# medivhna/TF_Face_Toolbox

Hardware: AMD Instinct MI355X
Metric: images/sec (whole node), SphereFaceNet-20 112x112 bs512 (higher is better)
Workload: dtype f32; 1 GPU; SphereFaceNet-20 + A-softmax training step, 112x112x3, global batch 512, 10575 classes, Momentum, fp32; global_batch=512, per_gpu_batch=512, parallelism=dp1

## Files before the change

include/fte.h:

```cpp
#ifndef FTE_H_
#define FTE_H_

#include <stddef.h>
#include <stdint.h>

#ifdef __cplusplus
extern "C" {
#endif

#define FTE_OK 0
#define FTE_EINVAL (-1)
#define FTE_EWORKSPACE (-2)

const char* fte_version(void);

#define FTE_MFMA_F32 0
#define FTE_MFMA_BF16 1
int fte_set_mfma_dtype(int dtype);
int fte_get_mfma_dtype(void);

#define FTE_CONV_DIRECT 0
#define FTE_CONV_WINOGRAD 1
#define FTE_CONV_AUTO 2
int fte_set_conv_algo(int algo);
int fte_get_conv_algo(void);
int fte_conv3x3_algo(int n, int h, int wd, int cin, int cout, int stride, int op);
size_t fte_wino_pack_bytes(int n, int h, int wd, int c);

int fte_prof_enable(int on);
int fte_prof_count(void);
int fte_prof_get(int i, int* sig, double* flops, float* ms);
int fte_prof_get_shape(int i, int* mnk, double* bytes);
int fte_prof_get_name(int i, char* buf, int buflen);


int fte_conv3x3_fwd(const float* x, const float* w, const float* bias, const float* alpha,
                    const float* res, float* z, float* y,
                    int n, int h, int wd, int cin, int cout, int stride,
                    void* ws, size_t ws_bytes, void* stream);
size_t fte_conv3x3_fwd_ws_bytes(int n, int h, int wd, int cin, int cout, int stride);
int fte_conv3x3_fwd_keep(const float* x, const float* w, const float* bias, const float* alpha,
                         const float* res, float* z, float* y,
                         int n, int h, int wd, int cin, int cout, int stride, float* vpack,
                         void* ws, size_t ws_bytes, void* stream);
int fte_conv3x3_fwd_keep_act(const float* x, const float* xalpha, const float* w, const float* bias, const float* alpha,
                             const float* res, float* z, float* y,
                             int n, int h, int wd, int cin, int cout, int stride, float* vpack,
                             void* ws, size_t ws_bytes, void* stream);

int fte_conv3x3_dgrad(const float* dz, const float* w, const float* addin,
                      const float* zprev, const float* alpha_prev,
                      float* raw, float* dzprev, float* dalpha_prev, float* dbias_prev,
                      int n, int h, int wd, int cin, int cout, int stride,
                      void* ws, size_t ws_bytes, void* stream);
size_t fte_conv3x3_dgrad_ws_bytes(int n, int h, int wd, int cin, int cout, int stride);

int fte_conv3x3_wgrad(const float* x, const float* dz, float* dw,
                      int n, int h, int wd, int cin, int cout, int stride,
                      void* ws, size_t ws_bytes, void* stream);
size_t fte_conv3x3_wgrad_ws_bytes(int n, int h, int wd, int cin, int cout, int stride);
int fte_conv3x3_wgrad_kept(const float* x, const float* dz, float* dw,
                           int n, int h, int wd, int cin, int cout, int stride, const float* vpack,
                           void* ws, size_t ws_bytes, void* stream);


int fte_conv2d_fwd(const float* x, const float* w, const float* bias, const float* alpha, const float* res,
                   float* z, float* y, int n, int h, int wd, int cin, int cout, int ksize, int stride,
                   void* ws, size_t ws_bytes, void* stream);
size_t fte_conv2d_fwd_ws_bytes(int n, int h, int wd, int cin, int cout, int ksize, int stride);
int fte_conv2d_dgrad(const float* dz, const float* w, const float* addin, const float* zprev,
                     const float* alpha_prev, float* raw, float* dzprev, float* dalpha_prev, float* dbias_prev,
                     int n, int h, int wd, int cin, int cout, int ksize, int stride,
                     void* ws, size_t ws_bytes, void* stream);
size_t fte_conv2d_dgrad_ws_bytes(int n, int h, int wd, int cin, int cout, int ksize, int stride);
int fte_conv2d_wgrad(const float* x, const float* dz, float* dw, int n, int h, int wd, int cin, int cout,
                     int ksize, int stride, void* ws, size_t ws_bytes, void* stream);
size_t fte_conv2d_wgrad_ws_bytes(int n, int h, int wd, int cin, int cout, int ksize, int stride);

int fte_im2col_first(const float* x, float* cols, int n, int h, int wd, int cin, int ksize, int stride,
                     int kpad, void* stream);
int fte_im2col_first_s16(const float* x, uint16_t* cols16, int n, int h, int wd, int cin, int ksize, int stride, int kpad, void* stream);

int fte_preprocess_u8(const uint8_t* slots, float* out, int n, long slot_stride, int channels, int in_h, int in_w, int crop_h, int crop_w,
                      void* stream);
int fte_preprocess_u8_aug(const uint8_t* slots, float* out, int n, long slot_stride, int channels, int in_h, int in_w, int crop_h,
                          int crop_w, void* stream);
size_t fte_preprocess_u8_geo_ws_bytes(int n, int channels, int crop_h, int crop_w);
int fte_preprocess_u8_geo(const uint8_t* slots, float* out, int n, long slot_stride, int channels, int in_h, int in_w, int crop_h,
                          int crop_w, const float* affine_table, void* ws, size_t ws_bytes, void* stream);

size_t fte_bn_ws_bytes(int c);
int fte_bn_train_fwd(const float* z, const float* gamma, const float* beta, const float* res, float* y,
                     float* mean, float* rstd, float* scale, float* shift, float* moving_mean, float* moving_var,
                     long rows, int c, float eps, float decay, int relu, void* ws, size_t ws_bytes, void* stream);
int fte_bn_infer_fwd(const float* z, const float* gamma, const float* beta, const float* moving_mean,
                     const float* moving_var, const float* res, float* y, float* scale, float* shift,
                     long rows, int c, float eps, int relu, void* stream);
int fte_bn_train_bwd(const float* dy, const float* ymask, const float* z, const float* gamma, const float* mean,
                     const float* rstd, float* dz, float* dgamma, float* dbeta, long rows, int c,
                     void* ws, size_t ws_bytes, void* stream);
int fte_bn_train_bwd_zmask(const float* dy, const float* z, const float* gamma, const float* mean, const float* rstd,
                           const float* scale, const float* shift, float* dz, float* dgamma, float* dbeta, long rows, int c,
                           void* ws, size_t ws_bytes, void* stream);
int fte_bn_train_bwd_res(const float* dy, const float* y, const float* z, const float* gamma, const float* mean, const float* rstd,
                         float* g_out, float* dz, float* dgamma, float* dbeta, long rows, int c,
                         void* ws, size_t ws_bytes, void* stream);
int fte_bn_train_stats(const float* z, const float* gamma, const float* beta, float* mean, float* rstd, float* scale, float* shift,
                       float* moving_mean, float* moving_var, long rows, int c, float eps, float decay,
                       void* ws, size_t ws_bytes, void* stream);
int fte_bn_infer_coef(const float* gamma, const float* beta, const float* moving_mean, const float* moving_var,
                      float* scale, float* shift, int c, float eps, void* stream);
size_t fte_bn_prelu_ws_bytes(int c);
int fte_bn_prelu_apply(const float* z, const float* scale, const float* shift, const float* alpha, float* y, long rows, int c,
                       void* stream);
int fte_bn_prelu_infer_fwd(const float* z, const float* gamma, const float* beta, const float* moving_mean, const float* moving_var,
                           const float* alpha, float* y, float* scale, float* shift, long rows, int c, float eps, void* stream);
int fte_bn_prelu_train_bwd(const float* dy, const float* z, const float* gamma, const float* mean, const float* rstd,
                           const float* scale, const float* shift, const float* alpha, float* dz, float* dgamma, float* dbeta,
                           float* dalpha, long rows, int c, void* ws, size_t ws_bytes, void* stream);
size_t fte_se_lin_ws_bytes(int n, int hw, int c);
int fte_se_lin_squeeze(const float* z, const float* scale, const float* shift, const float* mean, const float* rstd, float* sq, float* xm,
                       int n, int hw, int c, void* ws, size_t ws_bytes, void* stream);
int fte_se_lin_apply_fwd(const float* z, const float* scale, const float* shift, const float* gate, const float* shortcut, float* out,
                         int n, int hw, int c, void* stream);
int fte_se_lin_bwd_sums(const float* dy, const float* z, const float* gamma, const float* beta, const float* mean, const float* rstd,
                        const float* gate, float* s1, float* s2, float* dgate, int n, int hw, int c, void* ws, size_t ws_bytes, void* stream);
int fte_relu_bwd(const float* dy, const float* y, float* g, long n, void* stream);

int fte_maxpool3x3s2_fwd(const float* x, float* y, uint8_t* idx, int n, int h, int wd, int c, void* stream);
int fte_maxpool3x3s2_bwd(const float* dy, const uint8_t* idx, float* dx, int n, int h, int wd, int c, void* stream);
int fte_gap_fwd(const float* x, float* y, int n, int hw, int c, void* stream);
int fte_gap_bwd(const float* dy, float* dx, int n, int hw, int c, void* stream);
int fte_dropout_fwd(const float* x, float* mask, float* y, long n, float keep_prob, uint64_t seed, void* stream);
int fte_dropout_bwd(const float* dy, const float* mask, float* dx, long n, float keep_prob, void* stream);

int fte_gconv3x3_fwd(const float* x, const float* w, float* y, int n, int h, int wd, int c, int groups,
                     int stride, void* stream);
int fte_gconv3x3_pack_bf16(const float* w, uint16_t* wpk_fwd, uint16_t* wpk_dgrad, int c, int groups, void* stream);
// ... 245 lines not shown
```

tf_face_toolbox_amd/_lib.py:

```python
import ctypes
import os
from ctypes import c_char_p, c_float, c_int, c_long, c_size_t, c_uint64, c_void_p

_HERE = os.path.dirname(os.path.abspath(__file__))
LIB_PATH = os.environ.get('FTE_LIB') or os.path.join(_HERE, 'libfte.so')


class FteError(RuntimeError):
    pass


_P = c_void_p
_SIGS = {
    'fte_version': (c_char_p, []),
    'fte_prof_enable': (c_int, [c_int]),
    'fte_prof_count': (c_int, []),
    'fte_prof_get': (c_int, [c_int, _P, _P, _P]),
    'fte_prof_get_shape': (c_int, [c_int, _P, _P]),
    'fte_prof_get_name': (c_int, [c_int, _P, c_int]),
    'fte_conv3x3_fwd': (c_int, [_P] * 7 + [c_int] * 6 + [_P, c_size_t, _P]),
    'fte_conv3x3_fwd_ws_bytes': (c_size_t, [c_int] * 6),
    'fte_conv3x3_dgrad': (c_int, [_P] * 9 + [c_int] * 6 + [_P, c_size_t, _P]),
    'fte_conv3x3_dgrad_ws_bytes': (c_size_t, [c_int] * 6),
    'fte_conv3x3_wgrad': (c_int, [_P] * 3 + [c_int] * 6 + [_P, c_size_t, _P]),
# ... 19 lines not shown
    'fte_bn_train_stats': (c_int, [_P] * 9 + [c_long, c_int, c_float, c_float, _P, c_size_t, _P]),
    'fte_bn_infer_coef': (c_int, [_P] * 6 + [c_int, c_float, _P]),
    'fte_bn_prelu_ws_bytes': (c_size_t, [c_int]),
    'fte_bn_prelu_apply': (c_int, [_P] * 5 + [c_long, c_int, _P]),
    'fte_bn_prelu_infer_fwd': (c_int, [_P] * 9 + [c_long, c_int, c_float, _P]),
    'fte_bn_prelu_train_bwd': (c_int, [_P] * 12 + [c_long, c_int, _P, c_size_t, _P]),
    'fte_se_lin_ws_bytes': (c_size_t, [c_int] * 3),
    'fte_se_lin_squeeze': (c_int, [_P] * 7 + [c_int] * 3 + [_P, c_size_t, _P]),
    'fte_se_lin_apply_fwd': (c_int, [_P] * 6 + [c_int] * 3 + [_P]),
    'fte_se_lin_bwd_sums': (c_int, [_P] * 10 + [c_int] * 3 + [_P, c_size_t, _P]),
    'fte_relu_bwd': (c_int, [_P] * 3 + [c_long, _P]),
    'fte_maxpool3x3s2_fwd': (c_int, [_P] * 3 + [c_int] * 4 + [_P]),
    'fte_maxpool3x3s2_bwd': (c_int, [_P] * 3 + [c_int] * 4 + [_P]),
    'fte_gap_fwd': (c_int, [_P] * 2 + [c_int] * 3 + [_P]),
    'fte_gap_bwd': (c_int, [_P] * 2 + [c_int] * 3 + [_P]),
    'fte_dropout_fwd': (c_int, [_P] * 3 + [c_long, c_float, c_uint64, _P]),
    'fte_dropout_bwd': (c_int, [_P] * 3 + [c_long, c_float, _P]),
    'fte_gconv3x3_fwd': (c_int, [_P] * 3 + [c_int] * 6 + [_P]),
    'fte_gconv3x3_pack_bf16': (c_int, [_P] * 3 + [c_int, c_int, _P]),
    'fte_gconv3x3_bf16': (c_int, [_P] * 3 + [c_int] * 6 + [_P]),
    'fte_gconv3x3_wgrad_bf16_ws_bytes': (c_size_t, [c_int] * 6),
    'fte_gconv3x3_wgrad_bf16': (c_int, [_P] * 3 + [c_int] * 6 + [_P, c_size_t, _P]),
    'fte_gconv3x3_dgrad': (c_int, [_P] * 3 + [c_int] * 6 + [_P]),
    'fte_gconv3x3_wgrad': (c_int, [_P] * 3 + [c_int] * 6 + [_P, c_size_t, _P]),
    'fte_gconv3x3_wgrad_ws_bytes': (c_size_t, [c_int] * 6),
    'fte_bcast_add': (c_int, [_P] * 2 + [c_int] * 3 + [c_float, _P]),
    'fte_act_fwd': (c_int, [_P] * 2 + [c_long, c_int, _P]),
    'fte_act_bwd': (c_int, [_P] * 3 + [c_long, c_int, _P]),
    'fte_channel_scale_fwd': (c_int, [_P] * 3 + [c_int] * 3 + [_P]),
    'fte_channel_scale_bwd': (c_int, [_P] * 5 + [c_int] * 4 + [_P]),
    'fte_to_bf16': (c_int, [_P, _P, c_long, _P]),
    'fte_pack_weights_bf16': (c_int, [_P, _P, _P, c_int, c_int, c_int, _P]),
    'fte_pack_weights_bf16_table': (c_int, [_P, _P, _P, c_int, c_long, c_int, _P]),
    'fte_conv2d_fwd16': (c_int, [_P] * 8 + [c_int] * 7 + [_P, c_size_t, _P]),
    'fte_conv2d_dgrad16': (c_int, [_P] * 10 + [c_int] * 7 + [_P, c_size_t, _P]),
    'fte_conv2d_wgrad16': (c_int, [_P] * 3 + [c_int] * 7 + [_P, c_size_t, _P]),
    'fte_conv2d_fwd_s16': (c_int, [_P] * 9 + [c_int] * 7 + [_P, c_size_t, _P]),
    'fte_conv2d_dgrad_s16': (c_int, [_P] * 9 + [c_int] * 7 + [_P, c_size_t, _P]),
    'fte_conv3x3_first_fwd_s16': (c_int, [_P] * 6 + [c_int] * 6 + [_P]),
    'fte_conv3x3_first_wgrad_s16': (c_int, [_P] * 3 + [c_int] * 6 + [_P, c_size_t, _P]),
    'fte_bn_train_fwd_s16': (c_int, [_P] * 11 + [c_long, c_int, c_float, c_float, c_int, c_int, _P, c_size_t, _P]),
    'fte_bn_infer_fwd_s16': (c_int, [_P] * 9 + [c_long, c_int, c_float, c_int, c_int, _P]),
    'fte_bn_train_bwd_s16': (c_int, [_P] * 12 + [c_long, c_int, c_int, _P, c_size_t, _P]),
    'fte_relu_bwd_s16': (c_int, [_P] * 3 + [c_long, _P]),
    'fte_maxpool3x3s2_fwd_s16': (c_int, [_P] * 3 + [c_int] * 4 + [_P]),
    'fte_maxpool3x3s2_bwd_s16': (c_int, [_P] * 3 + [c_int] * 4 + [_P]),
    'fte_gap_fwd_s16': (c_int, [_P] * 2 + [c_int] * 3 + [_P]),
    'fte_gap_bwd_s16': (c_int, [_P] * 2 + [c_int] * 3 + [_P]),
    'fte_gconv3x3_bf16_s16': (c_int, [_P] * 3 + [c_int] * 6 + [_P]),
    'fte_gconv3x3_wgrad_bf16_s16': (c_int, [_P] * 3 + [c_int] * 6 + [_P, c_size_t, _P]),
    'fte_channel_scale_fwd_s16': (c_int, [_P] * 3 + [c_int] * 3 + [_P]),
    'fte_channel_scale_bwd_s16': (c_int, [_P] * 4 + [c_int] * 4 + [_P]),
    'fte_channel_scale_bwd_apply_s16': (c_int, [_P] * 4 + [c_int] * 3 + [c_float, _P]),
    'fte_dense_small': (c_int, [_P] * 5 + [c_int] * 5 + [_P]),
    'fte_se_squeeze': (c_int, [_P] * 7 + [c_int] * 4 + [_P]),
    'fte_se_apply_fwd': (c_int, [_P] * 6 + [c_int] * 4 + [_P]),
    'fte_se_bwd_gate': (c_int, [_P] * 12 + [c_int] * 4 + [_P]),
    'fte_se_bn_bwd_coef': (c_int, [_P] * 11 + [c_int] * 3 + [_P]),
    'fte_se_bn_bwd_apply': (c_int, [_P] * 6 + [c_int] * 4 + [_P]),
    'fte_dwconv3x3_fwd_s16': (c_int, [_P] * 3 + [c_int] * 5 + [_P]),
    'fte_dwconv3x3_dgrad_s16': (c_int, [_P] * 3 + [c_int] * 5 + [_P]),
    'fte_dwconv3x3_wgrad_s16': (c_int, [_P] * 3 + [c_int] * 5 + [_P, c_size_t, _P]),
    'fte_channel_gather_s16': (c_int, [_P] * 4 + [c_long] + [c_int] * 3 + [_P]),
    'fte_channel_gather_affine_s16': (c_int, [_P] * 4 + [c_int, _P, _P, c_int, c_long, c_int, c_int, _P, _P, c_int, _P, _P, c_int, _P]),
    'fte_bn_train_stats_s16': (c_int, [_P] * 9 + [c_long, c_int, c_float, c_float, c_int, _P, c_size_t, _P]),
    'fte_conv2d_bn_fwd_ws_bytes': (c_size_t, [c_int] * 7),
    'fte_conv2d_bn_fwd': (c_int, [_P] * 11 + [c_float, c_float] + [_P] * 3 + [c_int] * 8 + [_P, c_size_t, _P]),
    'fte_conv2d_bn_fwd_folds': (c_int, [c_int] * 8),
    'fte_conv2d_dgrad_bn_ws_bytes': (c_size_t, [c_int] * 7),
    'fte_conv2d_dgrad_bn': (c_int, [_P] * 14 + [c_int] * 8 + [_P, c_size_t, _P]),
    'fte_bn_apply': (c_int, [_P] * 5 + [c_long, c_int, c_int, c_int, _P]),
    'fte_bn_bwd_apply': (c_int, [_P] * 4 + [c_long, c_int, c_int, _P]),
    'fte_gconv3x3_bn_ws_bytes': (c_size_t, [c_int] * 5),
    'fte_gconv3x3_bn_fwd_bf16_s16': (c_int, [_P] * 11 + [c_float, c_float] + [_P] * 3 + [c_int] * 5 + [_P, c_size_t, _P]),
    'fte_gconv3x3_dgrad_bn_bf16_s16': (c_int, [_P] * 12 + [c_int] * 5 + [_P, c_size_t, _P]),
    'fte_set_mfma_dtype': (c_int, [c_int]),
    'fte_get_mfma_dtype': (c_int, []),
    'fte_set_conv_algo': (c_int, [c_int]),
    'fte_conv3x3_algo': (c_int, [c_int] * 7),
    'fte_wino_pack_bytes': (c_size_t, [c_int] * 4),
    'fte_conv3x3_fwd_keep': (c_int, [_P] * 7 + [c_int] * 6 + [_P, _P, c_size_t, _P]),
    'fte_conv3x3_fwd_keep_act': (c_int, [_P] * 8 + [c_int] * 6 + [_P, _P, c_size_t, _P]),
    'fte_conv3x3_wgrad_kept': (c_int, [_P] * 3 + [c_int] * 6 + [_P, _P, c_size_t, _P]),
    'fte_get_conv_algo': (c_int, []),
    'fte_l2_normalize_rows': (c_int, [_P] * 3 + [c_int] * 2 + [_P]),
    'fte_pair_scores': (c_int, [_P] * 4 + [c_int] * 3 + [_P]),
    'fte_topk_search_ws_bytes': (c_size_t, [c_int] * 4),
    'fte_topk_search': (c_int, [_P] * 2 + [c_int] * 7 + [_P] * 3 + [c_size_t, _P]),
    'fte_topk_merge': (c_int, [_P] * 2 + [c_int] * 3 + [_P] * 3),
    'fte_score_histograms': (c_int, [_P, _P, c_int, _P, _P] + [c_int] * 4 + [_P] * 3),
    'fte_template_pool': (c_int, [_P, _P, c_int, c_int, _P, c_int, _P, c_int, _P, c_int, _P, _P]),
    'fte_set_pair_scores': (c_int, [_P, c_int, c_int, _P, c_int, _P, c_int, _P, c_int, _P, _P, c_int, _P, c_int, _P, _P]),
    'fte_megaface_pair_scores': (c_int, [_P, c_int, _P, c_int, c_int, _P, _P, c_int, _P, _P]),
    'fte_megaface_scan_ws_bytes': (c_size_t, [c_int] * 2),
    'fte_megaface_scan': (c_int, [_P, c_int, _P, c_int, c_int, _P, _P, c_int, c_int, _P, _P, _P, c_size_t, _P]),
    'fte_pfc_sample_ws_bytes': (c_size_t, [c_int]),
    'fte_pfc_sample': (c_int, [_P] + [c_int] * 5 + [_P] * 4 + [c_size_t, _P]),
    'fte_pfc_gather_cols': (c_int, [_P] * 3 + [c_int] * 5 + [_P]),
    'fte_pfc_scatter_cols': (c_int, [_P] * 3 + [c_int] * 5 + [_P]),
    'fte_pfc_momentum_update_cols': (c_int, [_P] * 4 + [c_int] * 5 + [c_float] * 4 + [_P]),
    'fte_pfc_adam_update_cols': (c_int, [_P] * 5 + [c_int] * 5 + [c_float] * 6 + [c_int, _P]),
    'fte_knn_links_threshold': (c_int, [_P] * 2 + [c_int] * 2 + [c_float, c_int, _P, _P]),
    'fte_knn_links_rank_order': (c_int, [_P] * 2 + [c_int] * 2 + [c_float] * 2 + [_P, _P]),
    'fte_components': (c_int, [_P] * 2 + [c_int] * 2 + [_P] * 3),
    'fte_dwconv3x3_fwd': (c_int, [_P] * 3 + [c_int] * 5 + [_P]),
    'fte_dwconv3x3_dgrad': (c_int, [_P] * 3 + [c_int] * 5 + [_P]),
    'fte_dwconv3x3_wgrad': (c_int, [_P] * 3 + [c_int] * 5 + [_P, c_size_t, _P]),
    'fte_dwconv3x3_wgrad_ws_bytes': (c_size_t, [c_int] * 5),
    'fte_channel_gather': (c_int, [_P] * 4 + [c_long] + [c_int] * 3 + [_P]),
    'fte_channel_gather_affine': (c_int, [_P] * 4 + [c_int, _P, _P, c_int, c_long, c_int, c_int, _P, _P, c_int, _P, _P, c_int, _P]),
    'fte_conv3x3_first_fwd': (c_int, [_P] * 6 + [c_int] * 6 + [_P]),
    'fte_conv3x3_first_wgrad': (c_int, [_P] * 3 + [c_int] * 6 + [_P, c_size_t, _P]),
    'fte_conv3x3_first_wgrad_ws_bytes': (c_size_t, [c_int] * 6),
    'fte_gemm_nn': (c_int, [_P] * 4 + [c_int] * 3 + [_P, c_size_t, _P]),
    'fte_gemm_nn_act': (c_int, [_P] * 4 + [c_int] * 4 + [_P, c_size_t, _P]),
    'fte_gemm_nt': (c_int, [_P] * 4 + [c_int] + [_P] * 3 + [c_int] * 3 + [_P, c_size_t, _P]),
    'fte_gemm_tn': (c_int, [_P] * 3 + [c_int] * 3 + [_P, c_size_t, _P]),
    'fte_gemm_ws_bytes': (c_size_t, [c_int] * 3),
    'fte_softmax_ce_fwd_bwd': (c_int, [_P] * 4 + [c_int] * 3 + [c_float, _P]),
    'fte_focal_loss_fwd_bwd': (c_int, [_P] * 4 + [c_int] * 3 + [c_float] * 3 + [_P]),
    'fte_asoftmax_fwd_bwd': (c_int, [_P] * 4 + [c_float] + [_P] * 4 + [c_int] * 3 + [c_float, _P]),
    'fte_asoftmax_colcoef': (c_int, [_P] * 4 + [c_int] * 3 + [_P]),
    'fte_margin_softmax_fwd_bwd': (c_int, [_P] * 4 + [c_float] * 3 + [_P] * 4 + [c_int] * 3 + [c_float, _P]),
    'fte_margin_softmax_rows_fwd_bwd': (c_int, [_P] * 4 + [c_float] + [_P] * 6 + [c_int] * 3 + [c_float, _P]),
    'fte_subcenter_margin_softmax_fwd_bwd': (c_int, [_P] * 4 + [c_int] + [c_float] * 3 + [_P] * 4 + [c_int] * 3 + [c_float, _P]),
    'fte_subcenter_colcoef': (c_int, [_P] * 4 + [c_int] * 4 + [_P]),
    'fte_subcenter_assign': (c_int, [_P] * 3 + [c_int] + [_P] * 2 + [c_int] * 3 + [_P]),
    'fte_adaface_margins': (c_int, [_P, c_int] + [c_float] * 3 + [c_int] + [_P] * 4),
    'fte_row_norms': (c_int, [_P] * 2 + [c_int] * 3 + [_P]),
    'fte_col_norms': (c_int, [_P] * 2 + [c_int] * 3 + [_P]),
    'fte_add_scaled_rows_cols': (c_int, [_P] * 4 + [c_int] * 3 + [_P]),
    'fte_flip_width': (c_int, [_P] * 2 + [c_int] * 4 + [_P]),
    'fte_axpby': (c_int, [c_float, _P, c_float, _P, _P, c_long, _P]),
    'fte_center_loss_fwd_bwd_update': (c_int, [_P] * 5 + [c_int] * 3 + [c_float] * 2 + [_P, c_size_t, _P]),
    'fte_center_scatter_update': (c_int, [_P] * 3 + [c_int] * 3 + [c_float, _P]),
    'fte_batch_hard_triplet_fwd_bwd': (c_int, [_P] * 2 + [c_float, c_int, c_float] + [_P] * 2 + [c_int] * 2 + [_P, c_size_t, _P]),
    'fte_reduce_rows': (c_int, [_P] * 3 + [c_int, c_long, c_long, c_int, c_float, _P]),
    'fte_sumsq': (c_int, [_P, c_long, c_float, _P, _P, c_size_t, _P]),
    'fte_sum': (c_int, [_P, c_long, c_float, _P, _P, c_size_t, _P]),
    'fte_momentum_update': (c_int, [_P] * 3 + [c_long] + [c_float] * 4 + [_P]),
    'fte_adam_update': (c_int, [_P] * 4 + [c_long] + [c_float] * 6 + [c_int, _P]),
}

_lib = None


def exported_names():
    return sorted(_SIGS)


_CODES = {-1: 'FTE_EINVAL -- a null pointer, a shape the kernel family does not tile (channel multiples, stride, '
              'ksize) or a tensor of 2 GiB or more (buffer-load range)',
          -2: 'FTE_EWORKSPACE -- workspace missing or smaller than the matching *_ws_bytes() query'}

MFMA_DTYPES = {'f32': 0, 'fp32': 0, 'float32': 0, 'bf16': 1, 'bfloat16': 1, 'bf16s': 1}
_storage16 = False


def load():
    global _lib
    if _lib is not None:
        return _lib
    if not os.path.exists(LIB_PATH):
        raise FteError('libfte.so not found at %s -- build it with `python -c "import __graft_entry__ as g; g.build()"` '
                       '(or tf_face_toolbox_amd/csrc/build.sh). There is no CPU fallback.' % LIB_PATH)
    lib = ctypes.CDLL(LIB_PATH)
# ... 101 lines not shown
```

tf_face_toolbox_amd/csrc/api.hip:

```cpp
#include <hip/hip_runtime.h>
#include <stdio.h>
#include <stdlib.h>
#include <string.h>

#include <initializer_list>

#include "../../include/fte.h"
#include "igemm.h"
#include "wgrad16.h"
#include "pw16.h"
#include "kernels.h"
#include "layers.h"
#include "wino.h"
#include "search.h"
#include "partial_fc.h"
#include "cluster.h"
#include "iresnet.h"

namespace {

struct Pads { int out, before; };
inline Pads same_pads(int in, int k, int stride) {
    const int out = (in + stride - 1) / stride;
    int total = (out - 1) * stride + k - in;
// ... 267 lines not shown
    const WinoGeom g = wino_geom(n, h, wd);
    WinoWs w;
    w.v_off = align_up(head);
    if (op == 0) {
        w.u_off = w.v_off + align_up(wino_pack_floats(g.M, cin) * 4);
        w.slab_off = w.total = w.u_off + align_up((size_t)16 * cin * cout * 4);
    } else if (op == 1) {
        w.u_off = w.v_off + align_up(wino_pack_floats(g.M, cout) * 4);
        w.slab_off = w.total = w.u_off + align_up((size_t)16 * cin * cout * 4);
    } else {
        w.u_off = w.v_off + align_up(wino_pack_floats(g.M, cin) * 4);
        w.slab_off = w.u_off;
        w.total = w.slab_off + align_up((size_t)wino_wgrad_splits(cin, cout) * 16 * cin * cout * 4);
    }
    return w;
}
}

extern "C" {

#ifndef FTE_SRC_SHA
#define FTE_SRC_SHA "unstamped"
#endif
const char* fte_version(void) { return "fte 0.2 gfx950 fp32-mfma src:" FTE_SRC_SHA; }

int fte_to_bf16(const float* x, uint16_t* y, long n, void* stream) {
    if (!x || !y || n <= 0 || n % 4) return FTE_EINVAL;
    return rc(k_to_bf16(x, y, n, (hipStream_t)stream));
}
int fte_pack_weights_bf16(const float* w, uint16_t* w16, uint16_t* w16t, int ksize, int cin, int cout, void* stream) {
    if (!w || (!w16 && !w16t) || ksize <= 0 || cin <= 0 || cout <= 0) return FTE_EINVAL;
    return rc(k_pack_weights_bf16(w, w16, w16t, ksize * ksize, cin, cout, (hipStream_t)stream));
}

int fte_pack_weights_bf16_table(const float* params, uint16_t* dst, const int32_t* table, int nconv, long total, int transposed, void* stream) {
    if (!params || !dst || !table || nconv <= 0 || nconv > 64 || total <= 0 || total % 4) return FTE_EINVAL;
    return rc(k_pack_weights_table(params, dst, table, nconv, total, transposed, (hipStream_t)stream));
}

int fte_set_mfma_dtype(int dtype) {
    if (dtype != FTE_MFMA_F32 && dtype != FTE_MFMA_BF16) return FTE_EINVAL;
    igemm_set_bf16(dtype == FTE_MFMA_BF16);
    return FTE_OK;
}
int fte_get_mfma_dtype(void) { return igemm_get_bf16() ? FTE_MFMA_BF16 : FTE_MFMA_F32; }

int fte_set_conv_algo(int algo) {
    if (algo < FTE_CONV_DIRECT || algo > FTE_CONV_AUTO) return FTE_EINVAL;
    wino_set_algo(algo);
    return FTE_OK;
}
int fte_get_conv_algo(void) { return wino_get_algo(); }

int fte_prof_enable(int on) { igemm_prof_enable(on != 0, on == 1); return FTE_OK; }
int fte_prof_count(void) { return igemm_prof_count(); }
int fte_prof_get_shape(int i, int* mnk, double* bytes) {
    if (!mnk || !bytes) return FTE_EINVAL;
    return rc(igemm_prof_get_shape(i, mnk, bytes));
}
int fte_prof_get_name(int i, char* buf, int buflen) {
    if (!buf || buflen <= 0) return FTE_EINVAL;
    return rc(igemm_prof_get_name(i, buf, buflen));
}
int fte_prof_get(int i, int* sig, double* flops, float* ms) {
    if (!sig || !flops || !ms) return FTE_EINVAL;
    return rc(igemm_prof_get(i, sig, flops, ms));
}

size_t fte_conv2d_fwd_ws_bytes(int n, int h, int wd, int cin, int cout, int ksize, int stride) {
    if (n <= 0 || cin <= 0 || cin % 32 || cout <= 0 || cout % 64) return 0;
    const Pads ph = same_pads(h, ksize, stride), pw = same_pads(wd, ksize, stride);
    size_t need = both_modes([&] { return plan_rows((long)n * ph.out * pw.out, cout, (long)ksize * ksize * cin, true, false, EPI_FWD).pw_bytes; });
    if (wino_sized(n, h, wd, cin, cout, ksize, stride, 0)) {
        const size_t wn = wino_ws(n, h, wd, cin, cout, 0, 0).total;
        if (wn > need) need = wn;
    }
    return need;
}

static int conv2d_fwd_impl(const void* x, const void* w, bool src16, const float* bias, const float* alpha, const float* res,
                           float* z, float* y, uint16_t* y16, int n, int h, int wd, int cin, int cout, int ksize, int stride,
                           void* ws, size_t ws_bytes, void* stream, const uint16_t* res16 = nullptr, uint16_t* z16 = nullptr,
                           float* stat_part = nullptr, int* stat_rows = nullptr, float* vpack = nullptr,
                           const float* xalpha = nullptr, bool z_only_ok = false) {
    const bool z_only = z_only_ok && !y && z && vpack;
    if ((xalpha || z_only_ok) && !vpack) return FTE_EINVAL;
    if (!x || !w || (!y && !(src16 && y16) && !z_only) || n <= 0 || cin % 32 || cout % 64 || (stride != 1 && stride != 2) || (ksize != 1 && ksize != 3))
        return FTE_EINVAL;
    const Pads ph = same_pads(h, ksize, stride), pw = same_pads(wd, ksize, stride);
    IgemmParams p;
    zero_params(&p);
    p.M = n * ph.out * pw.out; p.N = cout; p.K = ksize * ksize * cin; p.kchunk = p.K;
    p.a_OH = ph.out; p.a_OW = pw.out; p.a_IH = h; p.a_IW = wd; p.a_stride = stride;
    p.a_ld = cin; p.a_KC = cin; p.a_NT = ksize * ksize;
    for (int r = 0; r < ksize; ++r)
        for (int s = 0; s < ksize; ++s) { p.a_dh[r * ksize + s] = r - ph.before; p.a_dw[r * ksize + s] = s - pw.before; }
    p.A = (const float*)x;
    p.B = (const float*)w;
    p.c_ld = cout;
    p.Y = y; p.Z = z; p.R = res; p.bias = bias; p.alpha = alpha; p.Y16 = y16;
    p.R16 = res16; p.Z16 = z16;
    int bl = BL_KN;
    if (src16) {
        p.src16 = 1; p.b_ld = cin; bl = BL_NK;
        for (int t = 0; t < ksize * ksize; ++t) p.b_tapoff[t] = t * cout * cin;
    } else {
        p.b_ld = cout;
    }
    if (!set_bytes(&p, (size_t)n * h * wd * cin, (size_t)ksize * ksize * cin * cout, src16 ? 2 : 4)) return FTE_EINVAL;
    if (!src16 && !stat_part && (y || z_only) && wino_wanted(n, h, wd, cin, cout, ksize, stride, 0)) {
        WinoWs wl = wino_ws(n, h, wd, cin, cout, 0, 0);
        if (vpack) { wl.u_off = 0; wl.total = align_up((size_t)16 * cin * cout * 4); }
        if (ws && ws_bytes >= wl.total) {
            if (!aligned16({x, w, bias, alpha, res, z, y, ws, vpack, xalpha})) return FTE_EINVAL;
            float* V = vpack ? vpack : (float*)((char*)ws + wl.v_off);
            float* U = (float*)((char*)ws + wl.u_off);
            hipError_t e = wino_transform_filter((const float*)w, U, cin, cout, 0, (hipStream_t)stream);
            if (e != hipSuccess) return (int)e;
            e = wino_transform_tiles((const float*)x, V, n, h, wd, cin, 0, (hipStream_t)stream, wino_fwd_small_tiles(), xalpha);
            if (e != hipSuccess) return (int)e;
            WinoMMParams q;
            memset(&q, 0, sizeof(q));
            q.V = V; q.U = U; q.K = cin; q.N = cout; q.g = wino_geom(n, h, wd);
            q.Y = y; q.Z = z; q.R = res; q.bias = bias; q.alpha = alpha;
            return rc(wino_mm(q, EPI_FWD, (hipStream_t)stream));
        }
    }
    if (vpack) return FTE_EWORKSPACE;
    RowPlan rp = plan_rows(p.M, p.N, p.K, ws != nullptr, false, EPI_FWD);
    if (rp.tail_mode >= 2 && ws_bytes < rp.pw_bytes) rp = plan_rows(p.M, p.N, p.K, false);
    if (stat_part) {
        if (rp.tail_mode == 2) return FTE_EINVAL;
        p.SP = stat_part;
        *stat_rows = (int)(rp.main_mtiles + rp.tail_mtiles);
    }
    return rc(launch_rows(p, rp, AL_MK, bl, EPI_FWD, 0, (float*)ws, (hipStream_t)stream));
}
int fte_conv2d_fwd(const float* x, const float* w, const float* bias, const float* alpha, const float* res,
                   float* z, float* y, int n, int h, int wd, int cin, int cout, int ksize, int stride,
                   void* ws, size_t ws_bytes, void* stream) {
    return conv2d_fwd_impl(x, w, false, bias, alpha, res, z, y, nullptr, n, h, wd, cin, cout, ksize, stride, ws, ws_bytes, stream);
}
int fte_conv2d_fwd16(const uint16_t* x16, const uint16_t* w16t, const float* bias, const float* alpha, const float* res,
                     float* z, float* y, uint16_t* y16, int n, int h, int wd, int cin, int cout, int ksize, int stride,
                     void* ws, size_t ws_bytes, void* stream) {
    Plan16 guard;
    return conv2d_fwd_impl(x16, w16t, true, bias, alpha, res, z, y, y16, n, h, wd, cin, cout, ksize, stride, ws, ws_bytes, stream);
}

int fte_conv2d_fwd_s16(const uint16_t* x16, const uint16_t* w16t, const float* bias, const float* alpha, const uint16_t* res16,
                       uint16_t* z16, uint16_t* y16, float* z32, float* y32, int n, int h, int wd, int cin, int cout, int ksize, int stride,
                       void* ws, size_t ws_bytes, void* stream) {
    if (!y16 || (res16 && ((uintptr_t)res16 & 15))) return FTE_EINVAL;
    Plan16 guard;
    PlanS16 storage(!z32 && !y32);
    return conv2d_fwd_impl(x16, w16t, true, bias, alpha, nullptr, z32, y32, y16, n, h, wd, cin, cout, ksize, stride, ws, ws_bytes, stream, res16, z16);
}

size_t fte_conv3x3_fwd_ws_bytes(int n, int h, int wd, int cin, int cout, int stride) {
    return fte_conv2d_fwd_ws_bytes(n, h, wd, cin, cout, 3, stride);
}
int fte_conv3x3_fwd(const float* x, const float* w, const float* bias, const float* alpha, const float* res,
                    float* z, float* y, int n, int h, int wd, int cin, int cout, int stride,
                    void* ws, size_t ws_bytes, void* stream) {
    return fte_conv2d_fwd(x, w, bias, alpha, res, z, y, n, h, wd, cin, cout, 3, stride, ws, ws_bytes, stream);
}
int fte_conv3x3_fwd_keep(const float* x, const float* w, const float* bias, const float* alpha, const float* res,
                         float* z, float* y, int n, int h, int wd, int cin, int cout, int stride, float* vpack,
                         void* ws, size_t ws_bytes, void* stream) {
    if (vpack && ((uintptr_t)vpack & 15)) return FTE_EINVAL;
    return conv2d_fwd_impl(x, w, false, bias, alpha, res, z, y, nullptr, n, h, wd, cin, cout, 3, stride, ws, ws_bytes, stream,
                           nullptr, nullptr, nullptr, nullptr, vpack);
}
int fte_conv3x3_fwd_keep_act(const float* x, const float* xalpha, const float* w, const float* bias, const float* alpha, const float* res,
                             float* z, float* y, int n, int h, int wd, int cin, int cout, int stride, float* vpack,
                             void* ws, size_t ws_bytes, void* stream) {
    if (!vpack || ((uintptr_t)vpack & 15) || (!y && !z)) return FTE_EINVAL;
    return conv2d_fwd_impl(x, w, false, bias, alpha, res, z, y, nullptr, n, h, wd, cin, cout, 3, stride, ws, ws_bytes, stream,
                           nullptr, nullptr, nullptr, nullptr, vpack, xalpha, true);
}
int fte_conv3x3_algo(int n, int h, int wd, int cin, int cout, int stride, int op) {
    if (op < 0 || op > 2) return FTE_EINVAL;
    return (!igemm_get_bf16() && wino_sized(n, h, wd, cin, cout, 3, stride, op)) ? FTE_CONV_WINOGRAD : FTE_CONV_DIRECT;
}
size_t fte_wino_pack_bytes(int n, int h, int wd, int c) {
    if (n <= 0 || h < 2 || wd < 2 || c <= 0 || c % 64) return 0;
    return wino_pack_floats(wino_geom(n, h, wd).M, c) * sizeof(float);
}

namespace {
struct DgradClass { int ph, pw, hq, wq, ntap, dh[9], dw[9], wt[9]; RowPlan rp; long mtiles; };
int dgrad_classes(int n, int h, int wd, int cin, int cout, int ksize, int stride, DgradClass* cls) {
    const Pads ph = same_pads(h, ksize, stride), pw = same_pads(wd, ksize, stride);
    int nc = 0;
    for (int a = 0; a < stride; ++a)
        for (int b = 0; b < stride; ++b) {
            DgradClass& c = cls[nc];
            c.ph = a; c.pw = b;
            c.hq = (h - a + stride - 1) / stride;
            c.wq = (wd - b + stride - 1) / stride;
            c.ntap = 0;
            if (c.hq <= 0 || c.wq <= 0) continue;
            for (int r = 0; r < ksize; ++r) {
                if ((a + ph.before - r) % stride) continue;
                for (int s = 0; s < ksize; ++s) {
                    if ((b + pw.before - s) % stride) continue;
                    c.dh[c.ntap] = (a + ph.before - r) / stride;
                    c.dw[c.ntap] = (b + pw.before - s) / stride;
                    c.wt[c.ntap] = r * ksize + s;
                    ++c.ntap;
                }
            }
            const long M = (long)n * c.hq * c.wq;
            static const bool cls_big = getenv("FTE_DGRAD_CLS_BIG") && atoi(getenv("FTE_DGRAD_CLS_BIG")) == 1;
            c.rp = plan_rows(M, cin, (long)c.ntap * cout, true, stride != 1 && !cls_big, EPI_DGRAD);
            c.mtiles = c.rp.main_mtiles + c.rp.tail_mtiles;
            ++nc;
        }
    return nc;
}
static bool dgrad_merged16() {
    static const bool on = getenv("FTE_DGRAD_MERGED16") && atoi(getenv("FTE_DGRAD_MERGED16")) == 1;
    return on && plan_bf16();
}
bool dgrad_mergeable(const DgradClass* cls, int nc, int n, int cin) {
    static const char* mode = getenv("FTE_DGRAD_CLASSES");
    if (nc != 4 || (mode && mode[0] == 's')) return false;
    for (int i = 0; i < nc; ++i)
        if (cls[i].hq != cls[0].hq || cls[i].wq != cls[0].wq || cls[i].ntap < 1) return false;
    if ((mode && mode[0] == 'm') || dgrad_merged16()) return true;
    const long tiles = (((long)n * cls[0].hq * cls[0].wq + 63) / 64) * (cin / 64);
    return tiles < SLOTS;
}
static int dgrad_merged_tile(int cin) {
    if (!dgrad_merged16()) return TILE_64x64;
    return cin % 128 == 0 ? TILE_128x128 : TILE_128x64;
}
long dgrad_merged_rows(const DgradClass* cls, int nc, int n, int cin) {
    if (!dgrad_mergeable(cls, nc, n, cin)) return 0;
    int bm, bn;
    igemm_tile_dims(dgrad_merged_tile(cin), &bm, &bn);
    return (long)nc * (((long)n * cls[0].hq * cls[0].wq + bm - 1) / bm);
}
int dgrad_merged_plan(const DgradClass* cls, int nc, int n, int cin, int* order) {
    for (int i = 0; i < nc; ++i) order[i] = i;
    for (int i = 0; i < nc; ++i)
        for (int j = i + 1; j < nc; ++j)
            if (cls[order[j]].ntap > cls[order[i]].ntap) { const int t = order[i]; order[i] = order[j]; order[j] = t; }
    (void)n;
    return dgrad_merged_tile(cin);
}
}

size_t fte_conv2d_dgrad_ws_bytes(int n, int h, int wd, int cin, int cout, int ksize, int stride) {
    if (n <= 0 || cin <= 0 || cin % 64 || cout % 32) return 0;
    size_t need = both_modes([&] {
        DgradClass cls[4];
        const int nc = dgrad_classes(n, h, wd, cin, cout, ksize, stride, cls);
        long rows = 0;
        size_t pw = 0;
        for (int i = 0; i < nc; ++i) { rows += cls[i].mtiles; if (cls[i].rp.pw_bytes > pw) pw = cls[i].rp.pw_bytes; }
        const long merged_rows = dgrad_merged_rows(cls, nc, n, cin);
        if (merged_rows > rows) rows = merged_rows;
        return 2 * align_up((size_t)rows * cin * sizeof(float)) + SCRATCH_BYTES + pw;
    });
    if (wino_sized(n, h, wd, cin, cout, ksize, stride, 1)) {
        const WinoGeom g = wino_geom(n, h, wd);
        const size_t wn = wino_ws(n, h, wd, cin, cout, 1, 2 * align_up((size_t)g.MB * cin * sizeof(float)) + SCRATCH_BYTES).total;
        if (wn > need) need = wn;
    }
    return need;
}

struct DgradBn {
    const void* zbn; const void* ybn;
    const float* gamma; const float* mean; const float* rstd; const float* scale; const float* shift;
    float* dgamma; float* dbeta; float* coef;
};
static int conv2d_dgrad_impl(const void* dz, const void* w, bool src16, const float* addin, const float* zprev,
                             const float* alpha_prev, float* raw, float* dzprev, uint16_t* dzprev16, float* dalpha_prev, float* dbias_prev,
                             int n, int h, int wd, int cin, int cout, int ksize, int stride, void* ws, size_t ws_bytes, void* stream,
                             const uint16_t* addin16 = nullptr, const uint16_t* zprev16 = nullptr, uint16_t* raw16 = nullptr,
                             const DgradBn* bn = nullptr) {
    const float* zx = nullptr;
    const uint16_t* zx16 = nullptr;
    if (bn) {
        const void* msk = (!bn->scale && bn->ybn) ? bn->ybn : bn->zbn;
        const void* zb = (!bn->scale && bn->ybn) ? bn->zbn : nullptr;
        if (src16) { zprev16 = (const uint16_t*)msk; zx16 = (const uint16_t*)zb; }
        else { zprev = (const float*)msk; zx = (const float*)zb; }
        alpha_prev = bn->gamma;
        dalpha_prev = bn->dgamma; dbias_prev = bn->dbeta;
    }
    if (zprev16 && !zprev) zprev = reinterpret_cast<const float*>(zprev16);
    const bool z16only = zprev16 != nullptr;
    if (!dz || !w || (!dzprev && !(src16 && dzprev16)) || n <= 0 || cout % 32 || cin % 64 || (stride != 1 && stride != 2) || (ksize != 1 && ksize != 3)) return FTE_EINVAL;
    if (zprev && !alpha_prev) return FTE_EINVAL;
    const Pads pho = same_pads(h, ksize, stride), pwo = same_pads(wd, ksize, stride);
    if (!src16 && !bn && dzprev && !dzprev16 && !addin16 && !zprev16 && !raw16 && wino_wanted(n, h, wd, cin, cout, ksize, stride, 1)) {
        const WinoGeom g = wino_geom(n, h, wd);
        const size_t half_w = align_up((size_t)g.MB * cin * sizeof(float));
        const WinoWs wl = wino_ws(n, h, wd, cin, cout, 1, 2 * half_w + SCRATCH_BYTES);
        if (ws && ws_bytes >= wl.total) {
            if (!aligned16({dz, w, addin, zprev, alpha_prev, raw, dzprev, ws})) return FTE_EINVAL;
            const bool part = zprev && (dalpha_prev || dbias_prev);
            float* V = (float*)((char*)ws + wl.v_off);
            float* U = (float*)((char*)ws + wl.u_off);
            hipError_t e = wino_transform_filter((const float*)w, U, cin, cout, 1, (hipStream_t)stream);
            if (e != hipSuccess) return (int)e;
            e = wino_transform_tiles((const float*)dz, V, n, h, wd, cout, 0, (hipStream_t)stream);
            if (e != hipSuccess) return (int)e;
            WinoMMParams q;
            memset(&q, 0, sizeof(q));
            q.V = V; q.U = U; q.K = cout; q.N = cin; q.g = g;
            q.ADD = addin; q.RAW = raw; q.Zin = zprev; q.alpha = alpha_prev; q.amod = cin; q.DZ = dzprev;
            q.PA = part ? (float*)ws : nullptr; q.PB = part ? (float*)((char*)ws + half_w) : nullptr;
            e = wino_mm(q, EPI_DGRAD, (hipStream_t)stream);
            if (e != hipSuccess) return (int)e;
            if (part) {
                float* scratch = (float*)((char*)ws + 2 * half_w);
                if (dalpha_prev && dbias_prev) return rc(k_reduce_rows2(q.PA, dalpha_prev, q.PB, dbias_prev, nullptr, 1, g.MB, cin, 1, 1.f, scratch, (hipStream_t)stream));
                if (dalpha_prev) return rc(k_reduce_rows(q.PA, dalpha_prev, nullptr, 1, g.MB, cin, 1, 1.f, scratch, (hipStream_t)stream));
                return rc(k_reduce_rows(q.PB, dbias_prev, nullptr, 1, g.MB, cin, 1, 1.f, scratch, (hipStream_t)stream));
            }
            return FTE_OK;
        }
    }
    DgradClass cls[4];
    const int nc = dgrad_classes(n, h, wd, cin, cout, ksize, stride, cls);
    const bool merged = dgrad_mergeable(cls, nc, n, cin);
    long rows = 0;
    for (int i = 0; i < nc; ++i) rows += cls[i].mtiles;
    if (merged) rows = dgrad_merged_rows(cls, nc, n, cin);
    const bool want_part = zprev && (dalpha_prev || dbias_prev);
    const size_t half = align_up((size_t)rows * cin * sizeof(float));
    size_t pw_need = 0;
    for (int i = 0; i < nc && !merged; ++i) if (cls[i].rp.pw_bytes > pw_need) pw_need = cls[i].rp.pw_bytes;
    const size_t fixed = 2 * half + SCRATCH_BYTES;
    if ((want_part || pw_need) && (!ws || ws_bytes < fixed + pw_need)) return FTE_EWORKSPACE;
    float* scratch = want_part ? (float*)((char*)ws + 2 * half) : nullptr;
    float* pwbuf = pw_need ? (float*)((char*)ws + fixed) : nullptr;
    float* PA = want_part ? (float*)ws : nullptr;
    float* PB = want_part ? (float*)((char*)ws + half) : nullptr;
    if (merged) {
        int order[4];
        const int tile = dgrad_merged_plan(cls, nc, n, cin, order);
        IgemmParams p;
        zero_params(&p);
        const DgradClass& c0 = cls[0];
        p.M = n * c0.hq * c0.wq; p.N = cin; p.a_KC = cout;
        p.A = (const float*)dz; p.a_OH = c0.hq; p.a_OW = c0.wq; p.a_IH = pho.out; p.a_IW = pwo.out; p.a_stride = 1; p.a_ld = cout;
        p.ncls = nc;
        int t = 0;
        for (int k = 0; k < nc; ++k) {
            const DgradClass& c = cls[order[k]];
            p.cls_tap0[k] = t; p.cls_ph[k] = c.ph; p.cls_pw[k] = c.pw;
            for (int j = 0; j < c.ntap; ++j, ++t) { p.a_dh[t] = c.dh[j]; p.a_dw[t] = c.dw[j]; p.b_tapoff[t] = c.wt[j] * cin * cout; }
        }
        p.cls_tap0[nc] = t;
        p.a_NT = t; p.K = t * cout; p.kchunk = p.K;
        p.B = (const float*)w; p.b_ld = cout;
        p.c_OH = c0.hq; p.c_OW = c0.wq; p.c_FH = h; p.c_FW = wd; p.c_step = stride; p.c_ld = cin;
        p.ADD = addin; p.RAW = raw; p.Zin = z16only ? nullptr : zprev; p.alpha = alpha_prev; p.amod = cin; p.DZ = dzprev;
        p.ADD16 = addin16; p.Zin16 = zprev16; p.RAW16 = raw16;
        p.PA = PA; p.PB = PB; p.prow0 = 0;
        if (bn) { p.bn_mu = bn->mean; p.bn_rs = bn->rstd; p.bn_sc = bn->scale; p.bn_sh = bn->shift; p.Zx = zx; p.Zx16 = zx16; }
        p.src16 = src16 ? 1 : 0; p.DZ16 = dzprev16;
        if (!set_bytes(&p, (size_t)n * pho.out * pwo.out * cout, (size_t)ksize * ksize * cin * cout, src16 ? 2 : 4)) return FTE_EINVAL;
        hipError_t e = igemm_launch(p, AL_MK, BL_NK, EPI_DGRAD, tile, 1, (hipStream_t)stream);
        if (e != hipSuccess) return (int)e;
    } else {
    long prow = 0;
    for (int i = 0; i < nc; ++i) {
        const DgradClass& c = cls[i];
        IgemmParams p;
        zero_params(&p);
        p.M = n * c.hq * c.wq; p.N = cin; p.K = c.ntap * cout; p.kchunk = p.K;
        p.A = (const float*)dz; p.a_OH = c.hq; p.a_OW = c.wq; p.a_IH = pho.out; p.a_IW = pwo.out; p.a_stride = 1;
        p.a_ld = cout; p.a_KC = cout; p.a_NT = c.ntap;
        for (int t = 0; t < c.ntap; ++t) {
            p.a_dh[t] = c.dh[t]; p.a_dw[t] = c.dw[t];
            p.b_tapoff[t] = c.wt[t] * cin * cout;
        }
        p.B = (const float*)w; p.b_ld = cout;
        p.src16 = src16 ? 1 : 0; p.DZ16 = dzprev16;
        if (stride == 1) { p.c_OH = 0; }
        else { p.c_OH = c.hq; p.c_OW = c.wq; p.c_FH = h; p.c_FW = wd; p.c_step = stride; p.c_ph = c.ph; p.c_pw = c.pw; }
        p.c_ld = cin;
        p.ADD = addin; p.RAW = raw; p.Zin = z16only ? nullptr : zprev; p.alpha = alpha_prev; p.amod = cin; p.DZ = dzprev;
        p.ADD16 = addin16; p.Zin16 = zprev16; p.RAW16 = raw16;
        p.PA = PA; p.PB = PB;
        if (bn) { p.bn_mu = bn->mean; p.bn_rs = bn->rstd; p.bn_sc = bn->scale; p.bn_sh = bn->shift; p.Zx = zx; p.Zx16 = zx16; }
        if (!set_bytes(&p, (size_t)n * pho.out * pwo.out * cout, (size_t)ksize * ksize * cin * cout, src16 ? 2 : 4)) return FTE_EINVAL;
        hipError_t e = launch_rows(p, c.rp, AL_MK, BL_NK, EPI_DGRAD, prow, pwbuf, (hipStream_t)stream);
        if (e != hipSuccess) return (int)e;
        prow += c.mtiles;
    }
    }
    if (bn)
        return rc(l_bn_bwd_finalize(PB, PA, cin, (int)rows, (long)n * h * wd, cin, bn->gamma, bn->mean, bn->rstd, bn->dgamma, bn->dbeta,
                                    bn->coef, (hipStream_t)stream));
    if (want_part) {
        if (dalpha_prev && dbias_prev) {
            hipError_t e = k_reduce_rows2(PA, dalpha_prev, PB, dbias_prev, nullptr, 1, rows, cin, 1, 1.f, scratch, (hipStream_t)stream);
            if (e != hipSuccess) return (int)e;
        } else {
            if (dalpha_prev) { hipError_t e = k_reduce_rows(PA, dalpha_prev, nullptr, 1, rows, cin, 1, 1.f, scratch, (hipStream_t)stream); if (e != hipSuccess) return (int)e; }
            if (dbias_prev) { hipError_t e = k_reduce_rows(PB, dbias_prev, nullptr, 1, rows, cin, 1, 1.f, scratch, (hipStream_t)stream); if (e != hipSuccess) return (int)e; }
        }
    }
    return FTE_OK;
}

int fte_conv2d_dgrad(const float* dz, const float* w, const float* addin, const float* zprev,
                     const float* alpha_prev, float* raw, float* dzprev, float* dalpha_prev, float* dbias_prev,
                     int n, int h, int wd, int cin, int cout, int ksize, int stride, void* ws, size_t ws_bytes, void* stream) {
    return conv2d_dgrad_impl(dz, w, false, addin, zprev, alpha_prev, raw, dzprev, nullptr, dalpha_prev, dbias_prev,
                             n, h, wd, cin, cout, ksize, stride, ws, ws_bytes, stream);
}
int fte_conv2d_dgrad16(const uint16_t* dz16, const uint16_t* w16, const float* addin, const float* zprev,
                       const float* alpha_prev, float* raw, float* dzprev, uint16_t* dzprev16, float* dalpha_prev, float* dbias_prev,
                       int n, int h, int wd, int cin, int cout, int ksize, int stride, void* ws, size_t ws_bytes, void* stream) {
    Plan16 guard;
    return conv2d_dgrad_impl(dz16, w16, true, addin, zprev, alpha_prev, raw, dzprev, dzprev16, dalpha_prev, dbias_prev,
                             n, h, wd, cin, cout, ksize, stride, ws, ws_bytes, stream);
}

int fte_conv2d_dgrad_s16(const uint16_t* dz16, const uint16_t* w16, const uint16_t* addin16, const uint16_t* zprev16,
                         const float* alpha_prev, uint16_t* raw16, uint16_t* dzprev16, float* dalpha_prev, float* dbias_prev,
                         int n, int h, int wd, int cin, int cout, int ksize, int stride, void* ws, size_t ws_bytes, void* stream) {
    if (!dzprev16) return FTE_EINVAL;
    Plan16 guard;
    PlanS16 storage(true);
    return conv2d_dgrad_impl(dz16, w16, true, nullptr, nullptr, alpha_prev, nullptr, nullptr, dzprev16, dalpha_prev, dbias_prev,
                             n, h, wd, cin, cout, ksize, stride, ws, ws_bytes, stream, addin16, zprev16, raw16);
}

size_t fte_conv3x3_dgrad_ws_bytes(int n, int h, int wd, int cin, int cout, int stride) {
    return fte_conv2d_dgrad_ws_bytes(n, h, wd, cin, cout, 3, stride);
}
int fte_conv3x3_dgrad(const float* dz, const float* w, const float* addin, const float* zprev,
                      const float* alpha_prev, float* raw, float* dzprev, float* dalpha_prev, float* dbias_prev,
                      int n, int h, int wd, int cin, int cout, int stride, void* ws, size_t ws_bytes, void* stream) {
    return fte_conv2d_dgrad(dz, w, addin, zprev, alpha_prev, raw, dzprev, dalpha_prev, dbias_prev,
                            n, h, wd, cin, cout, 3, stride, ws, ws_bytes, stream);
}

namespace {
inline bool wgrad_split_major() {
    static const bool on = !getenv("FTE_WGRAD_SPLIT_MAJOR") || atoi(getenv("FTE_WGRAD_SPLIT_MAJOR")) != 0;
    return on;
}
void wgrad_plan(int n, int h, int wd, int cin, int cout, int ksize, int stride, int* tile, int* splits, int* kchunk, int* K) {
    const Pads ph = same_pads(h, ksize, stride), pw = same_pads(wd, ksize, stride);
    *K = n * ph.out * pw.out;
    const long M = (long)ksize * ksize * cin;
    static const int wg_tile = getenv("FTE_WGRAD_TILE") ? atoi(getenv("FTE_WGRAD_TILE")) : -1;
    const int narrow = (M % 192 == 0 && M % 128 != 0) ? TILE_192x64 : TILE_128x64;
    const bool tiny = ksize == 1 && M * cout <= 256L * 256;
    *tile = wg_tile >= 0 ? wg_tile : (tiny ? TILE_64x64 : (cout % 128 == 0) ? TILE_128x128 : narrow);
    plan_splits(tiles_of(*tile, M, cout), *K, splits, kchunk, false);
    if (wg_tile < 0 && *tile != TILE_64x64 && *splits > 1 && *kchunk < 1024) {
        *tile = TILE_64x64;
        plan_splits(tiles_of(*tile, M, cout), *K, splits, kchunk, false);
    }
}
}

size_t fte_conv2d_wgrad_ws_bytes(int n, int h, int wd, int cin, int cout, int ksize, int stride) {
    if (n <= 0 || cin <= 0 || cin % 4 || cout <= 0 || cout % 64) return 0;
    int tile, splits, kchunk, K;
    wgrad_plan(n, h, wd, cin, cout, ksize, stride, &tile, &splits, &kchunk, &K);
    size_t need = splits > 1 ? (size_t)splits * ksize * ksize * cin * cout * sizeof(float) : 0;
    if (ksize == 3 && stride == 1) {
        Wgrad16Params g;
        int cfg = 0;
        if (wgrad16_plan(n, h, wd, cin, cout, &g, &cfg) && g.S > 1) {
            const size_t gneed = (size_t)g.S * g.slab * sizeof(float);
            if (gneed > need) need = gneed;
        }
    }
    if (ksize == 1 && stride == 1) {
        Wgrad16Params g;
        int cfg = 0;
        if (wgrad16p_plan(n, h, wd, cin, cout, &g, &cfg) && g.S > 1) {
            const size_t gneed = (size_t)g.S * g.slab * sizeof(float);
            if (gneed > need) need = gneed;
        }
    }
    if (wino_sized(n, h, wd, cin, cout, ksize, stride, 2)) {
        const size_t wn = wino_ws(n, h, wd, cin, cout, 2, 0).total;
        if (wn > need) need = wn;
    }
    return need + SCRATCH_BYTES;
}
size_t fte_conv3x3_wgrad_ws_bytes(int n, int h, int wd, int cin, int cout, int stride) {
    return fte_conv2d_wgrad_ws_bytes(n, h, wd, cin, cout, 3, stride);
}

static int conv2d_wgrad_impl(const void* x, const void* dz, bool src16, float* dw, int n, int h, int wd, int cin, int cout, int ksize, int stride,
                             void* ws, size_t ws_bytes, void* stream, const float* vpack = nullptr) {
    if (src16 && (cin % 8 || cout % 8)) return FTE_EINVAL;
    if ((!x && !vpack) || !dz || !dw || n <= 0 || cin % 4 || cout % 64 || (stride != 1 && stride != 2) || (ksize != 1 && ksize != 3)) return FTE_EINVAL;
    const Pads ph = same_pads(h, ksize, stride), pw = same_pads(wd, ksize, stride);
    {
        const size_t lim = (size_t)1 << 31, es = src16 ? 2 : 4;
        if ((size_t)n * h * wd * cin * es >= lim || (size_t)n * ph.out * pw.out * cout * es >= lim) return FTE_EINVAL;
    }
    int tile, splits, kchunk, K;
    wgrad_plan(n, h, wd, cin, cout, ksize, stride, &tile, &splits, &kchunk, &K);
    if (!src16 && wino_wanted(n, h, wd, cin, cout, ksize, stride, 2)) {
        WinoWs wl = wino_ws(n, h, wd, cin, cout, 2, 0);
        if (vpack) {
            const size_t vsz = wl.u_off - wl.v_off;
            wl.u_off -= vsz; wl.slab_off -= vsz; wl.total -= vsz;
        }
        if (ws && ws_bytes >= wl.total) {
            if (!aligned16({x, dz, dw, ws, vpack})) return FTE_EINVAL;
            const float* V = vpack ? vpack : (float*)((char*)ws + wl.v_off);
            float* slabs = (float*)((char*)ws + wl.slab_off);
            hipError_t e = hipSuccess;
            if (!vpack) e = wino_transform_tiles((const float*)x, (float*)((char*)ws + wl.v_off), n, h, wd, cin, 0, (hipStream_t)stream);
            if (e != hipSuccess) return (int)e;
            return rc(wino_wgrad(V, (const float*)dz, slabs, dw, wino_geom(n, h, wd), cin, cout, (hipStream_t)stream));
        }
    }
    if (vpack) return FTE_EWORKSPACE;
    if (src16 && ksize == 3 && stride == 1) {
// ... 1086 lines not shown
```

tf_face_toolbox_amd/csrc/kernels.h:

```cpp
#pragma once
#include <hip/hip_runtime.h>
#include <stdint.h>

hipError_t k_pack_weights_table(const float* params, unsigned short* w16t, const int* table, int nconv, long total, int transposed, hipStream_t st);
hipError_t k_conv_first_fwd(const float* x, const float* w, const float* bias, const float* alpha, float* z, float* y,
                            unsigned short* z16, unsigned short* y16, int n, int h, int wd, int cin, int cout, int ho, int wo, int stride, int pt, int pl, hipStream_t st);
int k_conv_first_wgrad_blocks(long npix);
hipError_t k_conv_first_wgrad(const float* x, const float* dz, const unsigned short* dz16, float* part, int n, int h, int wd, int cin, int cout, int ho, int wo,
                              int stride, int pt, int pl, int blocks, hipStream_t st);
constexpr long REDUCE_SCRATCH_FLOATS = 1 << 18;
hipError_t k_reduce_rows(const float* in, float* out, const float* bias, int bmod, long rows, long cols, int fold, float scale,
                         float* scratch, hipStream_t st, int act = 0);
hipError_t k_reduce_rows2(const float* in, float* out, const float* in2, float* out2, const float* bias, int bmod, long rows, long cols,
                          int fold, float scale, float* scratch, hipStream_t st, int act = 0);
hipError_t k_sum(const float* a, long n, float scale, float* out, float* ws, bool sq, hipStream_t st);
hipError_t k_softmax_ce(const float* logits, const int32_t* labels, float* loss_rows, float* dlogits, int n, int c, int ld, float gs, hipStream_t st);
hipError_t k_to_bf16(const float* x, unsigned short* y, long n, hipStream_t st);
hipError_t k_pack_weights_bf16(const float* w, unsigned short* w16, unsigned short* w16t, int taps, int cin, int cout, hipStream_t st);
hipError_t k_focal_loss(const float* logits, const int32_t* labels, float* loss_rows, float* dlogits, int n, int c, int ld,
                        float gamma, float alpha, float gs, hipStream_t st);
hipError_t k_asoftmax(const float* s, const float* xn, const float* wn, const int32_t* labels, float lam, float* f, float* loss_rows,
                      float* G, float* rowcoef, int n, int c, int ld, float gs, hipStream_t st);
hipError_t k_margin_softmax(const float* s, const float* xn, const float* wn, const int32_t* labels, float scale, float m, float m3,
                            float* f, float* loss_rows, float* G, float* rowcoef, int n, int c, int ld, float gs, hipStream_t st);
hipError_t k_margin_softmax_rows(const float* s, const float* xn, const float* wn, const int32_t* labels, float scale, const float* a_rows,
                                 const float* b_rows, float* f, float* loss_rows, float* G, float* rowcoef, int n, int c, int ld, float gs,
                                 hipStream_t st);
hipError_t k_subcenter_margin_softmax(const float* s, const float* xn, const float* wn, const int32_t* labels, int K, float scale, float m,
                                      float m3, float* f, float* loss_rows, float* G, float* rowcoef, int n, int c, int ld, float gs,
                                      hipStream_t st);
hipError_t k_subcenter_colcoef(const float* G, const float* s, const float* wn, float* cc, int K, int n, int c, int ld, hipStream_t st);
hipError_t k_subcenter_assign(const float* x, const float* wt, const int32_t* labels, int K, int32_t* sel, float* cosv, int n, int d, int c,
                              hipStream_t st);
hipError_t k_adaface_margins(const float* xn, int n, float m, float h, float t_alpha, int update, float* stats, float* a_rows, float* b_rows,
                             hipStream_t st);
hipError_t k_asoftmax_colcoef(const float* G, const float* s, const float* wn, float* cc, int n, int c, int ld, hipStream_t st);
hipError_t k_row_norms(const float* a, float* out, int rows, int cols, int ld, hipStream_t st);
hipError_t k_col_norms(const float* a, float* out, int rows, int cols, int ld, hipStream_t st);
hipError_t k_add_scaled(float* a, const float* b, const float* rc, const float* cc, int rows, int cols, int ld, hipStream_t st);
hipError_t k_flip_w(const float* x, float* y, long rows, int w, int c, hipStream_t st);
hipError_t k_axpby(float a, const float* x, float b, const float* y, float* out, long n, hipStream_t st);
hipError_t k_center_loss(const float* feat, const int32_t* labels, float* centers, float* loss_rows, float* dfeat,
                         int n, int d, int num_classes, float alpha, float gs, float* ws, hipStream_t st);
hipError_t k_center_update(const float* diff, const int32_t* labels, float* centers, int n, int d, int num_classes, float alpha, hipStream_t st);
hipError_t k_triplet(const float* feat, const int32_t* labels, float margin, bool soft, float lw, float* loss_rows, float* dfeat,
                     int n, int d, float* ws, hipStream_t st);
hipError_t k_dense_small(const float* a, const float* w, const float* bias, const float* mask, float* out, int m, int n, int k,
                         bool trans_w, int act, bool bf16, hipStream_t st);
hipError_t k_momentum(float* w, float* acc, const float* g, long n, float lr, float mom, float wd, float gs, hipStream_t st);
hipError_t k_adam(float* w, float* m, float* v, const float* g, long n, float lr_t, float b1, float b2, float eps, float wd, float gs, hipStream_t st);
hipError_t k_preprocess_u8(const unsigned char* slots, float* out, int n, long slot_stride, int channels, int in_h, int in_w,
                           int crop_h, int crop_w, hipStream_t st);
hipError_t k_preprocess_u8_aug(const unsigned char* slots, float* out, int n, long slot_stride, int channels, int in_h, int in_w,
                               int crop_h, int crop_w, hipStream_t st);
size_t k_preprocess_u8_geo_ws_bytes(int n, int channels, int crop_h, int crop_w);
hipError_t k_preprocess_u8_geo(const unsigned char* slots, float* out, int n, long slot_stride, int channels, int in_h, int in_w,
                               int crop_h, int crop_w, const float* table, void* ws, hipStream_t st);
```

tf_face_toolbox_amd/csrc/kernels.hip:

```cpp
#include <hip/hip_runtime.h>
#include <stdint.h>
#include <stdlib.h>
#include <math.h>

#include "kernels.h"

typedef float f32x4 __attribute__((ext_vector_type(4)));

namespace {

__device__ __forceinline__ float wave_sum(float v) {
#pragma unroll
    for (int o = 32; o > 0; o >>= 1) v += __shfl_xor(v, o);
    return v;
}
__device__ __forceinline__ float wave_max(float v) {
#pragma unroll
    for (int o = 32; o > 0; o >>= 1) v = fmaxf(v, __shfl_xor(v, o));
    return v;
}
__device__ __forceinline__ float block_sum(float v, float* sh) {
    v = wave_sum(v);
    __syncthreads();
    if ((threadIdx.x & 63) == 0) sh[threadIdx.x >> 6] = v;
// ... 91 lines not shown

typedef float f32x16k __attribute__((ext_vector_type(16)));
template <int CIN, int COUT>
__global__ __launch_bounds__(256) void conv_first_wgrad_kernel(
    const float* __restrict__ x, const float* __restrict__ dz, const unsigned short* __restrict__ dz16, float* __restrict__ part,
    int n, int h, int wd, int ho, int wo, int stride, int pt, int pl, long rows_per_block) {
    constexpr int NH = COUT / 32, K = 9 * CIN;
    __shared__ float red[4][32][COUT];
    const int lane = threadIdx.x & 63, wv = threadIdx.x >> 6;
    const int li = lane & 31, lh = lane >> 5;
    const bool kok = li < K;
    const int tap = kok ? li / CIN : 0, ch = kok ? li - tap * CIN : 0;
    const int r = tap / 3, sx = tap - r * 3;
    const long nrows = (long)n * ho;
    const long r0 = (long)blockIdx.x * rows_per_block, r1 = min(nrows, r0 + rows_per_block);
    f32x16k acc[NH];
#pragma unroll
    for (int e = 0; e < NH; ++e)
#pragma unroll
        for (int i = 0; i < 16; ++i) acc[e][i] = 0.f;
    constexpr int UP = 4;
    const int tpr = (wo + 2 * UP - 1) / (2 * UP);
    const long myrows = r1 > r0 + wv ? (r1 - r0 - wv + 3) / 4 : 0;
    const long ntrips = myrows * tpr;
    auto fetch = [&](long t, float (&a)[UP], float (&bv)[NH][UP]) {
        const long rk = t / tpr;
        const int ow0 = (int)(t - rk * tpr) * 2 * UP;
        const long row = r0 + wv + 4 * rk;
        const int img = (int)(row / ho), oh = (int)(row - (long)img * ho);
        const int ih = oh * stride + r - pt;
        const bool rok = kok && ih >= 0 && ih < h;
        const float* xrow = x + ((long)(img * h + (rok ? ih : 0)) * wd) * CIN + ch;
        const float* drow = dz ? dz + row * wo * COUT : nullptr;
        const unsigned short* drow16 = dz16 ? dz16 + row * wo * COUT : nullptr;
#pragma unroll
        for (int u = 0; u < UP; ++u) {
            const int ow = ow0 + 2 * u + lh;
            const bool pok = ow < wo;
            const int iw = ow * stride + sx - pl;
            const bool ok = rok && pok && iw >= 0 && iw < wd;
            const float av = xrow[(long)(ok ? iw : 0) * CIN];
            a[u] = ok ? av : 0.f;
            const long doff = (long)(pok ? ow : 0) * COUT + NH * li;
            if constexpr (NH == 2) {
                float v0, v1;
                if (drow) { const float2 tt = *reinterpret_cast<const float2*>(drow + doff); v0 = tt.x; v1 = tt.y; }
                else { const unsigned tt = *reinterpret_cast<const unsigned*>(drow16 + doff); v0 = __builtin_bit_cast(float, tt << 16); v1 = __builtin_bit_cast(float, tt & 0xffff0000u); }
                bv[0][u] = pok ? v0 : 0.f; bv[1][u] = pok ? v1 : 0.f;
            } else {
                const float v = drow ? drow[doff] : __builtin_bit_cast(float, (unsigned)drow16[doff] << 16);
                bv[0][u] = pok ? v : 0.f;
            }
        }
    };
    float a0[UP], b0[NH][UP], a1[UP], b1[NH][UP];
    if (ntrips > 0) fetch(0, a0, b0);
    for (long t = 0; t < ntrips; t += 2) {
        if (t + 1 < ntrips) fetch(t + 1, a1, b1);
#pragma unroll
        for (int u = 0; u < UP; ++u)
#pragma unroll
            for (int e = 0; e < NH; ++e) acc[e] = __builtin_amdgcn_mfma_f32_32x32x2f32(a0[u], b0[e][u], acc[e], 0, 0, 0);
        if (t + 1 < ntrips) {
            if (t + 2 < ntrips) fetch(t + 2, a0, b0);
#pragma unroll
            for (int u = 0; u < UP; ++u)
#pragma unroll
                for (int e = 0; e < NH; ++e) acc[e] = __builtin_amdgcn_mfma_f32_32x32x2f32(a1[u], b1[e][u], acc[e], 0, 0, 0);
        }
    }
#pragma unroll
    for (int i = 0; i < 16; ++i) {
        const int k = (i & 3) + 8 * (i >> 2) + 4 * lh;
#pragma unroll
        for (int e = 0; e < NH; ++e) red[wv][k][NH * li + e] = acc[e][i];
    }
    __syncthreads();
    for (int i = threadIdx.x; i < K * COUT; i += 256) {
        const int k = i / COUT, c = i % COUT;
        part[(long)blockIdx.x * K * COUT + i] = (red[0][k][c] + red[1][k][c]) + (red[2][k][c] + red[3][k][c]);
    }
}

__global__ __launch_bounds__(256) void reduce_rows_kernel(const float* __restrict__ in, float* __restrict__ out,
                                                          const float* __restrict__ bias, int bmod, long rows,
                                                          long cols, long rows_per_split, float scale,
                                                          const float* __restrict__ in2, float* __restrict__ out2, int act) {
    __shared__ float sh[4][64];
    if (blockIdx.z == 1) { in = in2; out = out2; }
    const int c = threadIdx.x & 63, rl = threadIdx.x >> 6;
    const long j = (long)blockIdx.x * 64 + c;
    const long r0 = (long)blockIdx.y * rows_per_split;
    const long r1 = min(rows, r0 + rows_per_split);
    float s0 = 0.f, s1 = 0.f;
    if (j < cols) {
        long r = r0 + rl;
        for (; r + 28 < r1; r += 32) {
            float v[8];
#pragma unroll
            for (int u = 0; u < 8; ++u) v[u] = in[(r + 4 * u) * cols + j];
            s0 += (v[0] + v[2]) + (v[4] + v[6]);
            s1 += (v[1] + v[3]) + (v[5] + v[7]);
        }
        for (; r + 4 < r1; r += 8) {
            s0 += in[r * cols + j];
            s1 += in[(r + 4) * cols + j];
        }
        if (r < r1) s0 += in[r * cols + j];
    }
    sh[rl][c] = s0 + s1;
    __syncthreads();
    if (rl == 0 && j < cols) {
        float v = ((sh[0][c] + sh[1][c]) + (sh[2][c] + sh[3][c])) * scale;
        if (bias) v += bias[j % bmod];
        if (act == 1) v = fmaxf(v, 0.f);
        else if (act == 2) v = 1.f / (1.f + expf(-v));
        out[(long)blockIdx.y * cols + j] = v;
    }
}

template <int QB>
__global__ __launch_bounds__(256) void reduce_slabs_kernel(const f32x4* __restrict__ in, f32x4* __restrict__ out, int rows, long quads) {
    constexpr int RL = 256 / QB;
    __shared__ f32x4 sh[RL][QB];
    const int cq = threadIdx.x % QB, rl = threadIdx.x / QB;
    const long q = (long)blockIdx.x * QB + cq;
    f32x4 s = {0.f, 0.f, 0.f, 0.f};
    if (q < quads) {
        const f32x4* src = in + q;
        int r = rl;
        for (; r + 7 * RL < rows; r += 8 * RL) {
            f32x4 v[8];
#pragma unroll
            for (int u = 0; u < 8; ++u) v[u] = src[(long)(r + u * RL) * quads];
            s += ((v[0] + v[1]) + (v[2] + v[3])) + ((v[4] + v[5]) + (v[6] + v[7]));
        }
        for (; r < rows; r += RL) s += src[(long)r * quads];
    }
    sh[rl][cq] = s;
    __syncthreads();
    if (rl == 0 && q < quads) {
        f32x4 t = sh[0][cq];
#pragma unroll
        for (int w = 1; w < RL; ++w) t += sh[w][cq];
        out[q] = t;
    }
}

template <int QB>
__global__ __launch_bounds__(256) void reduce_rows_q_kernel(const f32x4* __restrict__ in, f32x4* __restrict__ out, long rows, long quads,
                                                            long rows_per_split, const f32x4* __restrict__ in2, f32x4* __restrict__ out2) {
    constexpr int RL = 256 / QB;
    __shared__ f32x4 sh[RL][QB];
    if (blockIdx.z == 1) { in = in2; out = out2; }
    const int cq = threadIdx.x % QB, rl = threadIdx.x / QB;
    const long q = (long)blockIdx.x * QB + cq;
    const long r0 = (long)blockIdx.y * rows_per_split, r1 = min(rows, r0 + rows_per_split);
    f32x4 s = {0.f, 0.f, 0.f, 0.f};
    if (q < quads) {
        const f32x4* src = in + q;
        long r = r0 + rl;
        for (; r + 7 * RL < r1; r += 8 * RL) {
            f32x4 v[8];
#pragma unroll
            for (int u = 0; u < 8; ++u) v[u] = src[(r + u * RL) * quads];
            s += ((v[0] + v[1]) + (v[2] + v[3])) + ((v[4] + v[5]) + (v[6] + v[7]));
        }
        for (; r < r1; r += RL) s += src[r * quads];
    }
    sh[rl][cq] = s;
    __syncthreads();
    if (rl == 0 && q < quads) {
        f32x4 t = sh[0][cq];
#pragma unroll
        for (int w = 1; w < RL; ++w) t += sh[w][cq];
        out[(long)blockIdx.y * quads + q] = t;
    }
}

template <bool SQ>
__global__ __launch_bounds__(256) void partial_sum_kernel(const float* __restrict__ a, long n, float* __restrict__ part) {
    __shared__ float sh[4];
    float s = 0.f;
    const long n4 = n >> 2;
    const f32x4* a4 = reinterpret_cast<const f32x4*>(a);
    for (long i = (long)blockIdx.x * 256 + threadIdx.x; i < n4; i += (long)gridDim.x * 256) {
        const f32x4 v = a4[i];
        s += SQ ? (v[0] * v[0] + v[1] * v[1]) + (v[2] * v[2] + v[3] * v[3]) : (v[0] + v[1]) + (v[2] + v[3]);
    }
    if (blockIdx.x == 0 && threadIdx.x < (n & 3)) {
        const float v = a[(n4 << 2) + threadIdx.x];
        s += SQ ? v * v : v;
    }
    s = block_sum(s, sh);
    if (threadIdx.x == 0) part[blockIdx.x] = s;
}
__global__ __launch_bounds__(256) void final_sum_kernel(const float* __restrict__ part, int np, float scale, float* out) {
    __shared__ float sh[4];
    float s = 0.f;
    for (int i = threadIdx.x; i < np; i += 256) s += part[i];
    s = block_sum(s, sh);
    if (threadIdx.x == 0) out[0] = s * scale;
}

__global__ __launch_bounds__(256) void softmax_ce_kernel(const float* __restrict__ logits, const int32_t* __restrict__ labels,
                                                         float* __restrict__ loss_rows, float* __restrict__ dlogits,
                                                         int c, int ld, float gscale) {
    __shared__ float sh[4];
    const int row = blockIdx.x;
    const float* z = logits + (long)row * ld;
    float* d = dlogits + (long)row * ld;
    float mx = -INFINITY;
    for (int j = threadIdx.x; j < c; j += 256) mx = fmaxf(mx, z[j]);
    mx = block_max(mx, sh);
    float s = 0.f;
    for (int j = threadIdx.x; j < c; j += 256) s += expf(z[j] - mx);
    s = block_sum(s, sh);
    const int yl = labels[row];
    const bool bad = (unsigned)yl >= (unsigned)c;
    const int y = bad ? 0 : yl;
    const float inv = 1.f / s;
    for (int j = threadIdx.x; j < ld; j += 256) {
        float g = 0.f;
        if (j < c) g = (expf(z[j] - mx) * inv - (j == y ? 1.f : 0.f)) * gscale;
        d[j] = (bad && j < c) ? NAN : g;
    }
    if (threadIdx.x == 0) loss_rows[row] = bad ? NAN : logf(s) - (z[y] - mx);
}

template <int NPT>
__global__ __launch_bounds__(256) void softmax_ce_reg_kernel(const float* __restrict__ logits, const int32_t* __restrict__ labels,
                                                             float* __restrict__ loss_rows, float* __restrict__ dlogits,
                                                             int c, int ld, float gscale) {
    __shared__ float sh[4];
    const int row = blockIdx.x;
    const float* z = logits + (long)row * ld;
    float* d = dlogits + (long)row * ld;
    float v[NPT];
    float mx = -INFINITY;
#pragma unroll
    for (int i = 0; i < NPT; ++i) {
        const int j = threadIdx.x + 256 * i;
        v[i] = j < c ? z[j] : -INFINITY;
        mx = fmaxf(mx, v[i]);
    }
    mx = block_max(mx, sh);
    float s = 0.f;
#pragma unroll
    for (int i = 0; i < NPT; ++i) {
        const int j = threadIdx.x + 256 * i;
        v[i] = expf(v[i] - mx);
        if (j < c) s += v[i];
    }
    s = block_sum(s, sh);
    const int yl = labels[row];
    const bool bad = (unsigned)yl >= (unsigned)c;
    const int y = bad ? 0 : yl;
    const float inv = 1.f / s;
#pragma unroll
    for (int i = 0; i < NPT; ++i) {
// ... 835 lines not shown
    extern __shared__ float cfs[];
    const int a = blockIdx.x;
    for (int b = threadIdx.x; b < n; b += 256) cfs[b] = coef[(long)a * n + b] + coef[(long)b * n + a];
    __syncthreads();
    for (int k = threadIdx.x; k < d; k += 256) {
        float g = 0.f;
        const float fa = feat[(long)a * d + k];
        for (int b = 0; b < n; ++b) {
            const float cf = cfs[b];
            if (cf != 0.f) g += cf * (fa - feat[(long)b * d + k]);
        }
        dfeat[(long)a * d + k] = g;
    }
}

__global__ __launch_bounds__(256) void momentum_kernel(float* __restrict__ w, float* __restrict__ acc, const float* __restrict__ g,
                                                       long n, float lr, float mom, float wd, float gs) {
    const long n4 = n >> 2;
    f32x4* w4 = reinterpret_cast<f32x4*>(w);
    f32x4* a4 = reinterpret_cast<f32x4*>(acc);
    const f32x4* g4 = reinterpret_cast<const f32x4*>(g);
    for (long i = (long)blockIdx.x * 256 + threadIdx.x; i < n4; i += (long)gridDim.x * 256) {
        f32x4 wv = w4[i], av = a4[i];
        const f32x4 gv = g4[i];
        av = mom * av + (gs * gv + wd * wv);
        wv = wv - lr * av;
        a4[i] = av;
        w4[i] = wv;
    }
    if (blockIdx.x == 0 && threadIdx.x < (n & 3)) {
        const long i = (n4 << 2) + threadIdx.x;
        const float av = mom * acc[i] + (gs * g[i] + wd * w[i]);
        acc[i] = av;
        w[i] = w[i] - lr * av;
    }
}
__global__ __launch_bounds__(256) void adam_kernel(float* __restrict__ w, float* __restrict__ m, float* __restrict__ v,
                                                   const float* __restrict__ g, long n, float lr_t, float b1, float b2,
                                                   float eps, float wd, float gs) {
    for (long i = (long)blockIdx.x * 256 + threadIdx.x; i < n; i += (long)gridDim.x * 256) {
        const float gv = gs * g[i] + wd * w[i];
        const float mv = b1 * m[i] + (1.f - b1) * gv;
        const float vv = b2 * v[i] + (1.f - b2) * gv * gv;
        m[i] = mv;
        v[i] = vv;
        w[i] = w[i] - lr_t * mv / (sqrtf(vv) + eps);
    }
}

inline int grid_for(long n, int per) { long b = (n + per - 1) / per; return (int)(b < 1 ? 1 : (b > 4096 ? 4096 : b)); }

}

hipError_t k_conv_first_fwd(const float* x, const float* w, const float* bias, const float* alpha, float* z, float* y,
                            unsigned short* z16, unsigned short* y16,
                            int n, int h, int wd, int cin, int cout, int ho, int wo, int stride, int pt, int pl, hipStream_t st) {
    const long ngrp = (long)n * ho * ((wo + 31) / 32);
    long nb = (ngrp + 3) / 4;
    if (nb > 4096) nb = 4096;
    const int blocks = (int)nb;
#define FTE_CF(CI_, CO_) hipLaunchKernelGGL((conv_first_fwd_kernel<CI_, CO_>), dim3(blocks), dim3(256), 0, st, x, w, bias, alpha, z, y, z16, y16, n, h, wd, ho, wo, stride, pt, pl)
    if (cin == 1 && cout == 64) FTE_CF(1, 64);
    else if (cin == 3 && cout == 64) FTE_CF(3, 64);
    else if (cin == 1 && cout == 32) FTE_CF(1, 32);
    else if (cin == 3 && cout == 32) FTE_CF(3, 32);
    else return hipErrorInvalidValue;
#undef FTE_CF
    return hipGetLastError();
}
int k_conv_first_wgrad_blocks(long npix) { long b = (npix + 511) / 512; return (int)(b > 2048 ? 2048 : (b < 1 ? 1 : b)); }
hipError_t k_conv_first_wgrad(const float* x, const float* dz, const unsigned short* dz16, float* part, int n, int h, int wd, int cin, int cout, int ho, int wo,
                              int stride, int pt, int pl, int blocks, hipStream_t st) {
    const long nrows = (long)n * ho;
    const long rpb = (nrows + blocks - 1) / blocks;
#define FTE_CW(CI_, CO_) hipLaunchKernelGGL((conv_first_wgrad_kernel<CI_, CO_>), dim3(blocks), dim3(256), 0, st, x, dz, dz16, part, n, h, wd, ho, wo, stride, pt, pl, rpb)
    if (cin == 1 && cout == 64) FTE_CW(1, 64);
    else if (cin == 3 && cout == 64) FTE_CW(3, 64);
    else if (cin == 1 && cout == 32) FTE_CW(1, 32);
    else if (cin == 3 && cout == 32) FTE_CW(3, 32);
    else return hipErrorInvalidValue;
#undef FTE_CW
    return hipGetLastError();
}
hipError_t k_reduce_rows2(const float* in, float* out, const float* in2, float* out2, const float* bias, int bmod, long rows, long cols,
                          int fold, float scale, float* scratch, hipStream_t st, int act) {
    rows *= fold;
    cols /= fold;
    static const bool slabs_off = getenv("FTE_REDUCE_SLABS") && atoi(getenv("FTE_REDUCE_SLABS")) == 0;
    if (!slabs_off && !act && !in2 && !bias && scale == 1.f && rows >= 2 && rows < (1 << 20) && cols >= 4096 && cols % 4 == 0 &&
        (reinterpret_cast<uintptr_t>(in) | reinterpret_cast<uintptr_t>(out)) % 16 == 0) {
        const long quads = cols / 4;
        if (quads / 64 >= 1024 || rows < 32)
            hipLaunchKernelGGL(reduce_slabs_kernel<64>, dim3((unsigned)((quads + 63) / 64)), dim3(256), 0, st, reinterpret_cast<const f32x4*>(in),
                               reinterpret_cast<f32x4*>(out), (int)rows, quads);
        else
            hipLaunchKernelGGL(reduce_slabs_kernel<16>, dim3((unsigned)((quads + 15) / 16)), dim3(256), 0, st, reinterpret_cast<const f32x4*>(in),
                               reinterpret_cast<f32x4*>(out), (int)rows, quads);
        return hipGetLastError();
    }
    const unsigned nz = in2 ? 2 : 1;
    static const bool rq_off = getenv("FTE_REDUCE_ROWS_Q") && atoi(getenv("FTE_REDUCE_ROWS_Q")) == 0;
    if (!rq_off && !act && scratch && !bias && scale == 1.f && rows >= 32 && cols % 4 == 0 && cols <= 1024 &&
        (reinterpret_cast<uintptr_t>(in) | reinterpret_cast<uintptr_t>(out) | reinterpret_cast<uintptr_t>(in2) | reinterpret_cast<uintptr_t>(out2) |
         reinterpret_cast<uintptr_t>(scratch)) % 16 == 0) {
        const long quads = cols / 4;
        const int QB = quads >= 64 ? 64 : 16, RL = 256 / QB;
        const long qb = (quads + QB - 1) / QB;
        long rs = 1024 / (qb * nz);
        if (rs > rows / (8L * RL)) rs = rows / (8L * RL);
        if (rs * cols * nz > REDUCE_SCRATCH_FLOATS) rs = REDUCE_SCRATCH_FLOATS / (cols * nz);
        if (rs < 1 || rows < 256) rs = 1;
        const long rps = (rows + rs - 1) / rs;
        rs = (rows + rps - 1) / rps;
        f32x4* s1 = reinterpret_cast<f32x4*>(scratch);
        f32x4* s2 = s1 + rs * quads;
#define FTE_RQ(QB_, GY_, IN_, OUT_, ROWS_, RPS_, IN2_, OUT2_) hipLaunchKernelGGL((reduce_rows_q_kernel<QB_>), dim3((unsigned)qb, (unsigned)(GY_), nz), dim3(256), 0, st, \
            reinterpret_cast<const f32x4*>(IN_), reinterpret_cast<f32x4*>(OUT_), (long)(ROWS_), quads, (long)(RPS_), reinterpret_cast<const f32x4*>(IN2_), reinterpret_cast<f32x4*>(OUT2_))
        if (rs == 1) {
            if (QB == 64) FTE_RQ(64, 1, in, out, rows, rows, in2, out2); else FTE_RQ(16, 1, in, out, rows, rows, in2, out2);
            return hipGetLastError();
        }
        if (QB == 64) { FTE_RQ(64, rs, in, s1, rows, rps, in2, s2); FTE_RQ(64, 1, s1, out, rs, rs, s2, out2); }
        else { FTE_RQ(16, rs, in, s1, rows, rps, in2, s2); FTE_RQ(16, 1, s1, out, rs, rs, s2, out2); }
#undef FTE_RQ
        return hipGetLastError();
    }
    const long cb = (cols + 63) / 64;
    long rs = 1;
    if (scratch && cb < 512 && rows >= 64) {
        rs = 1;
        while (rs * rs < rows) ++rs;
        if (rs < 256 / cb) rs = 256 / cb;
        if (rs > 1024 / cb) rs = 1024 / cb;
        if (rs > rows / 16) rs = rows / 16;
        if (rs * cols * nz > REDUCE_SCRATCH_FLOATS) rs = REDUCE_SCRATCH_FLOATS / (cols * nz);
        if (rs < 1) rs = 1;
    }
    if (rs == 1) {
        hipLaunchKernelGGL(reduce_rows_kernel, dim3((unsigned)cb, 1, nz), dim3(256), 0, st, in, out, bias, bmod, rows, cols, rows, scale, in2, out2, act);
        return hipGetLastError();
    }
    const long rps = (rows + rs - 1) / rs;
    rs = (rows + rps - 1) / rps;
    float* scratch2 = scratch + rs * cols;
    hipLaunchKernelGGL(reduce_rows_kernel, dim3((unsigned)cb, (unsigned)rs, nz), dim3(256), 0, st, in, scratch, (const float*)nullptr, 1, rows, cols, rps, 1.f,
                       in2, scratch2, 0);
    hipLaunchKernelGGL(reduce_rows_kernel, dim3((unsigned)cb, 1, nz), dim3(256), 0, st, (const float*)scratch, out, bias, bmod, rs, cols, rs, scale,
                       (const float*)scratch2, out2, act);
    return hipGetLastError();
}
hipError_t k_reduce_rows(const float* in, float* out, const float* bias, int bmod, long rows, long cols, int fold, float scale,
                         float* scratch, hipStream_t st, int act) {
    return k_reduce_rows2(in, out, nullptr, nullptr, bias, bmod, rows, cols, fold, scale, scratch, st, act);
}
hipError_t k_sum(const float* a, long n, float scale, float* out, float* ws, bool sq, hipStream_t st) {
    const int nb = grid_for(n, 256 * 4 * 8) > 1024 ? 1024 : grid_for(n, 256 * 4 * 8);
    if (sq) hipLaunchKernelGGL(partial_sum_kernel<true>, dim3(nb), dim3(256), 0, st, a, n, ws);
    else hipLaunchKernelGGL(partial_sum_kernel<false>, dim3(nb), dim3(256), 0, st, a, n, ws);
    hipLaunchKernelGGL(final_sum_kernel, dim3(1), dim3(256), 0, st, ws, nb, scale, out);
    return hipGetLastError();
}
hipError_t k_softmax_ce(const float* logits, const int32_t* labels, float* loss_rows, float* dlogits, int n, int c, int ld, float gs, hipStream_t st) {
    if (ld <= 256 * 8) hipLaunchKernelGGL(softmax_ce_reg_kernel<8>, dim3(n), dim3(256), 0, st, logits, labels, loss_rows, dlogits, c, ld, gs);
    else if (ld <= 256 * 48) hipLaunchKernelGGL(softmax_ce_reg_kernel<48>, dim3(n), dim3(256), 0, st, logits, labels, loss_rows, dlogits, c, ld, gs);
    else hipLaunchKernelGGL(softmax_ce_kernel, dim3(n), dim3(256), 0, st, logits, labels, loss_rows, dlogits, c, ld, gs);
    return hipGetLastError();
}
namespace {
__global__ __launch_bounds__(256) void to_bf16_kernel(const float* __restrict__ x, unsigned short* __restrict__ y, long n4) {
    for (long i = (long)blockIdx.x * 256 + threadIdx.x; i < n4; i += (long)gridDim.x * 256) {
        const f32x4 v = *reinterpret_cast<const f32x4*>(x + i * 4);
        unsigned short o[4];
#pragma unroll
        for (int e = 0; e < 4; ++e) o[e] = __builtin_bit_cast(unsigned short, (__bf16)v[e]);
        *reinterpret_cast<uint2*>(y + i * 4) = make_uint2(o[0] | ((unsigned)o[1] << 16), o[2] | ((unsigned)o[3] << 16));
    }
}
__global__ __launch_bounds__(256) void pack_weights_kernel(const float* __restrict__ w, unsigned short* __restrict__ w16,
                                                           unsigned short* __restrict__ w16t, int taps, int cin, int cout) {
    const long total = (long)taps * cin * cout;
    for (long i = (long)blockIdx.x * 256 + threadIdx.x; i < total; i += (long)gridDim.x * 256) {
        const unsigned short v = __builtin_bit_cast(unsigned short, (__bf16)w[i]);
        if (w16) w16[i] = v;
        if (w16t) {
            const int co = (int)(i % cout);
            const long t2 = i / cout;
            const int ci = (int)(t2 % cin), tap = (int)(t2 / cin);
            w16t[((long)tap * cout + co) * cin + ci] = v;
        }
    }
}
typedef float f32x4k __attribute__((ext_vector_type(4)));
__global__ __launch_bounds__(256) void pack_weights_table_kernel(const float* __restrict__ params, unsigned short* __restrict__ w16t,
                                                                 const int* __restrict__ table, int nconv, long total4, int transposed) {
    __shared__ int tb[64 * 6];
    for (int i = threadIdx.x; i < nconv * 6; i += 256) tb[i] = table[i];
    __syncthreads();
    for (long i = (long)blockIdx.x * 256 + threadIdx.x; i < total4; i += (long)gridDim.x * 256) {
        int lo = 0, hi = nconv - 1;
        while (lo < hi) {
            const int mid = (lo + hi + 1) >> 1;
            if ((long)tb[mid * 6 + 5] <= i) lo = mid; else hi = mid - 1;
        }
        const int* d = tb + lo * 6;
        const int cin = d[3], cout = d[4];
        const long j = (i - d[5]) * 4;
        if (!transposed) {
            const f32x4k v = *reinterpret_cast<const f32x4k*>(params + d[0] + j);
            *reinterpret_cast<uint2*>(w16t + d[1] + j) = make_uint2(
                __builtin_bit_cast(unsigned short, (__bf16)v[0]) | ((unsigned)__builtin_bit_cast(unsigned short, (__bf16)v[1]) << 16),
                __builtin_bit_cast(unsigned short, (__bf16)v[2]) | ((unsigned)__builtin_bit_cast(unsigned short, (__bf16)v[3]) << 16));
            continue;
        }
        const int ci = (int)(j % cin);
        const long t2 = j / cin;
        const int co = (int)(t2 % cout), tap = (int)(t2 / cout);
        const float* src = params + d[0] + ((long)tap * cin + ci) * cout + co;
        unsigned short o[4];
#pragma unroll
        for (int e = 0; e < 4; ++e) o[e] = __builtin_bit_cast(unsigned short, (__bf16)src[(long)e * cout]);
        *reinterpret_cast<uint2*>(w16t + d[1] + j) = make_uint2(o[0] | ((unsigned)o[1] << 16), o[2] | ((unsigned)o[3] << 16));
    }
}
__global__ __launch_bounds__(256) void pack_weights_tiles_kernel(const float* __restrict__ params, unsigned short* __restrict__ w16t,
                                                                 const int* __restrict__ table, int nconv) {
    __shared__ int tb[64 * 6];
    __shared__ unsigned short tile[64][68];
    for (int i = threadIdx.x; i < nconv * 6; i += 256) tb[i] = table[i];
    __syncthreads();
    const int tid = threadIdx.x;
    for (long t = blockIdx.x;; t += gridDim.x) {
// ... 622 lines not shown
```

tf_face_toolbox_amd/csrc/wino.h:

```cpp
#pragma once
#include <hip/hip_runtime.h>
#include <stddef.h>

struct WinoGeom {
    int n, h, w, th, tw;
    long M;
    int MB;
};
WinoGeom wino_geom(int n, int h, int w);

inline size_t wino_pack_floats(long rows, int c) { return (size_t)((rows + 63) / 64) * 64 * (size_t)c * 16; }

hipError_t wino_transform_tiles(const float* x, float* pack, int n, int h, int w, int c, int mode, hipStream_t st, bool small = false,
                                const float* alpha = nullptr);
hipError_t wino_transform_filter(const float* w, float* pack, int cin, int cout, int dgrad, hipStream_t st);

struct WinoMMParams {
    const float* V;
    const float* U;
    int K, N;
    WinoGeom g;
    float* Y; float* Z; const float* R; const float* bias; const float* alpha;
    const float* ADD; float* RAW; const float* Zin; float* DZ; float* PA; float* PB;
    int amod;
};
hipError_t wino_mm(const WinoMMParams& p, int epi, hipStream_t st);
bool wino_lean_enabled();

int wino_wgrad_splits(int cin, int cout);
hipError_t wino_wgrad(const float* V, const float* dz, float* slabs, float* dw, const WinoGeom& g, int cin, int cout, hipStream_t st);

void wino_set_algo(int a);
int wino_get_algo();
```

tf_face_toolbox_amd/csrc/wino.hip:

```cpp
#include <hip/hip_runtime.h>
#include <stdint.h>
#include <stdio.h>
#include <stdlib.h>
#include <string.h>

#include <atomic>

#include "igemm.h"
#include "igemm_dev.h"
#include "wino.h"

#ifdef FTE_WINO_STAMP
__device__ unsigned long long* g_wino_stamp = nullptr;
extern "C" int fte_debug_set_wino_stamp(void* buf) {
    return (int)hipMemcpyToSymbol(HIP_SYMBOL(g_wino_stamp), &buf, sizeof(buf));
}
#endif

namespace {

using namespace igemm_dev;

typedef __attribute__((address_space(3))) void lds_void;
__device__ __forceinline__ void dma16(const __amdgpu_buffer_rsrc_t& r, char* lds, unsigned voff, unsigned soff) {
// ... 24 lines not shown
    int n = 0, ty = 0, tx = 0;
    const bool mv = m < M;
    if (mv) { n = (int)(m / tpi); const int rem = (int)(m - (long)n * tpi); ty = rem / TW; tx = rem - ty * TW; }
    const int y0 = 2 * ty - (MODE == 0 ? 1 : 0), x0 = 2 * tx - (MODE == 0 ? 1 : 0);
    const __amdgpu_buffer_rsrc_t rs = __builtin_amdgcn_make_buffer_rsrc(const_cast<float*>(x), 0, x_bytes, 0x00020000);
    const unsigned choff = (unsigned)(blockIdx.y * 32 + c4 * 4) * 4u;
    f32x4 d[P][P];
#pragma unroll
    for (int i = 0; i < P; ++i)
#pragma unroll
        for (int j = 0; j < P; ++j) {
            const int yy = y0 + i, xx = x0 + j;
            const bool ok = mv && yy >= 0 && yy < H && xx >= 0 && xx < W;
            d[i][j] = __builtin_bit_cast(f32x4, __builtin_amdgcn_raw_buffer_load_b128(rs, ok ? (unsigned)(((n * H + yy) * W + xx) * C) * 4u + choff : OOB, 0, 0));
        }
    if constexpr (ACT) {
        const f32x4 al4 = *reinterpret_cast<const f32x4*>(alpha + blockIdx.y * 32 + c4 * 4);
#pragma unroll
        for (int i = 0; i < P; ++i)
#pragma unroll
            for (int j = 0; j < P; ++j)
#pragma unroll
                for (int e = 0; e < 4; ++e) d[i][j][e] = d[i][j][e] > 0.f ? d[i][j][e] : al4[e] * d[i][j][e];
    }
    const int ks = blockIdx.y * 4 + (c4 >> 1), sw = (r >> 4) & 1;
    float* o = pack + (((size_t)mb * KS + ks) * 16 * 64 + r) * 8 + (((c4 & 1) ^ sw) << 2);
    if constexpr (MODE == 0) {
#pragma unroll
        for (int i = 0; i < 4; ++i) {
            f32x4 w[4];
#pragma unroll
            for (int j = 0; j < 4; ++j)
                w[j] = i == 0 ? d[0][j] - d[2][j] : i == 1 ? d[1][j] + d[2][j] : i == 2 ? d[2][j] - d[1][j] : d[1][j] - d[3][j];
            *reinterpret_cast<f32x4*>(o + (size_t)(4 * i + 0) * 512) = w[0] - w[2];
            *reinterpret_cast<f32x4*>(o + (size_t)(4 * i + 1) * 512) = w[1] + w[2];
            *reinterpret_cast<f32x4*>(o + (size_t)(4 * i + 2) * 512) = w[2] - w[1];
            *reinterpret_cast<f32x4*>(o + (size_t)(4 * i + 3) * 512) = w[1] - w[3];
        }
    } else {
#pragma unroll
        for (int i = 0; i < 4; ++i) {
            f32x4 u[2];
#pragma unroll
            for (int j = 0; j < 2; ++j)
                u[j] = i == 0 ? d[0][j] : i == 1 ? 0.5f * (d[0][j] + d[1][j]) : i == 2 ? 0.5f * (d[0][j] - d[1][j]) : d[1][j];
            *reinterpret_cast<f32x4*>(o + (size_t)(4 * i + 0) * 512) = u[0];
            *reinterpret_cast<f32x4*>(o + (size_t)(4 * i + 1) * 512) = 0.5f * (u[0] + u[1]);
            *reinterpret_cast<f32x4*>(o + (size_t)(4 * i + 2) * 512) = 0.5f * (u[0] - u[1]);
            *reinterpret_cast<f32x4*>(o + (size_t)(4 * i + 3) * 512) = u[1];
        }
    }
}

__global__ __launch_bounds__(256) void wino_filter_kernel(const float* __restrict__ w, float* __restrict__ pack, int cin, int cout, int dgrad) {
    const int K = dgrad ? cout : cin, NR = dgrad ? cin : cout;
    const int idx = blockIdx.x * 256 + threadIdx.x;
    if (idx >= K * NR) return;
    int k, row;
    if (dgrad) { k = idx % K; row = idx / K; }
    else { row = idx % NR; k = idx / NR; }
    float g[3][3];
#pragma unroll
    for (int a = 0; a < 3; ++a)
#pragma unroll
        for (int b = 0; b < 3; ++b)
            g[a][b] = dgrad ? w[(((2 - a) * 3 + (2 - b)) * (size_t)cin + row) * cout + k] : w[((a * 3 + b) * (size_t)cin + k) * cout + row];
    float p[4][3];
#pragma unroll
    for (int b = 0; b < 3; ++b) {
        p[0][b] = g[0][b];
        p[1][b] = 0.5f * (g[0][b] + g[1][b] + g[2][b]);
        p[2][b] = 0.5f * (g[0][b] - g[1][b] + g[2][b]);
        p[3][b] = g[2][b];
    }
    const int KS = K >> 3, rb = row >> 6, r = row & 63, c8 = k & 7;
    float* o = pack + ((((size_t)rb * KS + (k >> 3)) * 16) * 64 + r) * 8 + (((c8 >> 2) ^ ((r >> 4) & 1)) << 2) + (c8 & 3);
#pragma unroll
    for (int i = 0; i < 4; ++i) {
        o[(size_t)(4 * i + 0) * 512] = p[i][0];
        o[(size_t)(4 * i + 1) * 512] = 0.5f * (p[i][0] + p[i][1] + p[i][2]);
        o[(size_t)(4 * i + 2) * 512] = 0.5f * (p[i][0] - p[i][1] + p[i][2]);
        o[(size_t)(4 * i + 3) * 512] = p[i][2];
    }
}

template <int EPI, int NWN, bool LEAN>
__global__ __launch_bounds__(256 * NWN, 1) void wino_mm_kernel(const WinoMMParams p, int NBX, int GRP, int vid0, int nvirt) {
    constexpr int NW = 4 * NWN;
    constexpr int NST = LEAN ? 8 : 16;
    constexpr int BSTG = NWN * (SLAB_B / 2);
    constexpr int STG = SLAB_B + BSTG;
    extern __shared__ __attribute__((aligned(16))) char wsm[];
    const int tid = threadIdx.x;
    const int lane = tid & 63;
    const int wid = __builtin_amdgcn_readfirstlane(tid >> 6);
    const int q = wid & 1, mi = (wid >> 1) & 1, ni = NWN == 2 ? wid >> 2 : 0;
    const int hb = NWN == 2 ? 0 : (int)(blockIdx.x & 1);
    const int li = lane & 31, lh = lane >> 5;
    const int KS = p.K >> 3, NB = p.N >> 6;
    auto decode = [&](int vid, int& mb, int& nb) -> bool {
        if (GRP > 0) {
            const int xcd = vid & 7, slot = vid >> 3;
            const int grp = xcd % GRP, cls = xcd / GRP, C = 8 / GRP;
            mb = (slot / NBX) * C + cls;
            nb = grp * NBX + slot % NBX;
        } else {
            mb = vid / NB; nb = vid - mb * NB;
        }
        return mb < p.g.MB;
    };
    auto next_valid = [&](int vid, int& mb, int& nb) -> int {
        if constexpr (NWN == 2) {
            for (; vid < nvirt; vid += (int)gridDim.x)
                if (decode(vid, mb, nb)) return vid;
        } else if (vid == vid0) {
            int c = 0;
            for (int v = vid0; v < nvirt; ++v)
                if (decode(v, mb, nb)) {
                    if (c == (int)(blockIdx.x >> 1)) return v;
                    ++c;
                }
        }
        return nvirt;
    };
    const unsigned voff = (unsigned)lane * 16u;
    auto issue = [&](int mb, int nb, int s, int stage) {
        const __amdgpu_buffer_rsrc_t rsA = __builtin_amdgcn_make_buffer_rsrc(const_cast<float*>(p.V + (size_t)mb * KS * SLAB_F), 0, (unsigned)KS * SLAB_B, 0x00020000);
        const __amdgpu_buffer_rsrc_t rsB = __builtin_amdgcn_make_buffer_rsrc(const_cast<float*>(p.U + (size_t)nb * KS * SLAB_F), 0, (unsigned)KS * SLAB_B, 0x00020000);
        char* base = wsm + stage * STG;
#pragma unroll
        for (int i = 0; i < 32 / NW; ++i) {
            const int piece = wid + NW * i;
            dma16(rsA, base + piece * 1024, voff, (unsigned)(s * SLAB_B + piece * 1024));
        }
#pragma unroll
        for (int i = 0; i < 4; ++i) {
            const int piece = wid + NW * i;
            dma16(rsB, base + SLAB_B + piece * 1024, voff, (unsigned)(s * SLAB_B + (NWN == 2 ? piece : 2 * piece + hb) * 1024));
        }
    };
    constexpr int BPL = NWN * 1024;
    const int a_off = ((8 * q) * 64 + 32 * mi + li) * 32 + ((lh ^ ((li >> 4) & 1)) << 4);
    const int b_off = (8 * q) * BPL + (32 * ni + li) * 32 + ((lh ^ ((li >> 4) & 1)) << 4);
    float* xb = reinterpret_cast<float*>(wsm + STG);
    int* rowpix = reinterpret_cast<int*>(wsm + 2 * STG);
    int* rowflag = rowpix + 64;
    float* red = reinterpret_cast<float*>(rowflag + 64);

    int mb = 0, nb = 0;
    int vid = next_valid(NWN == 2 ? vid0 + (int)blockIdx.x : vid0, mb, nb);
    if (vid >= nvirt) return;
    f32x4 xa[4], xb4[4], ya[4], yb[4];
    auto read_frags = [&](int stage, int half, f32x4 (&fa)[4], f32x4 (&fb)[4], int t) {
        const char* As = wsm + stage * STG;
        fa[t] = *reinterpret_cast<const f32x4*>(As + a_off + (4 * half + t) * 2048);
        fb[t] = *reinterpret_cast<const f32x4*>(As + SLAB_B + b_off + (4 * half + t) * BPL);
    };
    auto dma_piece = [&](const __amdgpu_buffer_rsrc_t& rsA, const __amdgpu_buffer_rsrc_t& rsB, int s, int stage, int i) {
        char* base = wsm + stage * STG;
        if constexpr (NWN == 2) {
            const int piece = wid + 8 * (i >> 1);
            if (i & 1) dma16(rsB, base + SLAB_B + piece * 1024, voff, (unsigned)(s * SLAB_B + piece * 1024));
            else dma16(rsA, base + piece * 1024, voff, (unsigned)(s * SLAB_B + piece * 1024));
        } else {
            const int piece = wid + 4 * (i & 7);
            if (i >= 8) dma16(rsB, base + SLAB_B + piece * 1024, voff, (unsigned)(s * SLAB_B + (2 * piece + hb) * 1024));
// ... 335 lines not shown
            }
            __builtin_amdgcn_sched_barrier(0);
        });
    }
    asm volatile("s_waitcnt vmcnt(0)" ::: "memory");
    const size_t plane = (size_t)cin * cout;
#pragma unroll
    for (int t = 0; t < 2; ++t)
#pragma unroll
        for (int i = 0; i < 2; ++i)
#pragma unroll
            for (int k = 0; k < 2; ++k) {
                float* o = slabs + ((size_t)split * 16 + 2 * wid + t) * plane + (size_t)(cb * 64 + 32 * i + 4 * lh) * cout + nb * 64 + 32 * k + li;
#pragma unroll
                for (int r = 0; r < 16; ++r) o[(size_t)((r & 3) + 8 * (r >> 2)) * cout] = acc[t][i][k][r];
            }
}

constexpr int WF_E = 32;
__global__ __launch_bounds__(16 * WF_E) void wino_wgrad_finish_kernel(const float* __restrict__ slabs, float* __restrict__ dw, int S, long plane) {
    __shared__ float sums[16][WF_E + 1];
    const int t = threadIdx.x / WF_E, e = threadIdx.x % WF_E;
    const long idx = (long)blockIdx.x * WF_E + e;
    float acc = 0.f;
    if (idx < plane) {
        const float* src = slabs + (size_t)t * plane + idx;
#pragma unroll 8
        for (int s = 0; s < S; ++s) acc += src[(size_t)s * 16 * plane];
    }
    sums[t][e] = acc;
    __syncthreads();
    if (t != 0 || idx >= plane) return;
    float m[16];
#pragma unroll
    for (int k = 0; k < 16; ++k) m[k] = sums[k][e];
#pragma unroll
    for (int k = 0; k < 16; ++k) {
        const float sc = (((k >> 2) == 1 || (k >> 2) == 2) ? 0.5f : 1.f) * (((k & 3) == 1 || (k & 3) == 2) ? 0.5f : 1.f);
        m[k] *= sc;
    }
    float pr[3][4];
#pragma unroll
    for (int j = 0; j < 4; ++j) {
        pr[0][j] = m[0 + j] + m[4 + j] + m[8 + j];
        pr[1][j] = m[4 + j] - m[8 + j];
        pr[2][j] = m[4 + j] + m[8 + j] - m[12 + j];
    }
#pragma unroll
    for (int a = 0; a < 3; ++a) {
        dw[(size_t)(a * 3 + 0) * plane + idx] = pr[a][0] + pr[a][1] + pr[a][2];
        dw[(size_t)(a * 3 + 1) * plane + idx] = pr[a][1] - pr[a][2];
        dw[(size_t)(a * 3 + 2) * plane + idx] = pr[a][1] + pr[a][2] - pr[a][3];
    }
}

int g_algo = -1;

}

WinoGeom wino_geom(int n, int h, int w) {
    WinoGeom g;
    g.n = n; g.h = h; g.w = w; g.th = (h + 1) / 2; g.tw = (w + 1) / 2;
    g.M = (long)n * g.th * g.tw;
    g.MB = (int)((g.M + 63) / 64);
    return g;
}

hipError_t wino_transform_tiles(const float* x, float* pack, int n, int h, int w, int c, int mode, hipStream_t st, bool small, const float* alpha) {
    if (c % 32 || (alpha && mode != 0)) return hipErrorInvalidValue;
    const WinoGeom g = wino_geom(n, h, w);
    const size_t xb = (size_t)n * h * w * c * 4;
    if (xb >= ((size_t)1 << 31)) return hipErrorInvalidValue;
    const dim3 grid(8 * ((g.MB + 7) / 8) * (small ? 2 : 1), c / 32);
    if (mode == 0 && small && alpha) hipLaunchKernelGGL((wino_tiles_kernel<0, 256, true>), grid, dim3(256), 0, st, x, alpha, pack, h, w, c, g.th, g.tw, g.M, g.MB, (unsigned)xb);
    else if (mode == 0 && alpha) hipLaunchKernelGGL((wino_tiles_kernel<0, 512, true>), grid, dim3(512), 0, st, x, alpha, pack, h, w, c, g.th, g.tw, g.M, g.MB, (unsigned)xb);
    else if (mode == 0 && small) hipLaunchKernelGGL((wino_tiles_kernel<0, 256, false>), grid, dim3(256), 0, st, x, alpha, pack, h, w, c, g.th, g.tw, g.M, g.MB, (unsigned)xb);
    else if (mode == 0) hipLaunchKernelGGL((wino_tiles_kernel<0, 512, false>), grid, dim3(512), 0, st, x, alpha, pack, h, w, c, g.th, g.tw, g.M, g.MB, (unsigned)xb);
    else hipLaunchKernelGGL((wino_tiles_kernel<1, 512, false>), grid, dim3(512), 0, st, x, alpha, pack, h, w, c, g.th, g.tw, g.M, g.MB, (unsigned)xb);
    return hipGetLastError();
}

hipError_t wino_transform_filter(const float* w, float* pack, int cin, int cout, int dgrad, hipStream_t st) {
    if (cin % 64 || cout % 64) return hipErrorInvalidValue;
    const int total = cin * cout;
    hipLaunchKernelGGL(wino_filter_kernel, dim3((total + 255) / 256), dim3(256), 0, st, w, pack, cin, cout, dgrad);
    return hipGetLastError();
}

namespace {
template <int EPI, int NWN, bool LEAN>
hipError_t wino_mm_launch(const WinoMMParams& p, int NBX, int GRP, int vid0, int vid1, int grid, int tiles, hipStream_t st) {
    constexpr int NW = 4 * NWN;
    const size_t lds = 2 * ((size_t)SLAB_B + NWN * (SLAB_B / 2)) + 2560 + (size_t)NW * 16 * 36 * 4;
    static std::atomic<unsigned> attr{0u};
    int dev = 0;
    (void)hipGetDevice(&dev);
    const unsigned bit = 1u << (dev & 31);
    if (!(attr.load(std::memory_order_acquire) & bit)) {
        hipError_t e = hipFuncSetAttribute(reinterpret_cast<const void*>(wino_mm_kernel<EPI, NWN, LEAN>), hipFuncAttributeMaxDynamicSharedMemorySize, (int)lds);
        if (e != hipSuccess) return e;
        attr.fetch_or(bit, std::memory_order_release);
    }
    const int sig[5] = {AL_MK, BL_NK, EPI, 8, 1};
    const double frac = (double)tiles / ((double)p.g.MB * (p.N / 64));
    const double flops = 2.0 * 16.0 * (double)tiles * 64.0 * 64.0 * p.K;
    const double bytes = frac * ((double)wino_pack_floats(p.g.M, p.K) * 4.0 + 16.0 * p.N * p.K * 4.0 + (double)p.g.n * p.g.h * p.g.w * p.N * 4.0 *
                                 (EPI == EPI_FWD ? (1 + (p.Z ? 1 : 0) + (p.R ? 1 : 0)) : (1 + (p.ADD ? 1 : 0) + (p.RAW ? 1 : 0) + (p.Zin ? 1 : 0))));
    const int h = igemm_prof_begin(sig, (int)((long)tiles * 64 / (p.N / 64)), p.N, 16 * p.K, flops, bytes, st);
    hipLaunchKernelGGL((wino_mm_kernel<EPI, NWN, LEAN>), dim3(grid), dim3(256 * NWN), lds, st, p, NBX, GRP, vid0, vid1);
    static const char* const names[2][2][2] = {{{"wino_mm_kernel<0,1>", "wino_mm_kernel<0,1,1>"}, {"wino_mm_kernel<0,2>", "wino_mm_kernel<0,2,1>"}},
                                               {{"wino_mm_kernel<1,1>", "wino_mm_kernel<1,1,1>"}, {"wino_mm_kernel<1,2>", "wino_mm_kernel<1,2,1>"}}};
    igemm_prof_end(h, names[EPI == EPI_FWD ? 0 : 1][NWN - 1][LEAN ? 1 : 0], st);
    return hipGetLastError();
}
template <int NWN>
hipError_t wino_mm_pick(const WinoMMParams& p, int epi, bool lean, int NBX, int GRP, int vid0, int vid1, int grid, int tiles, hipStream_t st) {
    if (epi == EPI_FWD) return lean ? wino_mm_launch<EPI_FWD, NWN, true>(p, NBX, GRP, vid0, vid1, grid, tiles, st)
                                    : wino_mm_launch<EPI_FWD, NWN, false>(p, NBX, GRP, vid0, vid1, grid, tiles, st);
    return lean ? wino_mm_launch<EPI_DGRAD, NWN, true>(p, NBX, GRP, vid0, vid1, grid, tiles, st)
                : wino_mm_launch<EPI_DGRAD, NWN, false>(p, NBX, GRP, vid0, vid1, grid, tiles, st);
}
}

bool wino_lean_enabled() {
    const char* e = getenv("FTE_WINO_LEAN");
    return !e || strcmp(e, "0") != 0;
}

hipError_t wino_mm(const WinoMMParams& p, int epi, hipStream_t st) {
    if (p.K % 64 || p.N % 64 || p.g.MB <= 0) return hipErrorInvalidValue;
    if ((size_t)p.g.n * p.g.h * p.g.w * p.N >= ((size_t)1 << 31)) return hipErrorInvalidValue;
    if (epi == EPI_FWD ? (!p.Y && !p.Z) : !p.DZ) return hipErrorInvalidValue;
    const bool lean = wino_lean_enabled() && (epi == EPI_FWD ? (!p.R && !p.Y) : (!p.ADD && !p.RAW));
    const int NB = p.N / 64;
    int NBX = NB < 2 ? NB : 2, GRP = NB / NBX;
    static const int plain = getenv("FTE_WINO_PLAIN_ORDER") ? atoi(getenv("FTE_WINO_PLAIN_ORDER")) : 0;
    int nvirt;
    if (plain || NB % NBX || 8 % GRP) { GRP = 0; nvirt = p.g.MB * NB; }
    else { const int C = 8 / GRP; nvirt = 8 * ((p.g.MB + C - 1) / C) * NBX; }
    static int cus = 0;
    if (!cus) {
        int dev = 0;
        hipDeviceProp_t prop;
        if (hipGetDevice(&dev) != hipSuccess || hipGetDeviceProperties(&prop, dev) != hipSuccess) return hipErrorInvalidDevice;
        cus = prop.multiProcessorCount > 8 ? prop.multiProcessorCount / 8 * 8 : 8;
    }
    const int grid = nvirt < cus ? (nvirt + 7) / 8 * 8 : cus;
    static const int halves = getenv("FTE_WINO_HALF_TILES") ? atoi(getenv("FTE_WINO_HALF_TILES")) : 1;
    auto valid = [&](int vid) {
        if (GRP > 0) { const int xcd = vid & 7, slot = vid >> 3, cls = xcd / GRP, C = 8 / GRP; return (slot / NBX) * C + cls < p.g.MB; }
        return vid / NB < p.g.MB;
    };
    const int rounds = (nvirt + grid - 1) / grid, last = grid * (rounds - 1);
    int L = 0;
    for (int v = last; v < nvirt; ++v) L += valid(v) ? 1 : 0;
    const int total = p.g.MB * NB;
    int tail_base = nvirt;
    if (halves && L > 0 && 2 * L <= cus && (rounds == 1 || halves == 2)) tail_base = last;
    hipError_t e = hipSuccess;
    if (tail_base > 0) {
        e = wino_mm_pick<2>(p, epi, lean, NBX, GRP, 0, tail_base, grid, total - (tail_base < nvirt ? L : 0), st);
        if (e != hipSuccess) return e;
    }
    if (tail_base < nvirt) e = wino_mm_pick<1>(p, epi, lean, NBX, GRP, tail_base, nvirt, 2 * L, L, st);
    return e;
}

int wino_wgrad_splits(int cin, int cout) {
// ... 48 lines not shown
```

tf_face_toolbox_amd/nets/sphere.py:

```python
import math
import os
from collections import OrderedDict

import torch

from .. import _lib, heads
from ..loss import sample_size
from .net_base import NORMALISED_HEADS, Network, adaface_params, adaface_state, margin_params, side_stream

NUM_BLOCKS = (1, 2, 4, 1)
EMBED = 512


def same_pads(in_size, k, stride):
    out = -(-in_size // stride)
    total = max((out - 1) * stride + k - in_size, 0)
    return out, total // 2, total - total // 2


class _Conv(object):
    __slots__ = ('name', 'stage', 'stride', 'has_bias', 'second', 'cin', 'cout', 'hin', 'win', 'hout', 'wout')


class Variable(object):

    def __init__(self, name, kind, ref_shape, offset, size):
        self.name, self.kind, self.ref_shape, self.offset, self.size = name, kind, tuple(ref_shape), offset, size

    def __repr__(self):
        return '<Variable %s %s>' % (self.name, self.ref_shape)


def _stream():
    return torch.cuda.current_stream().cuda_stream


class SphereNet(Network):
    head = 'softmax'

    def __init__(self, weight_decay=0.0005, data_format='NCHW', name='SphereNet', seed=0):
        super(SphereNet, self).__init__(weight_decay, data_format, name)
        self.num_outputs = [64, 128, 256, 512]
        self.seed = seed
        self.built = False
        self.bf16_copies = os.environ.get('FTE_BF16_COPIES', '1') != '0'
        self.tower_scale = 1.0
        self.global_step = 0
        self.sub_centers = 1
        self._act_n = None

    def _conv_specs(self, h, w, cin):
        specs = []
        for si, nb in enumerate(NUM_BLOCKS):
            stage = '%s/conv%d' % (self.name, si + 1)
            lst = [(stage + '/Conv', 2, True, None)]
            for b in range(nb):
                blk = stage + ('/resBlock' if nb == 1 else '/Repeat/resBlock_%d' % (b + 1))
                lst += [(blk + '/Conv', 1, False, 0), (blk + '/Conv_1', 1, False, 1)]
            for nm, stride, has_bias, second in lst:
                c = _Conv()
                c.name, c.stage, c.stride, c.has_bias, c.second = nm, si, stride, has_bias, second
                c.cin, c.cout, c.hin, c.win = cin, self.num_outputs[si], h, w
                c.hout, c.wout = same_pads(h, 3, stride)[0], same_pads(w, 3, stride)[0]
                specs.append(c)
                h, w, cin = c.hout, c.wout, c.cout
        return specs

    def build(self, height, width, channels, num_classes, device='cuda'):
        _lib.load()
        self.device = torch.device(device)
        self.in_hwc = (height, width, channels)
        self.num_classes = int(num_classes)
        self.cpad = (self.num_classes + 127) // 128 * 128
        self.convs = self._conv_specs(height, width, channels)
        last = self.convs[-1]
        self.feat_hwc = (last.hout, last.wout, last.cout)
        self.fin = last.hout * last.wout * last.cout
        small, big = [], []
        for c in self.convs:
            if c.has_bias:
                small.append((c.name + '/biases', 'bias', (c.cout,), c.cout))
            small.append((c.name + '/alpha', 'alpha', (c.cout,), c.cout))
            big.append((c.name + '/weights', 'conv_w', (3, 3, c.cin, c.cout), 9 * c.cin * c.cout))
        small.append((self.name + '/fully_connected/biases', 'fc_b', (EMBED,), EMBED))
        big.append((self.name + '/fully_connected/weights', 'fc_w', (self.fin, EMBED), self.fin * EMBED))
        K = self.sub_centers
        big.append(('classifier/fc_classifier/weights', 'cls_w', (EMBED, K * self.num_classes), EMBED * K * self.cpad))
        self.variables = OrderedDict()
        off = 0
        for nm, kind, shape, size in small + big:
            self.variables[nm] = Variable(nm, kind, shape, off, size)
            off += (size + 3) // 4 * 4
        self.small_end = self.variables[big[0][0]].offset
        self.cls_start = self.variables['classifier/fc_classifier/weights'].offset
        self.fc_start = self.variables[self.name + '/fully_connected/weights'].offset
        self._stage_first = [min(self.variables[c.name + '/weights'].offset for c in self.convs if c.stage == st_)
                             for st_ in sorted(set(c.stage for c in self.convs))]
        self.arena_size = off
        dev = self.device
        self.params = torch.zeros(off, dtype=torch.float32, device=dev)
        self.grads = torch.zeros(off + 4, dtype=torch.float32, device=dev)
        self.loss_slots = self.grads[off:off + 4]
        self.state = self._make_state()
        self._init_params()
        self.built = True
        return self

    def _make_state(self):
        return OrderedDict()

    def view(self, name, arena=None):
        v = self.variables[name]
        a = self.params if arena is None else arena
        return a[v.offset:v.offset + v.size]

    def _init_params(self):
        g = torch.Generator().manual_seed(self.seed)
        for c in self.convs:
            if c.has_bias:
                lim = (6.0 / (9 * c.cin + 9 * c.cout)) ** 0.5
                w = (torch.rand(3, 3, c.cin, c.cout, generator=g) * 2 - 1) * lim
            else:
                w = torch.randn(3, 3, c.cin, c.cout, generator=g) * 0.01
            self.view(c.name + '/weights').copy_(w.reshape(-1))
            self.view(c.name + '/alpha').fill_(0.25)
        lim = (6.0 / (self.fin + EMBED)) ** 0.5
        w = (torch.rand(self.fin, EMBED, generator=g) * 2 - 1) * lim
        self.view(self.name + '/fully_connected/weights').copy_(w.reshape(-1))
        K = self.sub_centers
        wc = torch.zeros(EMBED, K, self.cpad)
        wc[:, :, :self.num_classes] = (torch.randn(EMBED, K * self.num_classes, generator=g) * 0.001).reshape(EMBED, K, self.num_classes)
        self.view('classifier/fc_classifier/weights').copy_(wc.reshape(-1))

    def _fc_perm(self, t, to_internal):
        if self.data_format == 'NHWC':
            return t
        h, w, c = self.feat_hwc
        if to_internal:
            return t.reshape(c, h, w, EMBED).permute(1, 2, 0, 3).reshape(self.fin, EMBED)
        return t.reshape(h, w, c, EMBED).permute(2, 0, 1, 3).reshape(self.fin, EMBED)

    def get_variable(self, name, arena=None):
        if name in self.state:
            return self.state[name].clone()
        v = self.variables[name]
        t = self.view(name, arena)
        if v.kind == 'cls_w':
            return t.reshape(EMBED, self.sub_centers, self.cpad)[:, :, :self.num_classes].reshape(v.ref_shape).clone()
        if v.kind == 'fc_w':
            return self._fc_perm(t.reshape(self.fin, EMBED), False).contiguous()
        return t.reshape(v.ref_shape).clone()

    def set_variable(self, name, value, arena=None):
        if name in self.state:
            self.state[name].copy_(torch.as_tensor(value, dtype=torch.float32).reshape(self.state[name].shape))
            return
        v = self.variables[name]
        t = torch.as_tensor(value, dtype=torch.float32).to(self.device)
        assert tuple(t.shape) == v.ref_shape, (name, tuple(t.shape), v.ref_shape)
        if v.kind == 'cls_w':
            buf = torch.zeros(EMBED, self.sub_centers, self.cpad, device=self.device)
            buf[:, :, :self.num_classes] = t.reshape(EMBED, self.sub_centers, self.num_classes)
            t = buf
        elif v.kind == 'fc_w':
            t = self._fc_perm(t, True)
        self.view(name, arena).copy_(t.reshape(-1))

    def load_params(self, params):
        for k, val in params.items():
            self.set_variable(k, val)

    def _storage16(self):
        return _lib.bf16_storage()

    def _alloc_acts(self, n):
        s16 = self._storage16()
        key = (s16, _lib.get_mfma_dtype(), _lib.query('fte_get_conv_algo'))
        if self._act_n == n and getattr(self, '_act_key', None) == key:
            return
        self._act_key = key
        dev = self.device
        f32 = dict(dtype=torch.float32, device=dev)
        i16 = dict(dtype=torch.int16, device=dev)
        self._act_s16 = s16
        self.y16 = None
        self.z, self.y = [], []
        last = len(self.convs) - 1
        for l, c in enumerate(self.convs):
            keep32 = not s16 or l == last
            self.z.append(torch.empty(n, c.hout, c.wout, c.cout, **f32) if keep32 else None)
            self.y.append(torch.empty(n, c.hout, c.wout, c.cout, **f32) if keep32 else None)
        self.lean = [False] * len(self.convs)
        if s16:
            self.z16 = [torch.empty(n, c.hout, c.wout, c.cout, **i16) for c in self.convs]
        self.emb = torch.empty(n, EMBED, **f32)
        hw = self._head_width()
        self.s_raw = torch.empty(n, hw, **f32)
        self.G = torch.empty(n, hw, **f32)
        self.logits_buf = torch.empty(n, hw // self.sub_centers, **f32) if self.head == 'asoftmax' or self.head in NORMALISED_HEADS else self.s_raw
        self.loss_rows = torch.empty(n, **f32)
        self.xn = torch.empty(n, **f32)
        self.wn = torch.empty(hw, **f32)
        self.rowcoef = torch.empty(n, **f32)
        self.colcoef = torch.empty(hw, **f32)
        self.demb = torch.empty(n, EMBED, **f32)
        self.bwd = {}
        for si in range(4):
            c = [q for q in self.convs if q.stage == si][0]
            shp = (n, c.hout, c.wout, c.cout)
            if s16:
                one = [torch.empty(shp, **f32)] if si == 3 else []
                self.bwd[si] = dict(dz=one, raw=list(one and [torch.empty(shp, **f32)]), dzi=0, rawi=0,
                                    dz16=[torch.empty(shp, **i16) for _ in range(self._dz_buffers())],
                                    raw16=[torch.empty(shp, **i16), torch.empty(shp, **i16)])
            else:
                self.bwd[si] = dict(dz=[torch.empty(shp, **f32) for _ in range(self._dz_buffers())],
                                    raw=[torch.empty(shp, **f32), torch.empty(shp, **f32)], dzi=0, rawi=0)
        need = 4096
        q = _lib.query
        self.vpack = [None] * len(self.convs)
        if not s16 and os.environ.get('FTE_WINO_KEEP', '1') != '0':
            for l, c in enumerate(self.convs):
                if l > 0 and c.stride == 1 and q('fte_conv3x3_algo', n, c.hin, c.win, c.cin, c.cout, 1, 0) == 1 \
                        and q('fte_conv3x3_algo', n, c.hin, c.win, c.cin, c.cout, 1, 2) == 1:
                    self.vpack[l] = torch.empty(q('fte_wino_pack_bytes', n, c.hin, c.win, c.cin) // 4, **f32)
            for l, c in enumerate(self.convs):
                if c.second == 1 and self.vpack[l] is not None and self.vpack[l - 1] is not None:
                    self.lean[l] = True
                    self.y[l - 1] = None
        for c in self.convs[1:]:
            need = max(need, q('fte_conv3x3_fwd_ws_bytes', n, c.hin, c.win, c.cin, c.cout, c.stride),
                       q('fte_conv3x3_wgrad_ws_bytes', n, c.hin, c.win, c.cin, c.cout, c.stride),
                       q('fte_conv3x3_dgrad_ws_bytes', n, c.hin, c.win, c.cin, c.cout, c.stride))
        c0 = self.convs[0]
        need = max(need, q('fte_conv3x3_first_wgrad_ws_bytes', n, c0.hin, c0.win, c0.cin, c0.cout, c0.stride),
                   q('fte_gemm_ws_bytes', n, EMBED, self.fin), q('fte_gemm_ws_bytes', n, hw, EMBED))
        self.ws = torch.empty((need + 3) // 4 + 1024, **f32)
        self.ws_bytes = self.ws.numel() * 4
        self.side = side_stream(self.device) if os.environ.get('FTE_SIDE_STREAM', '1') != '0' else None
        self.ws_side = torch.empty_like(self.ws) if self.side is not None else self.ws
        self._alloc_head(n)
        self._act_n = n
        self.y16 = None

    def _y_buf(self, l):
        if self.y[l] is None and not self._storage16():
            c = self.convs[l]
            self.y[l] = torch.empty(self._act_n, c.hout, c.wout, c.cout, dtype=torch.float32, device=self.device)
        return self.y[l]

    def _head_width(self):
        return self.sub_centers * self.cpad

    def _alloc_head(self, n):
        """further head buffers of a subclass, sized with the activations"""

    def _use_copies(self):
        return self.bf16_copies and _lib.get_mfma_dtype() == 'bf16'

    def _alloc_copies(self):
        if self.y16 is not None and self.y16[0].shape[0] == self._act_n:
            return
        i16 = dict(dtype=torch.int16, device=self.device)
        n = self._act_n
        self.y16 = [torch.empty(n, c.hout, c.wout, c.cout, **i16) for c in self.convs]
        for si in range(4):
            b = self.bwd[si]
            if 'dz16' not in b:
                b['dz16'] = [torch.empty(b['dz'][0].shape, **i16) for _ in b['dz']]
        if getattr(self, 'packs', None) is None:
            from ._packs import FilterPacks
            self.packs = FilterPacks([(c.name, self.variables[c.name + '/weights'].offset, 3, c.cin, c.cout) for c in self.convs[1:]], self.device)
            self.w16, self.w16t = self.packs.w16, self.packs.w16t

    def _pack_weights(self, st):
        self.packs.refresh(self.params, st)

    def prelu(self, x, name='prelu'):
        raise RuntimeError('PReLU is fused into the conv epilogue (fte_conv3x3_fwd); it is not a separate op here.')

    def _check_images(self, images):
        if not (isinstance(images, torch.Tensor) and images.is_cuda and images.dtype == torch.float32):
            raise TypeError('images must be a float32 CUDA tensor in NHWC (data.py:275-279 layout)')
        if not images.is_contiguous():
            images = images.contiguous()
        return images

    def _fwd_split(self, n, copies):
        env = os.environ.get('FTE_FWD_HALVES', 'auto')
        if env == '0' or copies or self.side is None or n < 2 or getattr(self, 'one_stream', False):
            return 0
        key = (n, getattr(self, '_act_key', None))
        if getattr(self, '_split_key', None) != key:
            q = _lib.query
            gran = 1
            for l, c in enumerate(self.convs):
                if self.vpack[l] is not None:
                    tpi = ((c.hin + 1) // 2) * ((c.win + 1) // 2)
                    gran = max(gran, 64 // math.gcd(64, tpi))
            a = int(os.environ.get('FTE_FWD_SPLIT', (n // 2) // gran * gran))
            ok, any_w = 0 < a < n, False
            for l, c in enumerate(self.convs):
                if l == 0 or c.stride != 1 or not ok:
                    continue
                algo = [q('fte_conv3x3_algo', m, c.hin, c.win, c.cin, c.cout, 1, 0) for m in (n, a, n - a)]
                any_w = any_w or algo[0] == 1
                if algo[1] != algo[0] or algo[2] != algo[0]:
                    ok = False
                if self.vpack[l] is not None and (a * ((c.hin + 1) // 2) * ((c.win + 1) // 2)) % 64:
                    ok = False
            self._split_key, self._split = key, (a if ok and any_w else 0)
        if not self._split:
            return 0
        return self._split if env == '1' or n >= int(os.environ.get('FTE_FWD_HALVES_MIN', '128')) else 0

    def _fwd_halves(self, n, copies):
        return self._fwd_split(n, copies) > 0

    def backbone(self, inputs, is_training=False, reuse=None):
        x = self._check_images(inputs)
        n, h, w, ch = x.shape
        if not self.built:
            raise RuntimeError('call build() or forward(..., num_classes=) with is_training=True first')
        assert (h, w, ch) == self.in_hwc, ((h, w, ch), self.in_hwc)
        self._alloc_acts(n)
        st = _stream()
        call = _lib.call
        keep = is_training
        self._images = x
        s16 = self._storage16()
        copies = self._use_copies() or s16
        self._copies_live = copies and keep
        self._s16_live = s16 and keep
        self._vpack_live = keep and not copies
        lean_live = self._vpack_live and os.environ.get('FTE_WINO_LEAN', '1') != '0'
        self._lean_live = lean_live
        nl = len(self.convs)
        if not lean_live:
            for l in range(nl):
                self._y_buf(l)
        if copies:
            self._alloc_copies()
            self._pack_weights(st)
        def part_pack(l, c, lo, hi, m):
            vp = self.vpack[l]
            if m != n:
                per = ((c.hin + 1) // 2) * ((c.win + 1) // 2) * c.cin * 16
                vp = vp[lo * per:hi * per] if hi < n else vp[lo * per:]
            return vp

        def layer(l, c, lo, hi, ws, st):
            m = hi - lo
            wv = self.view(c.name + '/weights')
            bv = self.view(c.name + '/biases') if c.has_bias else None
            av = self.view(c.name + '/alpha')
            zz = self.z[l][lo:hi] if keep and self.z[l] is not None else None
            if s16:
                z16 = self.z16[l][lo:hi] if keep else None
                if l == 0:
                    call('fte_conv3x3_first_fwd_s16', x[lo:hi], wv, bv, av, z16, self.y16[0][lo:hi], m, c.hin, c.win, c.cin, c.cout, c.stride, st)
                else:
                    call('fte_conv2d_fwd_s16', self.y16[l - 1][lo:hi], self.w16t[c.name], bv, av, self.y16[l - 2][lo:hi] if c.second == 1 else None,
                         z16, self.y16[l][lo:hi], zz, self.y[l][lo:hi] if self.y[l] is not None else None, m, c.hin, c.win, c.cin, c.cout, 3, c.stride,
                         ws, self.ws_bytes, st)
            elif lean_live and self.lean[l]:
                p = self.convs[l - 1]
                call('fte_conv3x3_fwd_keep_act', self.z[l - 1][lo:hi], self.view(p.name + '/alpha'), wv, bv, av, self.y[l - 2][lo:hi], zz,
                     self.y[l][lo:hi], m, c.hin, c.win, c.cin, c.cout, c.stride, part_pack(l, c, lo, hi, m), ws, self.ws_bytes, st)
            elif lean_live and l + 1 < nl and self.lean[l + 1]:
                call('fte_conv3x3_fwd_keep_act', self.y[l - 1][lo:hi], None, wv, bv, av, None, zz, None,
                     m, c.hin, c.win, c.cin, c.cout, c.stride, part_pack(l, c, lo, hi, m), ws, self.ws_bytes, st)
            elif l == 0:
                call('fte_conv3x3_first_fwd', x[lo:hi], wv, bv, av, zz, self.y[0][lo:hi], m, c.hin, c.win, c.cin, c.cout, c.stride, st)
                if copies:
                    call('fte_to_bf16', self.y[0][lo:hi], self.y16[0][lo:hi], self.y[0][lo:hi].numel(), st)
            else:
                res = self.y[l - 2][lo:hi] if c.second == 1 else None
                if copies:
                    call('fte_conv2d_fwd16', self.y16[l - 1][lo:hi], self.w16t[c.name], bv, av, res, zz, self._y_buf(l)[lo:hi], self.y16[l][lo:hi],
                         m, c.hin, c.win, c.cin, c.cout, 3, c.stride, ws, self.ws_bytes, st)
                elif keep and self.vpack[l] is not None:
                    call('fte_conv3x3_fwd_keep', self._y_buf(l - 1)[lo:hi], wv, bv, av, res, zz, self._y_buf(l)[lo:hi],
                         m, c.hin, c.win, c.cin, c.cout, c.stride, part_pack(l, c, lo, hi, m), ws, self.ws_bytes, st)
                else:
                    call('fte_conv3x3_fwd', self._y_buf(l - 1)[lo:hi], wv, bv, av, res, zz, self._y_buf(l)[lo:hi],
                         m, c.hin, c.win, c.cin, c.cout, c.stride, ws, self.ws_bytes, st)

        split = self._fwd_split(n, copies)
        if split:
            main, side = torch.cuda.current_stream(), self.side
            side.wait_stream(main)
            for l, c in enumerate(self.convs):
                layer(l, c, 0, split, self.ws, st)
                layer(l, c, split, n, self.ws_side, side.cuda_stream)
            main.wait_stream(side)
        else:
            for l, c in enumerate(self.convs):
                layer(l, c, 0, n, self.ws, st)
        call('fte_gemm_nn', self.y[-1], self.view(self.name + '/fully_connected/weights'),
             self.view(self.name + '/fully_connected/biases'), self.emb, n, EMBED, self.fin, self.ws, self.ws_bytes, st)
        return self.emb

    def _head_cols(self):
        cls = 'classifier/fc_classifier/weights'
        return self.view(cls), self.view(cls, self.grads), self.num_classes, self.cpad

    def _classifier_raw(self, n):
        W, _, _, ld = self._head_cols()
        _lib.call('fte_gemm_nn', self.emb, W, None, self.s_raw, n, self.sub_centers * ld, EMBED, self.ws, self.ws_bytes, _stream())

    def _ensure_built(self, images, num_classes):
        if not self.built:
            n, h, w, ch = images.shape
            self.build(h, w, ch, num_classes, images.device)
        else:
            assert num_classes == self.num_classes, 'num_classes changed after the variables were created'

    def forward(self, images, num_classes=None, is_training=True):
        if is_training:
            assert num_classes is not None, 'num_classes must be given when is_training=True'
            self._ensure_built(images, num_classes)
            self.backbone(images, is_training=True)
            self._classifier_raw(images.shape[0])
            return {'logits': self.s_raw[:, :self.num_classes]}
        return self._eval_features(images)

    def _eval_features(self, images):
        images = self._check_images(images)
        n, h, w, ch = images.shape
        st = _stream()
        out = torch.empty(n, EMBED, dtype=torch.float32, device=images.device)
        f1 = self.backbone(images, is_training=False)
        _lib.call('fte_axpby', 0.5, f1, 0.0, f1, out, n * EMBED, st)
        flipped = torch.empty_like(images)
        _lib.call('fte_flip_width', images, flipped, n, h, w, ch, st)
        f2 = self.backbone(flipped, is_training=False)
        _lib.call('fte_axpby', 1.0, out, 0.5, f2, out, n * EMBED, st)
        return out

    def _grad_scale(self, n):
        return self.tower_scale / n

    def _finish_losses(self, n):
        st = _stream()
        _lib.call('fte_sum', self.loss_rows, n, self.tower_scale / n, self.loss_slots[0:1], self.ws, self.ws_bytes, st)
        nreg = self.arena_size - self.small_end
        _lib.call('fte_sumsq', self.params[self.small_end:], nreg, 0.5 * self.weight_decay * self.tower_scale,
                  self.loss_slots[1:2], self.ws, self.ws_bytes, st)

    def loss_function(self, scope, labels, **logits):
        n = labels.shape[0]
        labels = heads.check_labels(labels)
        self._labels = labels
        _lib.call('fte_softmax_ce_fwd_bwd', self.s_raw, labels, self.loss_rows, self.G, n, self.num_classes, self.cpad,
                  self._grad_scale(n), _stream())
        self._finish_losses(n)
        return [self.loss_slots[0], self.loss_slots[1]], ['cross_entropy', 'reg_loss'], OrderedDict()

    def _head_backward(self, n, st):
        W, dW, _, ld = self._head_cols()
        ld *= self.sub_centers
        norm = self.head != 'softmax'
        heads.classifier_dw(self, self.emb, W, dW, n, EMBED, ld, self.ws, self.ws_bytes, st, norm)
        self._scatter_dw(st)
        heads.classifier_dx(self, self.emb, W, self.demb, n, EMBED, ld, self.ws, self.ws_bytes, st, norm)

    def _scatter_dw(self, st):
        """what a head on a subset of the columns does with its dW before the input side runs; nothing for all columns"""

    def backward_head(self):
        n = self._act_n
        st = _stream()
        call = _lib.call
        g = self.grads
        self._head_backward(n, st)
        fcw = self.name + '/fully_connected/weights'
        call('fte_reduce_rows', self.demb, self.view(self.name + '/fully_connected/biases', g), None, 1, n, EMBED, 1, 1.0, st)
        call('fte_gemm_tn', self.y[-1], self.demb, self.view(fcw, g), n, EMBED, self.fin, self.ws, self.ws_bytes, st)

    def backward(self):
        for stage in self.backward_stages():
            stage()

    def backward_stages(self):
        it = self._body_walk()
        return [self.backward_head] + [lambda it=it: next(it) for _ in range(len(self._stage_first))]

    @staticmethod
    def _dz_buffers():
        return max(2, int(os.environ.get('FTE_DZ_BUFFERS', '3')))

    def _side_stream(self, n):
        if self.side is None or getattr(self, 'one_stream', False):
            return None
        if os.environ.get('FTE_SIDE_STREAM') == '1':
            return self.side
        return self.side if (n <= 256 or _lib.get_mfma_dtype() == 'bf16' or _lib.query('fte_get_conv_algo') != 0) else None

    def backward_body(self):
        for _ in self._body_walk():
            pass

    def _body_walk(self):
        n = self._act_n
        st = _stream()
        call = _lib.call
        g = self.grads
        fcw = self.name + '/fully_connected/weights'
        L = self.convs
        last = len(L) - 1
        b4 = self.bwd[L[last].stage]
        d_out, dz_cur = b4['raw'][0], b4['dz'][0]
        b4['rawi'], b4['dzi'] = 0, 0
        call('fte_gemm_nt', self.demb, self.view(fcw), self.z[last], self.view(L[last].name + '/alpha'), L[last].cout,
             d_out, dz_cur, self.view(L[last].name + '/alpha', g), n, EMBED, self.fin, self.ws, self.ws_bytes, st)
        s16 = getattr(self, '_s16_live', False) and self._storage16()
        copies = s16 or (getattr(self, '_copies_live', False) and self._use_copies())
        dz16_cur = None
        d16_out = None
        if copies:
            dz16_cur = b4['dz16'][0]
            call('fte_to_bf16', dz_cur, dz16_cur, dz_cur.numel(), st)
        if s16:
            d16_out = b4['raw16'][0]
            call('fte_to_bf16', d_out, d16_out, d_out.numel(), st)
        trace = getattr(self, '_trace_dz', None)
        main, side = torch.cuda.current_stream(), self._side_stream(n)
        wst, wws = (side.cuda_stream, self.ws_side) if side is not None else (st, self.ws)
        readers = {}
        last_w = None
        for l in range(last, -1, -1):
            c = L[l]
            if trace is not None:
                trace[c.name] = (dz16_cur if s16 else dz_cur).clone()
            gw = self.view(c.name + '/weights', g)
            if l == 0:
                if last_w is not None:
                    main.wait_event(last_w)
                if s16:
                    call('fte_conv3x3_first_wgrad_s16', self._images, dz16_cur, gw, n, c.hin, c.win, c.cin, c.cout, c.stride,
                         self.ws, self.ws_bytes, st)
                else:
                    call('fte_conv3x3_first_wgrad', self._images, dz_cur, gw, n, c.hin, c.win, c.cin, c.cout, c.stride,
                         self.ws, self.ws_bytes, st)
                break
            if side is not None:
                side.wait_event(main.record_event())
            if copies:
                call('fte_conv2d_wgrad16', self.y16[l - 1], dz16_cur, gw, n, c.hin, c.win, c.cin, c.cout, 3, c.stride,
                     wws, self.ws_bytes, wst)
            elif getattr(self, '_vpack_live', False) and self.vpack[l] is not None:
                call('fte_conv3x3_wgrad_kept', None if getattr(self, '_lean_live', False) and self.lean[l] else self.y[l - 1], dz_cur, gw, n, c.hin, c.win, c.cin, c.cout, c.stride,
                     self.vpack[l], wws, self.ws_bytes, wst)
            else:
                call('fte_conv3x3_wgrad', self.y[l - 1], dz_cur, gw, n, c.hin, c.win, c.cin, c.cout, c.stride,
                     wws, self.ws_bytes, wst)
            if side is not None:
                last_w = readers[(dz16_cur if s16 else dz_cur).data_ptr()] = side.record_event()
            p = L[l - 1]
            bp = self.bwd[p.stage]
            if s16:
                if p.stage != c.stage:
                    bp['dzi'], bp['rawi'] = 0, 0
                    raw16_t = bp['raw16'][0]
                else:
                    bp['dzi'] = (bp['dzi'] + 1) % len(bp['dz16'])
                    raw16_t = bp['raw16'][bp['rawi'] ^ 1]
                dz16_prev = bp['dz16'][bp['dzi']]
                raw16 = raw16_t if p.second == 1 else None
                ev = readers.pop(dz16_prev.data_ptr(), None)
                if ev is not None:
                    main.wait_event(ev)
                call('fte_conv2d_dgrad_s16', dz16_cur, self.w16[c.name], d16_out if c.second == 0 else None, self.z16[l - 1],
                     self.view(p.name + '/alpha'), raw16, dz16_prev, self.view(p.name + '/alpha', g),
                     self.view(p.name + '/biases', g) if p.has_bias else None,
                     n, c.hin, c.win, c.cin, c.cout, 3, c.stride, self.ws, self.ws_bytes, st)
                if raw16 is not None:
                    d16_out = raw16
                    if p.stage == c.stage:
                        bp['rawi'] ^= 1
                dz16_cur = dz16_prev
                if p.stage != c.stage:
                    if last_w is not None:
                        main.wait_event(last_w)
                        last_w = None
                        readers.clear()
                    yield
                continue
            addin = d_out if c.second == 0 else None
            if p.stage != c.stage:
                bp['dzi'], bp['rawi'] = 0, 0
                dz_prev, raw_t = bp['dz'][0], bp['raw'][0]
            else:
                bp['dzi'] = (bp['dzi'] + 1) % len(bp['dz'])
                dz_prev = bp['dz'][bp['dzi']]
                raw_t = bp['raw'][bp['rawi'] ^ 1]
            raw = raw_t if p.second == 1 else None
            ev = readers.pop(dz_prev.data_ptr(), None)
            if ev is not None:
                main.wait_event(ev)
            if copies:
                dz16_prev = bp['dz16'][bp['dzi']]
                call('fte_conv2d_dgrad16', dz16_cur, self.w16[c.name], addin, self.z[l - 1],
                     self.view(p.name + '/alpha'), raw, dz_prev, dz16_prev, self.view(p.name + '/alpha', g),
                     self.view(p.name + '/biases', g) if p.has_bias else None,
                     n, c.hin, c.win, c.cin, c.cout, 3, c.stride, self.ws, self.ws_bytes, st)
                dz16_cur = dz16_prev
            else:
                call('fte_conv3x3_dgrad', dz_cur, self.view(c.name + '/weights'), addin, self.z[l - 1],
                     self.view(p.name + '/alpha'), raw, dz_prev, self.view(p.name + '/alpha', g),
                     self.view(p.name + '/biases', g) if p.has_bias else None,
                     n, c.hin, c.win, c.cin, c.cout, c.stride, self.ws, self.ws_bytes, st)
            if raw is not None:
                d_out = raw
                if p.stage == c.stage:
                    bp['rawi'] ^= 1
            dz_cur = dz_prev
            if p.stage != c.stage:
                if last_w is not None:
                    main.wait_event(last_w)
                    last_w = None
                    readers.clear()
                yield
        yield

    def param_list(self, is_training, trainable, scope=None):
        bb = [v for k, v in self.variables.items() if k.startswith(self.name + '/')]
        if is_training:
            return [bb, [self.variables['classifier/fc_classifier/weights']]]
        return [bb]

    def pretrained_param(self, scope=None):
        return [v for grp in self.param_list(is_training=False, trainable=False, scope=scope) for v in grp
                if self.name in v.name]

    def arena_groups(self):
        return [(0, self.small_end, False, 0), (self.small_end, self.cls_start, True, 0),
                (self.cls_start, self.arena_size, True, 1)]

    def grad_buckets(self):
        firsts = self._stage_first
        ends = firsts[1:] + [self.fc_start]
        buckets = [(self.fc_start, self.arena_size + 4)]
        for i in range(len(firsts) - 1, 0, -1):
            buckets.append((firsts[i], ends[i]))
        buckets.append((0, ends[0]))
        return buckets


class SphereNetMargin(SphereNet):
    head = 'asoftmax'
    needs_labels = True

    def __init__(self, weight_decay=0.0005, data_format='NCHW', name='SphereNet', seed=0,
                 lambda_base=1000.0, gamma=0.12, power=1.0, lambda_min=5.0):
        super(SphereNetMargin, self).__init__(weight_decay, data_format, name, seed)
        self.lambda_base, self.gamma, self.power, self.lambda_min = lambda_base, gamma, power, lambda_min

    def current_lambda(self):
        return max(self.lambda_min, self.lambda_base * (1.0 + self.gamma * self.global_step) ** (-self.power))

    def forward(self, images, labels=None, num_classes=None, is_training=True):
        if not is_training:
            return self._eval_features(images)
        assert num_classes is not None, 'num_classes must be given when is_training=True'
        assert labels is not None, 'margin nets take labels in forward (data_parallel.py:220)'
        self._ensure_built(images, num_classes)
        n = images.shape[0]
        self._check_sample(n)
        labels = heads.check_labels(labels)
        self._labels = labels
        st = _stream()
        self.backbone(images, is_training=True)
        labels, extra = self._sample_classes(labels, n, st)
        self._classifier_raw(n)
        W, _, c, ld = self._head_cols()
        heads.margin_forward(self, self.emb, W, self.s_raw, labels, self.logits_buf, self._head_spec(), n, EMBED, c, ld,
                             self._grad_scale(n), st)
        return dict({'logits': self.logits_buf[:, :c]}, **extra)

    def _check_sample(self, n):
        """a sampled-class head refuses a batch its sample cannot hold"""

    def _sample_classes(self, labels, n, st):
        return labels, {}

    def _head_spec(self):
        self.lam = self.current_lambda()
        return ('asoftmax', self.lam)

# ... 141 lines not shown
```

Before: 15360 images/sec.

## Batch Winograd filter transforms and defer dgrad bias/alpha reductions into table launches

Adds precomputed Winograd filter packs, transformed once per step in a single table-driven launch, for forward and dgrad of stride-1 3x3 convs. Dgrad partial sums for PReLU alpha and bias now go into a persistent arena. They are reduced in a few batched table launches at the end of backward instead of one reduce per layer. The aim is fewer small kernel launches and less redundant filter-transform work. In exchange it adds extra memory for the packs and parts and a more complex schedule. Filter packs are enabled only for small batches by default.

```diff
diff --git a/include/fte.h b/include/fte.h
--- a/include/fte.h
+++ b/include/fte.h
@@ -48,12 +48,31 @@
                              int n, int h, int wd, int cin, int cout, int stride, float* vpack,
                              void* ws, size_t ws_bytes, void* stream);
 
+size_t fte_wino_filter_pack_bytes(int cin, int cout);
+int fte_wino_filter_pack_blocks(int cin, int cout);
+int fte_wino_pack_filters_table(const float* params, float* packs, const int32_t* table, int nrows, int nblocks, long pack_floats, void* stream);
+int fte_conv3x3_fwd_pack(const float* x, const float* xalpha, const float* w, const float* bias, const float* alpha,
+                         const float* res, float* z, float* y,
+                         int n, int h, int wd, int cin, int cout, int stride, float* vpack, const float* upack,
+                         void* ws, size_t ws_bytes, void* stream);
+
 int fte_conv3x3_dgrad(const float* dz, const float* w, const float* addin,
                       const float* zprev, const float* alpha_prev,
                       float* raw, float* dzprev, float* dalpha_prev, float* dbias_prev,
                       int n, int h, int wd, int cin, int cout, int stride,
                       void* ws, size_t ws_bytes, void* stream);
 size_t fte_conv3x3_dgrad_ws_bytes(int n, int h, int wd, int cin, int cout, int stride);
+int fte_conv3x3_dgrad_pack(const float* dz, const float* w, const float* addin,
+                           const float* zprev, const float* alpha_prev,
+                           float* raw, float* dzprev, float* dalpha_prev, float* dbias_prev,
+                           int n, int h, int wd, int cin, int cout, int stride,
+                           const float* upack, float* parts, size_t parts_bytes,
+                           void* ws, size_t ws_bytes, void* stream);
+int fte_conv3x3_dgrad_parts_rows(int n, int h, int wd, int cin, int cout, int stride);
+size_t fte_conv3x3_dgrad_parts_bytes(int n, int h, int wd, int cin, int cout, int stride);
+int fte_reduce_rows_plan(long rows, long cols, int nmat, int* plan);
+int fte_reduce_rows_table(const float* in, float* out, float* scratch, const int32_t* table, int nrows, int blocks1, int blocks2,
+                          long out_floats, long scratch_floats, void* stream);
 
 int fte_conv3x3_wgrad(const float* x, const float* dz, float* dw,
                       int n, int h, int wd, int cin, int cout, int stride,
diff --git a/tf_face_toolbox_amd/_lib.py b/tf_face_toolbox_amd/_lib.py
--- a/tf_face_toolbox_amd/_lib.py
+++ b/tf_face_toolbox_amd/_lib.py
@@ -125,6 +125,15 @@
     'fte_conv3x3_fwd_keep': (c_int, [_P] * 7 + [c_int] * 6 + [_P, _P, c_size_t, _P]),
     'fte_conv3x3_fwd_keep_act': (c_int, [_P] * 8 + [c_int] * 6 + [_P, _P, c_size_t, _P]),
     'fte_conv3x3_wgrad_kept': (c_int, [_P] * 3 + [c_int] * 6 + [_P, _P, c_size_t, _P]),
+    'fte_wino_filter_pack_bytes': (c_size_t, [c_int] * 2),
+    'fte_wino_filter_pack_blocks': (c_int, [c_int] * 2),
+    'fte_wino_pack_filters_table': (c_int, [_P, _P, _P, c_int, c_int, c_long, _P]),
+    'fte_conv3x3_fwd_pack': (c_int, [_P] * 8 + [c_int] * 6 + [_P, _P, _P, c_size_t, _P]),
+    'fte_conv3x3_dgrad_pack': (c_int, [_P] * 9 + [c_int] * 6 + [_P, _P, c_size_t, _P, c_size_t, _P]),
+    'fte_conv3x3_dgrad_parts_rows': (c_int, [c_int] * 6),
+    'fte_conv3x3_dgrad_parts_bytes': (c_size_t, [c_int] * 6),
+    'fte_reduce_rows_plan': (c_int, [c_long, c_long, c_int, _P]),
+    'fte_reduce_rows_table': (c_int, [_P, _P, _P, _P, c_int, c_int, c_int, c_long, c_long, _P]),
     'fte_get_conv_algo': (c_int, []),
     'fte_l2_normalize_rows': (c_int, [_P] * 3 + [c_int] * 2 + [_P]),
     'fte_pair_scores': (c_int, [_P] * 4 + [c_int] * 3 + [_P]),
diff --git a/tf_face_toolbox_amd/csrc/api.hip b/tf_face_toolbox_amd/csrc/api.hip
--- a/tf_face_toolbox_amd/csrc/api.hip
+++ b/tf_face_toolbox_amd/csrc/api.hip
@@ -373,7 +373,7 @@
                            float* z, float* y, uint16_t* y16, int n, int h, int wd, int cin, int cout, int ksize, int stride,
                            void* ws, size_t ws_bytes, void* stream, const uint16_t* res16 = nullptr, uint16_t* z16 = nullptr,
                            float* stat_part = nullptr, int* stat_rows = nullptr, float* vpack = nullptr,
-                           const float* xalpha = nullptr, bool z_only_ok = false) {
+                           const float* xalpha = nullptr, bool z_only_ok = false, const float* upack = nullptr) {
     const bool z_only = z_only_ok && !y && z && vpack;
     if ((xalpha || z_only_ok) && !vpack) return FTE_EINVAL;
     if (!x || !w || (!y && !(src16 && y16) && !z_only) || n <= 0 || cin % 32 || cout % 64 || (stride != 1 && stride != 2) || (ksize != 1 && ksize != 3))
@@ -402,11 +402,12 @@
     if (!src16 && !stat_part && (y || z_only) && wino_wanted(n, h, wd, cin, cout, ksize, stride, 0)) {
         WinoWs wl = wino_ws(n, h, wd, cin, cout, 0, 0);
         if (vpack) { wl.u_off = 0; wl.total = align_up((size_t)16 * cin * cout * 4); }
-        if (ws && ws_bytes >= wl.total) {
-            if (!aligned16({x, w, bias, alpha, res, z, y, ws, vpack, xalpha})) return FTE_EINVAL;
+        if (upack) wl.total = wl.u_off;
+        if (wl.total == 0 || (ws && ws_bytes >= wl.total)) {
+            if (!aligned16({x, w, bias, alpha, res, z, y, wl.total ? ws : nullptr, vpack, xalpha, upack})) return FTE_EINVAL;
             float* V = vpack ? vpack : (float*)((char*)ws + wl.v_off);
-            float* U = (float*)((char*)ws + wl.u_off);
-            hipError_t e = wino_transform_filter((const float*)w, U, cin, cout, 0, (hipStream_t)stream);
+            const float* U = upack ? upack : (const float*)((char*)ws + wl.u_off);
+            hipError_t e = upack ? hipSuccess : wino_transform_filter((const float*)w, (float*)((char*)ws + wl.u_off), cin, cout, 0, (hipStream_t)stream);
             if (e != hipSuccess) return (int)e;
             e = wino_transform_tiles((const float*)x, V, n, h, wd, cin, 0, (hipStream_t)stream, wino_fwd_small_tiles(), xalpha);
             if (e != hipSuccess) return (int)e;
@@ -417,7 +418,7 @@
             return rc(wino_mm(q, EPI_FWD, (hipStream_t)stream));
         }
     }
-    if (vpack) return FTE_EWORKSPACE;
+    if (vpack || upack) return FTE_EWORKSPACE;
     RowPlan rp = plan_rows(p.M, p.N, p.K, ws != nullptr, false, EPI_FWD);
     if (rp.tail_mode >= 2 && ws_bytes < rp.pw_bytes) rp = plan_rows(p.M, p.N, p.K, false);
     if (stat_part) {
@@ -469,6 +470,27 @@
     if (!vpack || ((uintptr_t)vpack & 15) || (!y && !z)) return FTE_EINVAL;
     return conv2d_fwd_impl(x, w, false, bias, alpha, res, z, y, nullptr, n, h, wd, cin, cout, 3, stride, ws, ws_bytes, stream,
                            nullptr, nullptr, nullptr, nullptr, vpack, xalpha, true);
+}
+int fte_conv3x3_fwd_pack(const float* x, const float* xalpha, const float* w, const float* bias, const float* alpha, const float* res,
+                         float* z, float* y, int n, int h, int wd, int cin, int cout, int stride, float* vpack, const float* upack,
+                         void* ws, size_t ws_bytes, void* stream) {
+    if (((uintptr_t)vpack | (uintptr_t)upack) & 15) return FTE_EINVAL;
+    if (!vpack && (xalpha || !y)) return FTE_EINVAL;
+    return conv2d_fwd_impl(x, w, false, bias, alpha, res, z, y, nullptr, n, h, wd, cin, cout, 3, stride, ws, ws_bytes, stream,
+                           nullptr, nullptr, nullptr, nullptr, vpack, xalpha, vpack != nullptr, upack);
+}
+size_t fte_wino_filter_pack_bytes(int cin, int cout) {
+    if (cin <= 0 || cout <= 0 || cin % 64 || cout % 64) return 0;
+    return (size_t)16 * cin * cout * sizeof(float);
+}
+int fte_wino_filter_pack_blocks(int cin, int cout) {
+    if (cin <= 0 || cout <= 0 || cin % 64 || cout % 64) return 0;
+    return wino_filter_blocks(cin, cout);
+}
+int fte_wino_pack_filters_table(const float* params, float* packs, const int32_t* table, int nrows, int nblocks, long pack_floats, void* stream) {
+    if (!params || !packs || !table || nrows <= 0 || nrows > 64 || nblocks <= 0 || pack_floats <= 0 || (((uintptr_t)params | (uintptr_t)packs) & 15))
+        return FTE_EINVAL;
+    return rc(wino_transform_filter_table(params, packs, table, nrows, nblocks, pack_floats, (hipStream_t)stream));
 }
 int fte_conv3x3_algo(int n, int h, int wd, int cin, int cout, int stride, int op) {
     if (op < 0 || op > 2) return FTE_EINVAL;
@@ -572,7 +594,7 @@
                              const float* alpha_prev, float* raw, float* dzprev, uint16_t* dzprev16, float* dalpha_prev, float* dbias_prev,
                              int n, int h, int wd, int cin, int cout, int ksize, int stride, void* ws, size_t ws_bytes, void* stream,
                              const uint16_t* addin16 = nullptr, const uint16_t* zprev16 = nullptr, uint16_t* raw16 = nullptr,
-                             const DgradBn* bn = nullptr) {
+                             const DgradBn* bn = nullptr, const float* upack = nullptr, float* parts = nullptr, size_t parts_bytes = 0) {
     const float* zx = nullptr;
     const uint16_t* zx16 = nullptr;
     if (bn) {
@@ -591,13 +613,15 @@
     if (!src16 && !bn && dzprev && !dzprev16 && !addin16 && !zprev16 && !raw16 && wino_wanted(n, h, wd, cin, cout, ksize, stride, 1)) {
         const WinoGeom g = wino_geom(n, h, wd);
         const size_t half_w = align_up((size_t)g.MB * cin * sizeof(float));
-        const WinoWs wl = wino_ws(n, h, wd, cin, cout, 1, 2 * half_w + SCRATCH_BYTES);
+        WinoWs wl = wino_ws(n, h, wd, cin, cout, 1, parts ? 0 : 2 * half_w + SCRATCH_BYTES);
+        if (upack) wl.total = wl.u_off;
+        const bool part = zprev && (dalpha_prev || dbias_prev);
+        if (parts && part && parts_bytes < 2 * half_w) return FTE_EWORKSPACE;
         if (ws && ws_bytes >= wl.total) {
-            if (!aligned16({dz, w, addin, zprev, alpha_prev, raw, dzprev, ws})) return FTE_EINVAL;
-            const bool part = zprev && (dalpha_prev || dbias_prev);
+            if (!aligned16({dz, w, addin, zprev, alpha_prev, raw, dzprev, ws, upack, parts})) return FTE_EINVAL;
             float* V = (float*)((char*)ws + wl.v_off);
-            float* U = (float*)((char*)ws + wl.u_off);
-            hipError_t e = wino_transform_filter((const float*)w, U, cin, cout, 1, (hipStream_t)stream);
+            const float* U = upack ? upack : (const float*)((char*)ws + wl.u_off);
+            hipError_t e = upack ? hipSuccess : wino_transform_filter((const float*)w, (float*)((char*)ws + wl.u_off), cin, cout, 1, (hipStream_t)stream);
             if (e != hipSuccess) return (int)e;
             e = wino_transform_tiles((const float*)dz, V, n, h, wd, cout, 0, (hipStream_t)stream);
             if (e != hipSuccess) return (int)e;
@@ -605,10 +629,11 @@
             memset(&q, 0, sizeof(q));
             q.V = V; q.U = U; q.K = cout; q.N = cin; q.g = g;
             q.ADD = addin; q.RAW = raw; q.Zin = zprev; q.alpha = alpha_prev; q.amod = cin; q.DZ = dzprev;
-            q.PA = part ? (float*)ws : nullptr; q.PB = part ? (float*)((char*)ws + half_w) : nullptr;
+            char* pbase = parts ? (char*)parts : (char*)ws;
+            q.PA = part ? (float*)pbase : nullptr; q.PB = part ? (float*)(pbase + half_w) : nullptr;
             e = wino_mm(q, EPI_DGRAD, (hipStream_t)stream);
             if (e != hipSuccess) return (int)e;
-            if (part) {
+            if (part && !parts) {
                 float* scratch = (float*)((char*)ws + 2 * half_w);
                 if (dalpha_prev && dbias_prev) return rc(k_reduce_rows2(q.PA, dalpha_prev, q.PB, dbias_prev, nullptr, 1, g.MB, cin, 1, 1.f, scratch, (hipStream_t)stream));
                 if (dalpha_prev) return rc(k_reduce_rows(q.PA, dalpha_prev, nullptr, 1, g.MB, cin, 1, 1.f, scratch, (hipStream_t)stream));
@@ -616,7 +641,9 @@
             }
             return FTE_OK;
         }
-    }
+        if (parts) return FTE_EWORKSPACE;
+    }
+    if (upack) return FTE_EWORKSPACE;
     DgradClass cls[4];
     const int nc = dgrad_classes(n, h, wd, cin, cout, ksize, stride, cls);
     const bool merged = dgrad_mergeable(cls, nc, n, cin);
@@ -627,12 +654,14 @@
     const size_t half = align_up((size_t)rows * cin * sizeof(float));
     size_t pw_need = 0;
     for (int i = 0; i < nc && !merged; ++i) if (cls[i].rp.pw_bytes > pw_need) pw_need = cls[i].rp.pw_bytes;
-    const size_t fixed = 2 * half + SCRATCH_BYTES;
-    if ((want_part || pw_need) && (!ws || ws_bytes < fixed + pw_need)) return FTE_EWORKSPACE;
-    float* scratch = want_part ? (float*)((char*)ws + 2 * half) : nullptr;
+    const size_t fixed = parts ? 0 : 2 * half + SCRATCH_BYTES;
+    if (parts && want_part && (parts_bytes < 2 * half || ((uintptr_t)parts & 15))) return FTE_EWORKSPACE;
+    if (((want_part && !parts) || pw_need) && (!ws || ws_bytes < fixed + pw_need)) return FTE_EWORKSPACE;
+    float* scratch = want_part && !parts ? (float*)((char*)ws + 2 * half) : nullptr;
     float* pwbuf = pw_need ? (float*)((char*)ws + fixed) : nullptr;
-    float* PA = want_part ? (float*)ws : nullptr;
-    float* PB = want_part ? (float*)((char*)ws + half) : nullptr;
+    char* pbase = parts ? (char*)parts : (char*)ws;
+    float* PA = want_part ? (float*)pbase : nullptr;
+    float* PB = want_part ? (float*)(pbase + half) : nullptr;
     if (merged) {
         int order[4];
         const int tile = dgrad_merged_plan(cls, nc, n, cin, order);
@@ -691,7 +720,7 @@
     if (bn)
         return rc(l_bn_bwd_finalize(PB, PA, cin, (int)rows, (long)n * h * wd, cin, bn->gamma, bn->mean, bn->rstd, bn->dgamma, bn->dbeta,
                                     bn->coef, (hipStream_t)stream));
-    if (want_part) {
+    if (want_part && !parts) {
         if (dalpha_prev && dbias_prev) {
             hipError_t e = k_reduce_rows2(PA, dalpha_prev, PB, dbias_prev, nullptr, 1, rows, cin, 1, 1.f, scratch, (hipStream_t)stream);
             if (e != hipSuccess) return (int)e;
@@ -735,6 +764,46 @@
                       int n, int h, int wd, int cin, int cout, int stride, void* ws, size_t ws_bytes, void* stream) {
     return fte_conv2d_dgrad(dz, w, addin, zprev, alpha_prev, raw, dzprev, dalpha_prev, dbias_prev,
                             n, h, wd, cin, cout, 3, stride, ws, ws_bytes, stream);
+}
+
+int fte_conv3x3_dgrad_parts_rows(int n, int h, int wd, int cin, int cout, int stride) {
+    if (n <= 0 || cin <= 0 || cin % 64 || cout <= 0 || cout % 32 || (stride != 1 && stride != 2)) return 0;
+    if (wino_wanted(n, h, wd, cin, cout, 3, stride, 1)) return wino_geom(n, h, wd).MB;
+    DgradClass cls[4];
+    const int nc = dgrad_classes(n, h, wd, cin, cout, 3, stride, cls);
+    if (dgrad_mergeable(cls, nc, n, cin)) return (int)dgrad_merged_rows(cls, nc, n, cin);
+    long rows = 0;
+    for (int i = 0; i < nc; ++i) rows += cls[i].mtiles;
+    return (int)rows;
+}
+size_t fte_conv3x3_dgrad_parts_bytes(int n, int h, int wd, int cin, int cout, int stride) {
+    return 2 * align_up((size_t)fte_conv3x3_dgrad_parts_rows(n, h, wd, cin, cout, stride) * cin * sizeof(float));
+}
+int fte_conv3x3_dgrad_pack(const float* dz, const float* w, const float* addin, const float* zprev,
+                           const float* alpha_prev, float* raw, float* dzprev, float* dalpha_prev, float* dbias_prev,
+                           int n, int h, int wd, int cin, int cout, int stride, const float* upack, float* parts, size_t parts_bytes,
+                           void* ws, size_t ws_bytes, void* stream) {
+    if (((uintptr_t)upack | (uintptr_t)parts) & 15) return FTE_EINVAL;
+    return conv2d_dgrad_impl(dz, w, false, addin, zprev, alpha_prev, raw, dzprev, nullptr, dalpha_prev, dbias_prev,
+                             n, h, wd, cin, cout, 3, stride, ws, ws_bytes, stream, nullptr, nullptr, nullptr, nullptr, upack, parts, parts_bytes);
+}
+int fte_reduce_rows_plan(long rows, long cols, int nmat, int* plan) {
+    if (!plan || rows <= 0 || cols <= 0 || cols % 4 || (nmat != 1 && nmat != 2)) return FTE_EINVAL;
+    const ReducePlan pl = k_reduce_rows_plan(rows, cols, nmat, true, true, true, true);
+    if (pl.kind != REDUCE_SCALAR && pl.kind != REDUCE_Q16 && pl.kind != REDUCE_Q64) return FTE_EINVAL;
+    const int QB = pl.kind == REDUCE_Q64 ? 64 : 16;
+    const long cb = pl.kind == REDUCE_SCALAR ? (cols + 63) / 64 : (cols / 4 + QB - 1) / QB;
+    plan[0] = pl.kind; plan[1] = (int)pl.rs; plan[2] = (int)pl.rps;
+    plan[3] = (int)(cb * pl.rs * nmat); plan[4] = pl.rs > 1 ? (int)(cb * nmat) : 0;
+    plan[5] = pl.rs > 1 ? (int)(pl.rs * cols * nmat) : 0;
+    return FTE_OK;
+}
+int fte_reduce_rows_table(const float* in, float* out, float* scratch, const int32_t* table, int nrows, int blocks1, int blocks2,
+                          long out_floats, long scratch_floats, void* stream) {
+    if (!in || !out || !table || nrows <= 0 || nrows > 64 || blocks1 <= 0 || blocks2 < 0 || out_floats <= 0 || (blocks2 > 0 && (!scratch || scratch_floats <= 0)) ||
+        (((uintptr_t)in | (uintptr_t)out | (uintptr_t)scratch) & 15))
+        return FTE_EINVAL;
+    return rc(k_reduce_rows_table(in, out, scratch, table, nrows, blocks1, blocks2, out_floats, scratch_floats, (hipStream_t)stream));
 }
 
 namespace {
diff --git a/tf_face_toolbox_amd/csrc/kernels.h b/tf_face_toolbox_amd/csrc/kernels.h
--- a/tf_face_toolbox_amd/csrc/kernels.h
+++ b/tf_face_toolbox_amd/csrc/kernels.h
@@ -13,6 +13,11 @@
                          float* scratch, hipStream_t st, int act = 0);
 hipError_t k_reduce_rows2(const float* in, float* out, const float* in2, float* out2, const float* bias, int bmod, long rows, long cols,
                           int fold, float scale, float* scratch, hipStream_t st, int act = 0);
+enum { REDUCE_SCALAR = 0, REDUCE_Q16 = 1, REDUCE_Q64 = 2, REDUCE_SLABS16 = 3, REDUCE_SLABS64 = 4 };
+struct ReducePlan { int kind; long rs, rps; };
+ReducePlan k_reduce_rows_plan(long rows, long cols, int nmat, bool plain, bool has_scratch, bool al_io, bool al_all);
+hipError_t k_reduce_rows_table(const float* in, float* out, float* scratch, const int* table, int nrows, int blocks1, int blocks2,
+                               long out_floats, long scratch_floats, hipStream_t st);
 hipError_t k_sum(const float* a, long n, float scale, float* out, float* ws, bool sq, hipStream_t st);
 hipError_t k_softmax_ce(const float* logits, const int32_t* labels, float* loss_rows, float* dlogits, int n, int c, int ld, float gs, hipStream_t st);
 hipError_t k_to_bf16(const float* x, unsigned short* y, long n, hipStream_t st);
diff --git a/tf_face_toolbox_amd/csrc/kernels.hip b/tf_face_toolbox_amd/csrc/kernels.hip
--- a/tf_face_toolbox_amd/csrc/kernels.hip
+++ b/tf_face_toolbox_amd/csrc/kernels.hip
@@ -197,15 +197,12 @@
     }
 }
 
-__global__ __launch_bounds__(256) void reduce_rows_kernel(const float* __restrict__ in, float* __restrict__ out,
-                                                          const float* __restrict__ bias, int bmod, long rows,
-                                                          long cols, long rows_per_split, float scale,
-                                                          const float* __restrict__ in2, float* __restrict__ out2, int act) {
-    __shared__ float sh[4][64];
-    if (blockIdx.z == 1) { in = in2; out = out2; }
+__device__ __forceinline__ void reduce_rows_body(const float* __restrict__ in, float* __restrict__ out, const float* __restrict__ bias, int bmod,
+                                                 long rows, long cols, long rows_per_split, float scale, int act, unsigned bx, unsigned by,
+                                                 float (*sh)[64]) {
     const int c = threadIdx.x & 63, rl = threadIdx.x >> 6;
-    const long j = (long)blockIdx.x * 64 + c;
-    const long r0 = (long)blockIdx.y * rows_per_split;
+    const long j = (long)bx * 64 + c;
+    const long r0 = (long)by * rows_per_split;
     const long r1 = min(rows, r0 + rows_per_split);
     float s0 = 0.f, s1 = 0.f;
     if (j < cols) {
@@ -230,8 +227,16 @@
         if (bias) v += bias[j % bmod];
         if (act == 1) v = fmaxf(v, 0.f);
         else if (act == 2) v = 1.f / (1.f + expf(-v));
-        out[(long)blockIdx.y * cols + j] = v;
-    }
+        out[(long)by * cols + j] = v;
+    }
+}
+__global__ __launch_bounds__(256) void reduce_rows_kernel(const float* __restrict__ in, float* __restrict__ out,
+                                                          const float* __restrict__ bias, int bmod, long rows,
+                                                          long cols, long rows_per_split, float scale,
+                                                          const float* __restrict__ in2, float* __restrict__ out2, int act) {
+    __shared__ float sh[4][64];
+    if (blockIdx.z == 1) { in = in2; out = out2; }
+    reduce_rows_body(in, out, bias, bmod, rows, cols, rows_per_split, scale, act, blockIdx.x, blockIdx.y, sh);
 }
 
 template <int QB>
@@ -263,14 +268,12 @@
 }
 
 template <int QB>
-__global__ __launch_bounds__(256) void reduce_rows_q_kernel(const f32x4* __restrict__ in, f32x4* __restrict__ out, long rows, long quads,
-                                                            long rows_per_split, const f32x4* __restrict__ in2, f32x4* __restrict__ out2) {
+__device__ __forceinline__ void reduce_rows_q_body(const f32x4* __restrict__ in, f32x4* __restrict__ out, long rows, long quads, long rows_per_split,
+                                                   unsigned bx, unsigned by, f32x4 (*sh)[QB]) {
     constexpr int RL = 256 / QB;
-    __shared__ f32x4 sh[RL][QB];
-    if (blockIdx.z == 1) { in = in2; out = out2; }
     const int cq = threadIdx.x % QB, rl = threadIdx.x / QB;
-    const long q = (long)blockIdx.x * QB + cq;
-    const long r0 = (long)blockIdx.y * rows_per_split, r1 = min(rows, r0 + rows_per_split);
+    const long q = (long)bx * QB + cq;
+    const long r0 = (long)by * rows_per_split, r1 = min(rows, r0 + rows_per_split);
     f32x4 s = {0.f, 0.f, 0.f, 0.f};
     if (q < quads) {
         const f32x4* src = in + q;
@@ -289,8 +292,54 @@
         f32x4 t = sh[0][cq];
 #pragma unroll
         for (int w = 1; w < RL; ++w) t += sh[w][cq];
-        out[(long)blockIdx.y * quads + q] = t;
-    }
+        out[(long)by * quads + q] = t;
+    }
+}
+template <int QB>
+__global__ __launch_bounds__(256) void reduce_rows_q_kernel(const f32x4* __restrict__ in, f32x4* __restrict__ out, long rows, long quads,
+                                                            long rows_per_split, const f32x4* __restrict__ in2, f32x4* __restrict__ out2) {
+    __shared__ f32x4 sh[256 / QB][QB];
+    if (blockIdx.z == 1) { in = in2; out = out2; }
+    reduce_rows_q_body<QB>(in, out, rows, quads, rows_per_split, blockIdx.x, blockIdx.y, sh);
+}
+
+template <int PASS>
+__global__ __launch_bounds__(256) void reduce_rows_table_kernel(const float* __restrict__ in, float* __restrict__ out, float* __restrict__ scratch,
+                                                                const int* __restrict__ table, int nrows, long out_floats, long scratch_floats) {
+    __shared__ int tb[64 * 12];
+    __shared__ f32x4 sh[256];
+    for (int i = threadIdx.x; i < nrows * 12; i += 256) tb[i] = table[i];
+    __syncthreads();
+    int q = -1;
+    for (int i = 0; i < nrows; ++i) {
+        const int f = tb[i * 12 + (PASS == 1 ? 10 : 11)];
+        if (f >= 0 && (int)blockIdx.x >= f) q = i;
+    }
+    if (q < 0) return;
+    const int* d = tb + q * 12;
+    const long rows = d[4], cols = d[5], rs = d[7], rps = d[8];
+    const int kind = d[6], nz = d[1] >= 0 ? 2 : 1;
+    const int QB = kind == 2 ? 64 : 16;
+    const long cb = kind == 0 ? (cols + 63) / 64 : (cols / 4 + QB - 1) / QB;
+    const long gy = PASS == 1 ? rs : 1;
+    const long local = (long)blockIdx.x - d[PASS == 1 ? 10 : 11];
+    const unsigned bx = (unsigned)(local % cb), by = (unsigned)((local / cb) % gy);
+    const long bz = local / (cb * gy);
+    if (bz >= nz) return;
+    const long o_off = bz ? d[3] : d[2], s_off = (long)d[9] + bz * rs * cols;
+    if (o_off < 0 || o_off + cols > out_floats || (rs > 1 && (d[9] < 0 || (long)d[9] + nz * rs * cols > scratch_floats))) return;
+    const float* src;
+    float* dst;
+    long nr, per;
+    if (PASS == 1) {
+        src = in + (bz ? d[1] : d[0]); nr = rows;
+        if (rs == 1) { dst = out + o_off; per = rows; } else { dst = scratch + s_off; per = rps; }
+    } else {
+        src = scratch + s_off; dst = out + o_off; nr = rs; per = rs;
+    }
+    if (kind == 2) reduce_rows_q_body<64>(reinterpret_cast<const f32x4*>(src), reinterpret_cast<f32x4*>(dst), nr, cols / 4, per, bx, by, reinterpret_cast<f32x4(*)[64]>(sh));
+    else if (kind == 1) reduce_rows_q_body<16>(reinterpret_cast<const f32x4*>(src), reinterpret_cast<f32x4*>(dst), nr, cols / 4, per, bx, by, reinterpret_cast<f32x4(*)[16]>(sh));
+    else reduce_rows_body(src, dst, nullptr, 1, nr, cols, per, 1.f, 0, bx, by, reinterpret_cast<float(*)[64]>(sh));
 }
 
 template <bool SQ>
@@ -1292,27 +1341,18 @@
 #undef FTE_CW
     return hipGetLastError();
 }
-hipError_t k_reduce_rows2(const float* in, float* out, const float* in2, float* out2, const float* bias, int bmod, long rows, long cols,
-                          int fold, float scale, float* scratch, hipStream_t st, int act) {
-    rows *= fold;
-    cols /= fold;
+ReducePlan k_reduce_rows_plan(long rows, long cols, int nmat, bool plain, bool has_scratch, bool al_io, bool al_all) {
+    ReducePlan pl;
+    pl.rs = 1; pl.rps = rows;
     static const bool slabs_off = getenv("FTE_REDUCE_SLABS") && atoi(getenv("FTE_REDUCE_SLABS")) == 0;
-    if (!slabs_off && !act && !in2 && !bias && scale == 1.f && rows >= 2 && rows < (1 << 20) && cols >= 4096 && cols % 4 == 0 &&
-        (reinterpret_cast<uintptr_t>(in) | reinterpret_cast<uintptr_t>(out)) % 16 == 0) {
+    if (!slabs_off && plain && nmat == 1 && rows >= 2 && rows < (1 << 20) && cols >= 4096 && cols % 4 == 0 && al_io) {
         const long quads = cols / 4;
-        if (quads / 64 >= 1024 || rows < 32)
-            hipLaunchKernelGGL(reduce_slabs_kernel<64>, dim3((unsigned)((quads + 63) / 64)), dim3(256), 0, st, reinterpret_cast<const f32x4*>(in),
-                               reinterpret_cast<f32x4*>(out), (int)rows, quads);
-        else
-            hipLaunchKernelGGL(reduce_slabs_kernel<16>, dim3((unsigned)((quads + 15) / 16)), dim3(256), 0, st, reinterpret_cast<const f32x4*>(in),
-                               reinterpret_cast<f32x4*>(out), (int)rows, quads);
-        return hipGetLastError();
-    }
-    const unsigned nz = in2 ? 2 : 1;
+        pl.kind = (quads / 64 >= 1024 || rows < 32) ? REDUCE_SLABS64 : REDUCE_SLABS16;
+        return pl;
+    }
+    const long nz = nmat;
     static const bool rq_off = getenv("FTE_REDUCE_ROWS_Q") && atoi(getenv("FTE_REDUCE_ROWS_Q")) == 0;
-    if (!rq_off && !act && scratch && !bias && scale == 1.f && rows >= 32 && cols % 4 == 0 && cols <= 1024 &&
-        (reinterpret_cast<uintptr_t>(in) | reinterpret_cast<uintptr_t>(out) | reinterpret_cast<uintptr_t>(in2) | reinterpret_cast<uintptr_t>(out2) |
-         reinterpret_cast<uintptr_t>(scratch)) % 16 == 0) {
+    if (!rq_off && plain && has_scratch && rows >= 32 && cols % 4 == 0 && cols <= 1024 && al_all) {
         const long quads = cols / 4;
         const int QB = quads >= 64 ? 64 : 16, RL = 256 / QB;
         const long qb = (quads + QB - 1) / QB;
@@ -1322,6 +1362,51 @@
         if (rs < 1 || rows < 256) rs = 1;
         const long rps = (rows + rs - 1) / rs;
         rs = (rows + rps - 1) / rps;
+        pl.kind = QB == 64 ? REDUCE_Q64 : REDUCE_Q16; pl.rs = rs; pl.rps = rs == 1 ? rows : rps;
+        return pl;
+    }
+    const long cb = (cols + 63) / 64;
+    long rs = 1;
+    if (has_scratch && cb < 512 && rows >= 64) {
+        rs = 1;
+        while (rs * rs < rows) ++rs;
+        if (rs < 256 / cb) rs = 256 / cb;
+        if (rs > 1024 / cb) rs = 1024 / cb;
+        if (rs > rows / 16) rs = rows / 16;
+        if (rs * cols * nz > REDUCE_SCRATCH_FLOATS) rs = REDUCE_SCRATCH_FLOATS / (cols * nz);
+        if (rs < 1) rs = 1;
+    }
+    pl.kind = REDUCE_SCALAR;
+    if (rs > 1) {
+        const long rps = (rows + rs - 1) / rs;
+        pl.rs = (rows + rps - 1) / rps; pl.rps = rps;
+    }
+    return pl;
+}
+hipError_t k_reduce_rows2(const float* in, float* out, const float* in2, float* out2, const float* bias, int bmod, long rows, long cols,
+                          int fold, float scale, float* scratch, hipStream_t st, int act) {
+    rows *= fold;
+    cols /= fold;
+    const bool al_io = (reinterpret_cast<uintptr_t>(in) | reinterpret_cast<uintptr_t>(out)) % 16 == 0;
+    const bool al_all = (reinterpret_cast<uintptr_t>(in) | reinterpret_cast<uintptr_t>(out) | reinterpret_cast<uintptr_t>(in2) | reinterpret_cast<uintptr_t>(out2) |
+                         reinterpret_cast<uintptr_t>(scratch)) % 16 == 0;
+    const ReducePlan pl = k_reduce_rows_plan(rows, cols, in2 ? 2 : 1, !act && !bias && scale == 1.f, scratch != nullptr, al_io, al_all);
+    const long rs = pl.rs, rps = pl.rps;
+    if (pl.kind == REDUCE_SLABS64 || pl.kind == REDUCE_SLABS16) {
+        const long quads = cols / 4;
+        if (pl.kind == REDUCE_SLABS64)
+            hipLaunchKernelGGL(reduce_slabs_kernel<64>, dim3((unsigned)((quads + 63) / 64)), dim3(256), 0, st, reinterpret_cast<const f32x4*>(in),
+                               reinterpret_cast<f32x4*>(out), (int)rows, quads);
+        else
+            hipLaunchKernelGGL(reduce_slabs_kernel<16>, dim3((unsigned)((quads + 15) / 16)), dim3(256), 0, st, reinterpret_cast<const f32x4*>(in),
+                               reinterpret_cast<f32x4*>(out), (int)rows, quads);
+        return hipGetLastError();
+    }
+    const unsigned nz = in2 ? 2 : 1;
+    if (pl.kind == REDUCE_Q64 || pl.kind == REDUCE_Q16) {
+        const long quads = cols / 4;
+        const int QB = pl.kind == REDUCE_Q64 ? 64 : 16;
+        const long qb = (quads + QB - 1) / QB;
         f32x4* s1 = reinterpret_cast<f32x4*>(scratch);
         f32x4* s2 = s1 + rs * quads;
 #define FTE_RQ(QB_, GY_, IN_, OUT_, ROWS_, RPS_, IN2_, OUT2_) hipLaunchKernelGGL((reduce_rows_q_kernel<QB_>), dim3((unsigned)qb, (unsigned)(GY_), nz), dim3(256), 0, st, \
@@ -1336,27 +1421,23 @@
         return hipGetLastError();
     }
     const long cb = (cols + 63) / 64;
-    long rs = 1;
-    if (scratch && cb < 512 && rows >= 64) {
-        rs = 1;
-        while (rs * rs < rows) ++rs;
-        if (rs < 256 / cb) rs = 256 / cb;
-        if (rs > 1024 / cb) rs = 1024 / cb;
-        if (rs > rows / 16) rs = rows / 16;
-        if (rs * cols * nz > REDUCE_SCRATCH_FLOATS) rs = REDUCE_SCRATCH_FLOATS / (cols * nz);
-        if (rs < 1) rs = 1;
-    }
     if (rs == 1) {
         hipLaunchKernelGGL(reduce_rows_kernel, dim3((unsigned)cb, 1, nz), dim3(256), 0, st, in, out, bias, bmod, rows, cols, rows, scale, in2, out2, act);
         return hipGetLastError();
     }
-    const long rps = (rows + rs - 1) / rs;
-    rs = (rows + rps - 1) / rps;
     float* scratch2 = scratch + rs * cols;
     hipLaunchKernelGGL(reduce_rows_kernel, dim3((unsigned)cb, (unsigned)rs, nz), dim3(256), 0, st, in, scratch, (const float*)nullptr, 1, rows, cols, rps, 1.f,
                        in2, scratch2, 0);
     hipLaunchKernelGGL(reduce_rows_kernel, dim3((unsigned)cb, 1, nz), dim3(256), 0, st, (const float*)scratch, out, bias, bmod, rs, cols, rs, scale,
                        (const float*)scratch2, out2, act);
+    return hipGetLastError();
+}
+hipError_t k_reduce_rows_table(const float* in, float* out, float* scratch, const int* table, int nrows, int blocks1, int blocks2,
+                               long out_floats, long scratch_floats, hipStream_t st) {
+    if (nrows <= 0 || nrows > 64 || blocks1 <= 0 || blocks2 < 0) return hipErrorInvalidValue;
+    hipLaunchKernelGGL(reduce_rows_table_kernel<1>, dim3((unsigned)blocks1), dim3(256), 0, st, in, out, scratch, table, nrows, out_floats, scratch_floats);
+    if (blocks2 > 0)
+        hipLaunchKernelGGL(reduce_rows_table_kernel<2>, dim3((unsigned)blocks2), dim3(256), 0, st, in, out, scratch, table, nrows, out_floats, scratch_floats);
     return hipGetLastError();
 }
 hipError_t k_reduce_rows(const float* in, float* out, const float* bias, int bmod, long rows, long cols, int fold, float scale,
diff --git a/tf_face_toolbox_amd/csrc/wino.h b/tf_face_toolbox_amd/csrc/wino.h
--- a/tf_face_toolbox_amd/csrc/wino.h
+++ b/tf_face_toolbox_amd/csrc/wino.h
@@ -14,6 +14,8 @@
 hipError_t wino_transform_tiles(const float* x, float* pack, int n, int h, int w, int c, int mode, hipStream_t st, bool small = false,
                                 const float* alpha = nullptr);
 hipError_t wino_transform_filter(const float* w, float* pack, int cin, int cout, int dgrad, hipStream_t st);
+hipError_t wino_transform_filter_table(const float* params, float* packs, const int* table, int nrows, int nblocks, long pack_floats, hipStream_t st);
+inline int wino_filter_blocks(int cin, int cout) { return (cin >> 6) * (cout >> 4); }
 
 struct WinoMMParams {
     const float* V;
diff --git a/tf_face_toolbox_amd/csrc/wino.hip b/tf_face_toolbox_amd/csrc/wino.hip
--- a/tf_face_toolbox_amd/csrc/wino.hip
+++ b/tf_face_toolbox_amd/csrc/wino.hip
@@ -130,6 +130,62 @@
         o[(size_t)(4 * i + 2) * 512] = 0.5f * (p[i][0] - p[i][1] + p[i][2]);
         o[(size_t)(4 * i + 3) * 512] = p[i][2];
     }
+}
+
+__device__ __forceinline__ void wino_filter_quad(const float* __restrict__ w, float* __restrict__ pack, int cin, int cout, int dgrad, int rb, int ko, int t) {
+    const int K = dgrad ? cout : cin, KS = K >> 3;
+    const int half = t & 1, r = (t >> 1) & 63;
+    const int row = rb * 64 + r, k0 = ko * 8 + half * 4;
+    f32x4 g[3][3];
+#pragma unroll
+    for (int a = 0; a < 3; ++a)
+#pragma unroll
+        for (int b = 0; b < 3; ++b) {
+            if (dgrad) {
+                g[a][b] = *reinterpret_cast<const f32x4*>(w + (((2 - a) * 3 + (2 - b)) * (size_t)cin + row) * cout + k0);
+            } else {
+#pragma unroll
+                for (int e = 0; e < 4; ++e) g[a][b][e] = w[((a * 3 + b) * (size_t)cin + k0 + e) * cout + row];
+            }
+        }
+    f32x4 p[4][3];
+#pragma unroll
+    for (int b = 0; b < 3; ++b) {
+        p[0][b] = g[0][b];
+        p[1][b] = 0.5f * (g[0][b] + g[1][b] + g[2][b]);
+        p[2][b] = 0.5f * (g[0][b] - g[1][b] + g[2][b]);
+        p[3][b] = g[2][b];
+    }
+    float* o = pack + ((((size_t)rb * KS + ko) * 16) * 64 + r) * 8 + ((half ^ ((r >> 4) & 1)) << 2);
+#pragma unroll
+    for (int i = 0; i < 4; ++i) {
+        *reinterpret_cast<f32x4*>(o + (size_t)(4 * i + 0) * 512) = p[i][0];
+        *reinterpret_cast<f32x4*>(o + (size_t)(4 * i + 1) * 512) = 0.5f * (p[i][0] + p[i][1] + p[i][2]);
+        *reinterpret_cast<f32x4*>(o + (size_t)(4 * i + 2) * 512) = 0.5f * (p[i][0] - p[i][1] + p[i][2]);
+        *reinterpret_cast<f32x4*>(o + (size_t)(4 * i + 3) * 512) = p[i][2];
+    }
+}
+__global__ __launch_bounds__(256) void wino_filter_quads_kernel(const float* __restrict__ w, float* __restrict__ pack, int cin, int cout, int dgrad) {
+    const int KP = (dgrad ? cout : cin) >> 4;
+    const int rb = (int)blockIdx.x / KP, ko = ((int)blockIdx.x - rb * KP) * 2 + (threadIdx.x >> 7);
+    wino_filter_quad(w, pack, cin, cout, dgrad, rb, ko, threadIdx.x & 127);
+}
+__global__ __launch_bounds__(256) void wino_filter_table_kernel(const float* __restrict__ params, float* __restrict__ packs,
+                                                                const int* __restrict__ table, int nrows, long pack_floats) {
+    __shared__ int tb[64 * 6];
+    for (int i = threadIdx.x; i < nrows * 6; i += 256) tb[i] = table[i];
+    __syncthreads();
+    int q = -1;
+    for (int i = 0; i < nrows; ++i)
+        if ((int)blockIdx.x >= tb[i * 6 + 5]) q = i;
+    if (q < 0) return;
+    const int* d = tb + q * 6;
+    const int cin = d[1], cout = d[2], dgrad = d[3];
+    const int K = dgrad ? cout : cin, NR = dgrad ? cin : cout;
+    const int local = (int)blockIdx.x - d[5], KP = K >> 4;
+    const int rb = local / KP, ko = (local - rb * KP) * 2 + (threadIdx.x >> 7);
+    if (rb >= (NR >> 6) || (long)d[4] + 16L * cin * cout > pack_floats) return;
+    wino_filter_quad(params + d[0], packs + d[4], cin, cout, dgrad, rb, ko, threadIdx.x & 127);
 }
 
 template <int EPI, int NWN, bool LEAN>
@@ -631,8 +687,19 @@
 
 hipError_t wino_transform_filter(const float* w, float* pack, int cin, int cout, int dgrad, hipStream_t st) {
     if (cin % 64 || cout % 64) return hipErrorInvalidValue;
-    const int total = cin * cout;
-    hipLaunchKernelGGL(wino_filter_kernel, dim3((total + 255) / 256), dim3(256), 0, st, w, pack, cin, cout, dgrad);
+    const char* e = getenv("FTE_WINO_FILTER_QUADS");
+    if ((e && atoi(e) == 0) || ((uintptr_t)w | (uintptr_t)pack) % 16) {
+        const int total = cin * cout;
+        hipLaunchKernelGGL(wino_filter_kernel, dim3((total + 255) / 256), dim3(256), 0, st, w, pack, cin, cout, dgrad);
+    } else {
+        hipLaunchKernelGGL(wino_filter_quads_kernel, dim3((unsigned)wino_filter_blocks(cin, cout)), dim3(256), 0, st, w, pack, cin, cout, dgrad);
+    }
+    return hipGetLastError();
+}
+
+hipError_t wino_transform_filter_table(const float* params, float* packs, const int* table, int nrows, int nblocks, long pack_floats, hipStream_t st) {
+    if (nrows <= 0 || nrows > 64 || nblocks <= 0) return hipErrorInvalidValue;
+    hipLaunchKernelGGL(wino_filter_table_kernel, dim3((unsigned)nblocks), dim3(256), 0, st, params, packs, table, nrows, pack_floats);
     return hipGetLastError();
 }
 
diff --git a/tf_face_toolbox_amd/nets/_wino_packs.py b/tf_face_toolbox_amd/nets/_wino_packs.py
--- /dev/null
+++ b/tf_face_toolbox_amd/nets/_wino_packs.py
@@ -0,0 +1,88 @@
+import ctypes
+
+import torch
+
+from .. import _lib
+
+CHUNK = 64
+
+
+class WinoFilterPacks(object):
+
+    def __init__(self, entries, device):
+        q = _lib.query
+        rows = {0: [], 1: []}
+        off = 0
+        self.fwd, self.dgrad = {}, {}
+        spans = []
+        for name, src, cin, cout, want_f, want_d in entries:
+            size = q('fte_wino_filter_pack_bytes', cin, cout) // 4
+            if not size:
+                continue
+            for dg, want in ((0, want_f), (1, want_d)):
+                if want:
+                    rows[dg].append([int(src), cin, cout, dg, off, q('fte_wino_filter_pack_blocks', cin, cout)])
+                    spans.append((name, dg, off, size))
+                    off += size
+        self.total = off
+        self.arena = torch.empty(max(off, 4), dtype=torch.float32, device=device)
+        for name, dg, o, size in spans:
+            (self.dgrad if dg else self.fwd)[name] = self.arena[o:o + size]
+        self.launches = {0: [], 1: []}
+        for dg in (0, 1):
+            for c0 in range(0, len(rows[dg]), CHUNK):
+                tab, first = [], 0
+                for src, cin, cout, d, dst, blocks in rows[dg][c0:c0 + CHUNK]:
+                    tab.append([src, cin, cout, d, dst, first])
+                    first += blocks
+                self.launches[dg].append((torch.tensor(tab, dtype=torch.int32, device=device).contiguous(), len(tab), first))
+
+    def _refresh(self, dg, params, st):
+        for tab, n, blocks in self.launches[dg]:
+            _lib.call('fte_wino_pack_filters_table', params, self.arena, tab, n, blocks, self.arena.numel(), st)
+
+    def refresh_fwd(self, params, st):
+        self._refresh(0, params, st)
+
+    def refresh_dgrad(self, params, st):
+        self._refresh(1, params, st)
+
+
+def reduce_plan(rows, cols, nmat):
+    plan = (ctypes.c_int * 6)()
+    r = _lib.query('fte_reduce_rows_plan', rows, cols, nmat, ctypes.cast(plan, ctypes.c_void_p))
+    if r != 0:
+        raise _lib.FteError('fte_reduce_rows_plan(%d, %d, %d) failed with code %d' % (rows, cols, nmat, r))
+    return tuple(plan)
+
+
+class PartsReducer(object):
+
+    def __init__(self, layers, device):
+        self.parts, self.launches = {}, []
+        off = soff = 0
+        rows_all = []
+        for key, rows, cols, nbytes, o1, o2 in layers:
+            assert nbytes % 32 == 0 and o1 % 4 == 0 and (o2 is None or o2 % 4 == 0), (key, nbytes, o1, o2)
+            nmat = 1 if o2 is None else 2
+            kind, rs, rps, b1, b2, sfl = reduce_plan(rows, cols, nmat)
+            half = nbytes // 8
+            rows_all.append((key, off, nbytes // 4, [off, off + half if nmat == 2 else -1, o1, -1 if o2 is None else o2, rows, cols, kind, rs, rps,
+                                                     soff if b2 else 0], b1, b2))
+            off += nbytes // 4
+            soff += (sfl + 3) // 4 * 4
+        self.arena = torch.empty(max(off, 4), dtype=torch.float32, device=device)
+        self.scratch = torch.empty(max(soff, 4), dtype=torch.float32, device=device)
+        for key, o, size, _, _, _ in rows_all:
+            self.parts[key] = self.arena[o:o + size]
+        for c0 in range(0, len(rows_all), CHUNK):
+            tab, f1, f2 = [], 0, 0
+            for _, _, _, row, b1, b2 in rows_all[c0:c0 + CHUNK]:
+                tab.append(row + [f1, f2 if b2 else -1])
+                f1 += b1
+                f2 += b2
+            self.launches.append((torch.tensor(tab, dtype=torch.int32, device=device).contiguous(), len(tab), f1, f2))
+
+    def run(self, out, out_floats, st):
+        for tab, n, b1, b2 in self.launches:
+            _lib.call('fte_reduce_rows_table', self.arena, out, self.scratch, tab, n, b1, b2, out_floats, self.scratch.numel(), st)
diff --git a/tf_face_toolbox_amd/nets/sphere.py b/tf_face_toolbox_amd/nets/sphere.py
--- a/tf_face_toolbox_amd/nets/sphere.py
+++ b/tf_face_toolbox_amd/nets/sphere.py
@@ -103,8 +103,21 @@
         self.loss_slots = self.grads[off:off + 4]
         self.state = self._make_state()
         self._init_params()
+        self._build_wino_packs()
         self.built = True
         return self
+
+    def _build_wino_packs(self):
+        from ._wino_packs import WinoFilterPacks
+        q = _lib.query
+        self._wpack_key = q('fte_get_conv_algo')
+        ent = []
+        for c in self.convs[1:]:
+            if c.stride == 1:
+                ent.append((c.name, self.variables[c.name + '/weights'].offset, c.cin, c.cout,
+                            q('fte_conv3x3_algo', 1, c.hin, c.win, c.cin, c.cout, 1, 0) == 1,
+                            q('fte_conv3x3_algo', 1, c.hin, c.win, c.cin, c.cout, 1, 1) == 1))
+        self.wpacks = WinoFilterPacks(ent, self.device)
 
     def _make_state(self):
         return OrderedDict()
@@ -180,6 +193,8 @@
             return
         self._act_key = key
         dev = self.device
+        if getattr(self, '_wpack_key', None) != key[2]:
+            self._build_wino_packs()
         f32 = dict(dtype=torch.float32, device=dev)
         i16 = dict(dtype=torch.int16, device=dev)
         self._act_s16 = s16
@@ -237,6 +252,22 @@
                    q('fte_gemm_ws_bytes', n, EMBED, self.fin), q('fte_gemm_ws_bytes', n, hw, EMBED))
         self.ws = torch.empty((need + 3) // 4 + 1024, **f32)
         self.ws_bytes = self.ws.numel() * 4
+        self.use_up = [False] * len(self.convs)
+        self.use_ud = [False] * len(self.convs)
+        self.reducer = None
+        if not s16 and _lib.get_mfma_dtype() == 'f32':
+            from ._wino_packs import PartsReducer
+            lay = []
+            for l, c in enumerate(self.convs):
+                if l == 0:
+                    continue
+                self.use_up[l] = c.name in self.wpacks.fwd and q('fte_conv3x3_algo', n, c.hin, c.win, c.cin, c.cout, c.stride, 0) == 1
+                self.use_ud[l] = c.name in self.wpacks.dgrad and q('fte_conv3x3_algo', n, c.hin, c.win, c.cin, c.cout, c.stride, 1) == 1
+                p = self.convs[l - 1]
+                lay.append((l, q('fte_conv3x3_dgrad_parts_rows', n, c.hin, c.win, c.cin, c.cout, c.stride), c.cin,
+                            q('fte_conv3x3_dgrad_parts_bytes', n, c.hin, c.win, c.cin, c.cout, c.stride),
+                            self.variables[p.name + '/alpha'].offset, self.variables[p.name + '/biases'].offset if p.has_bias else None))
+            self.reducer = PartsReducer(lay, dev)
         self.side = side_stream(self.device) if os.environ.get('FTE_SIDE_STREAM', '1') != '0' else None
         self.ws_side = torch.empty_like(self.ws) if self.side is not None else self.ws
         self._alloc_head(n)
@@ -342,6 +373,17 @@
         if copies:
             self._alloc_copies()
             self._pack_weights(st)
+        mode = os.environ.get('FTE_WINO_PACKS', 'auto')
+        if mode == 'auto':
+            mode = '1' if n <= int(os.environ.get('FTE_WINO_PACKS_MAX', '64')) else 'parts'
+        packs_on = not copies and self.reducer is not None and mode in ('1', 'filters')
+        self._packs_live = packs_on and keep
+        self._parts_live = keep and not copies and self.reducer is not None and mode in ('1', 'parts')
+        if packs_on:
+            self.wpacks.refresh_fwd(self.params, st)
+            if keep:
+                self.wpacks.refresh_dgrad(self.params, st)
+
         def part_pack(l, c, lo, hi, m):
             vp = self.vpack[l]
             if m != n:
@@ -363,6 +405,19 @@
                     call('fte_conv2d_fwd_s16', self.y16[l - 1][lo:hi], self.w16t[c.name], bv, av, self.y16[l - 2][lo:hi] if c.second == 1 else None,
                          z16, self.y16[l][lo:hi], zz, self.y[l][lo:hi] if self.y[l] is not None else None, m, c.hin, c.win, c.cin, c.cout, 3, c.stride,
                          ws, self.ws_bytes, st)
+            elif packs_on and self.use_up[l]:
+                up = self.wpacks.fwd[c.name]
+                if lean_live and self.lean[l]:
+                    p = self.convs[l - 1]
+                    call('fte_conv3x3_fwd_pack', self.z[l - 1][lo:hi], self.view(p.name + '/alpha'), wv, bv, av, self.y[l - 2][lo:hi], zz,
+                         self.y[l][lo:hi], m, c.hin, c.win, c.cin, c.cout, c.stride, part_pack(l, c, lo, hi, m), up, ws, self.ws_bytes, st)
+                elif lean_live and l + 1 < nl and self.lean[l + 1]:
+                    call('fte_conv3x3_fwd_pack', self.y[l - 1][lo:hi], None, wv, bv, av, None, zz, None,
+                         m, c.hin, c.win, c.cin, c.cout, c.stride, part_pack(l, c, lo, hi, m), up, ws, self.ws_bytes, st)
+                else:
+                    vp = part_pack(l, c, lo, hi, m) if keep and self.vpack[l] is not None else None
+                    call('fte_conv3x3_fwd_pack', self._y_buf(l - 1)[lo:hi], None, wv, bv, av, self.y[l - 2][lo:hi] if c.second == 1 else None, zz,
+                         self._y_buf(l)[lo:hi], m, c.hin, c.win, c.cin, c.cout, c.stride, vp, up, ws, self.ws_bytes, st)
             elif lean_live and self.lean[l]:
                 p = self.convs[l - 1]
                 call('fte_conv3x3_fwd_keep_act', self.z[l - 1][lo:hi], self.view(p.name + '/alpha'), wv, bv, av, self.y[l - 2][lo:hi], zz,
@@ -527,6 +582,8 @@
         trace = getattr(self, '_trace_dz', None)
         main, side = torch.cuda.current_stream(), self._side_stream(n)
         wst, wws = (side.cuda_stream, self.ws_side) if side is not None else (st, self.ws)
+        packs_live = getattr(self, '_packs_live', False) and not copies and self.reducer is not None
+        parts_live = getattr(self, '_parts_live', False) and not copies and self.reducer is not None
         readers = {}
         last_w = None
         for l in range(last, -1, -1):
@@ -535,6 +592,8 @@
                 trace[c.name] = (dz16_cur if s16 else dz_cur).clone()
             gw = self.view(c.name + '/weights', g)
             if l == 0:
+                if parts_live:
+                    self.reducer.run(g, self.small_end, st)
                 if last_w is not None:
                     main.wait_event(last_w)
                 if s16:
@@ -606,6 +665,13 @@
                      self.view(p.name + '/biases', g) if p.has_bias else None,
                      n, c.hin, c.win, c.cin, c.cout, 3, c.stride, self.ws, self.ws_bytes, st)
                 dz16_cur = dz16_prev
+            elif packs_live or parts_live:
+                pt = self.reducer.parts[l] if parts_live else None
+                call('fte_conv3x3_dgrad_pack', dz_cur, self.view(c.name + '/weights'), addin, self.z[l - 1],
+                     self.view(p.name + '/alpha'), raw, dz_prev, self.view(p.name + '/alpha', g),
+                     self.view(p.name + '/biases', g) if p.has_bias else None,
+                     n, c.hin, c.win, c.cin, c.cout, c.stride, self.wpacks.dgrad[c.name] if packs_live and self.use_ud[l] else None, pt, pt.numel() * 4 if parts_live else 0,
+                     self.ws, self.ws_bytes, st)
             else:
                 call('fte_conv3x3_dgrad', dz_cur, self.view(c.name + '/weights'), addin, self.z[l - 1],
                      self.view(p.name + '/alpha'), raw, dz_prev, self.view(p.name + '/alpha', g),
```

Result: no change. 15350 images/sec, median of 3 (-0.1%).
